# GavinLynch04/FastSelect

Hardware: AMD Instinct MI355X
Metric: feature-scores/sec (n*p/s) MultiSURF fp32 (higher is better)
Workload: dtype u16 pass 1, fp32 pass 2 (fp64 accumulation)

## Files before the change

### fastselect_amd/csrc/fs_api.cpp

```cpp
#include <cmath>
#include <cstring>
#include <string>
#include <vector>

#include "../../include/fastselect_amd.h"
#include "fs_cfs.h"
#include "fs_internal.h"
#include "fs_jmi.h"
#include "fs_mdr.h"
#include "fs_mi.h"
#include "fs_mrmr.h"
#include "fs_pairscan.h"
#include "fs_stir.h"

#include <chrono>
#include <cstdio>
#include <cstdlib>

namespace fs {
static thread_local std::string g_last_error;
void set_error(const std::string& msg) { g_last_error = msg; }

static thread_local int g_accum = FS_ACCUM_FAST;
int accumulation_mode() { return g_accum; }

TestHooks& test_hooks() {
  static TestHooks h;
  return h;
}

bool trace_on() {
  static const bool on = std::getenv("FS_TRACE") != nullptr;
  return on;
}

void trace_mark(const char* phase) {
  if (!trace_on()) return;
  using clk = std::chrono::steady_clock;
  static thread_local clk::time_point last = clk::now();
  const clk::time_point now = clk::now();
  std::fprintf(stderr, "[fs_trace] %-22s %9.3f ms\n", phase,
               std::chrono::duration<double, std::milli>(now - last).count());
  last = now;
}
}

using namespace fs;

static int map_prep_rc(int rc) { return rc == 0 ? FS_OK : FS_EINVAL; }

static int apply_accumulation(Prepared& P) {
  P.ref_accum = g_accum == FS_ACCUM_REFERENCE ? 1 : 0;
  if (P.ref_accum && P.algo == ALGO_MULTISURF && !test_hooks().ref_q16) P.no_q16 = 1;
  return FS_OK;
}

static int no_reference_devices() {
  if (g_accum != FS_ACCUM_REFERENCE) return FS_OK;
  set_error("reference-order accumulation runs on one device (its column sums are one "
            "sequential float32 sum per feature)");
  return FS_ENOTSUP;
}

static int check_backend(int backend, int device) {
  if (backend != FS_BACKEND_CPU && backend != FS_BACKEND_GPU) {
    set_error("backend must be FS_BACKEND_CPU or FS_BACKEND_GPU");
    return FS_EINVAL;
  }
  if (backend == FS_BACKEND_GPU) {
    const int nd = gpu::device_count();
    if (nd <= 0) {
      set_error("backend='gpu' was selected, but no HIP device (MI355X) is visible");
      return FS_ENODEV;
    }
    if (device < 0 || device >= nd) {
      set_error("device ordinal out of range");
      return FS_EINVAL;
    }
  }
  return FS_OK;
}

static int check_devices(const int* devices, int n) {
  if (!devices || n < 1) {
    set_error("devices: need at least one device ordinal");
    return FS_EINVAL;
  }
  const int nd = gpu::device_count();
  if (nd <= 0) {
    set_error("backend='gpu' was selected, but no HIP device (MI355X) is visible");
    return FS_ENODEV;
  }
  for (int i = 0; i < n; i++)
    if (devices[i] < 0 || devices[i] >= nd) {
      set_error("devices: ordinal " + std::to_string(devices[i]) + " out of range (" +
                std::to_string(nd) + " visible)");
      return FS_EINVAL;
    }
  return FS_OK;
}

extern "C" {

const char* fs_version(void) { return "fastselect_amd 0.1.0 (gfx950)"; }

const char* fs_last_error(void) { return g_last_error.c_str(); }

int fs_device_count(void) { return gpu::device_count(); }

int fs_set_accumulation(int mode, int* previous) {
  if (mode != FS_ACCUM_FAST && mode != FS_ACCUM_REFERENCE) {
    set_error("accumulation mode must be FS_ACCUM_FAST or FS_ACCUM_REFERENCE");
    return FS_EINVAL;
  }
  if (previous) *previous = g_accum;
  g_accum = mode;
  return FS_OK;
}

int fs_get_accumulation(void) { return g_accum; }

int fs_test_hook(const char* name, int64_t value) {
  if (!name) {
    set_error("fs_test_hook: name is NULL");
    return FS_EINVAL;
  }
  TestHooks& h = test_hooks();
  const std::string k(name);
  if (k == "reset") h = TestHooks();
  else if (k == "ksplit") h.ksplit = value;
  else if (k == "q16") h.q16 = value;
  else if (k == "sparse") h.sparse = value;
  else if (k == "shards") h.shards = value;
  else if (k == "q16_guard_off") h.q16_guard_off = value;
  else if (k == "thr_exact_all") h.thr_exact_all = value;
  else if (k == "exact_gather") h.exact_gather = value;
  else if (k == "row_panel") h.row_panel = value;
  else if (k == "rf_xlds") h.rf_xlds = value;
  else if (k == "rf_fcap") h.rf_fcap = value;
  else if (k == "ties_1w") h.ties_1w = value;
  else if (k == "ties_coop") h.ties_coop = value;
  else if (k == "rf_ref_replay") h.rf_ref_replay = value;
  else if (k == "ref_q16") h.ref_q16 = value;
  else if (k == "surf_f64") h.surf_f64 = value;
  else if (k == "star_split") h.star_split = value;
  else if (k == "colsort_star") h.colsort_star = value;
  else if (k == "colsort_bins12") h.colsort_bins12 = value;
  else if (k == "colsort_global") h.colsort_global = value;
  else if (k == "mi_tiles") h.mi_tiles = value;
  else if (k == "list_cap") h.list_cap = value;
  else if (k == "cfs_rows_cap") h.cfs_rows_cap = value;
  else if (k == "seg_len") h.seg_len = value;
  else if (k == "pass2_generic") h.pass2_generic = value;
  else if (k == "mdr_top_cap") h.mdr_top_cap = value;
  else if (k == "mdr_ranks") h.mdr_ranks = value;
  else if (k == "mdr_blocks") h.mdr_blocks = value;
  else if (k == "mdr_labels") h.mdr_labels = value;
  else if (k == "pair_tiles") h.pair_tiles = value;
  else if (k == "pair_cap") h.pair_cap = value;
  else if (k == "pair_labels") h.pair_labels = value;
  else if (k == "pair_lab_ranks") h.pair_lab_ranks = value;
  else if (k == "stir_chunk") h.stir_chunk = value;
  else if (k == "stir_seg_len") h.stir_seg_len = value;
  else {
    set_error("fs_test_hook: unknown hook '" + k + "'");
    return FS_EINVAL;
  }
  return FS_OK;
}

int fs_multisurf_last_guard(double* risk_out, int* rerun_out) {
  return gpu::multisurf_last_guard(risk_out, rerun_out);
}

int fs_device_cache_release(void) {
  gpu::dev_cache_release();
  return FS_OK;
}

int fs_host_alloc(uint64_t bytes, void** out) {
  if (!out) {
    set_error("fs_host_alloc: out is NULL");
    return FS_EINVAL;
  }
  *out = nullptr;
  if (gpu::device_count() <= 0) {
    set_error("backend='gpu' requested but no HIP device is visible");
    return FS_ENODEV;
  }
  return gpu::host_alloc(out, (size_t)bytes);
}

int fs_host_free(void* p) {
  gpu::host_free(p);
  return FS_OK;
}

int fs_stage_x(int device, const void* x, int x_is_f64, int64_t n, int64_t p, uint64_t* staged) {
  if (!x || !staged || n < 1 || p < 1) {
    set_error("fs_stage_x: need x, staged, n >= 1 and p >= 1");
    return FS_EINVAL;
  }
  if (gpu::device_count() <= 0) {
    set_error("backend='gpu' requested but no HIP device is visible");
    return FS_ENODEV;
  }
  return gpu::stage_x(device, x, x_is_f64, n, p, staged);
}

int fs_stage_x_device(int device, const void* x, const void* x_device, int x_is_f64, int64_t n,
                      int64_t p, uint64_t* staged) {
  if (!x || !x_device || !staged || n < 1 || p < 1) {
    set_error("fs_stage_x_device: need x, x_device, staged, n >= 1 and p >= 1");
    return FS_EINVAL;
  }
  if (gpu::device_count() <= 0) {
    set_error("backend='gpu' requested but no HIP device is visible");
    return FS_ENODEV;
  }
  return gpu::stage_x_device(device, x, x_device, x_is_f64, n, p, staged);
}

int fs_stage_x_cast(int device, const void* x, int x_is_f64, int64_t n, int64_t p, int n_jobs,
                    float* out, int* finite, uint64_t* staged) {
  if (!x || !out || !finite || !staged || n < 1 || p < 1) {
    set_error("fs_stage_x_cast: need x, out, finite, staged, n >= 1 and p >= 1");
    return FS_EINVAL;
  }
  if (gpu::device_count() <= 0) {
    set_error("backend='gpu' requested but no HIP device is visible");
    return FS_ENODEV;
  }
  return gpu::stage_x_cast(device, x, x_is_f64, n, p, n_jobs, out, finite, staged);
}

int fs_unstage_x(uint64_t staged) { return gpu::unstage_x(staged); }

int fs_all_finite(const void* x, int x_is_f64, int64_t n, int64_t p, int n_jobs, int* finite) {
  if (!x || !finite || n < 0 || p < 0) {
    set_error("fs_all_finite: need x, finite, n >= 0 and p >= 0");
    return FS_EINVAL;
  }
  *finite = cpu::all_finite(x, x_is_f64, n * p, n_jobs);
  return FS_OK;
}

int fs_column_stats(int backend, int device, const void* x, int x_is_f64, int64_t n, int64_t p,
                    int64_t count_cap, void* colmin_out, void* colmax_out,
                    int64_t* ndistinct_out) {
  int rc = check_backend(backend, device);
  if (rc != FS_OK) return rc;
  if (!x || !colmin_out || !colmax_out || !ndistinct_out || n < 1 || p < 1 || count_cap < 0) {
    set_error("fs_column_stats: need x, outputs, n >= 1, p >= 1 and count_cap >= 0");
    return FS_EINVAL;
  }
  const int f64 = x_is_f64 ? 1 : 0;
  trace_mark("column_stats: enter");
  if (backend == FS_BACKEND_GPU)
    rc = gpu::column_stats(x, f64, n, p, count_cap, device, colmin_out, colmax_out, ndistinct_out);
  else
    rc = cpu::column_stats(x, f64, n, p, count_cap, -1, colmin_out, colmax_out, ndistinct_out);
  trace_mark("column_stats");
  return rc;
}

int fs_multisurf_score(int backend, int device, const float* x, int64_t n, int64_t p,
                       const double* y, const float* recip, const int64_t* feat_idx,
                       int64_t n_kept, int use_star, const uint8_t* is_discrete, int n_jobs,
                       float* scores_out) {
  if (!scores_out) {
    set_error("scores_out is NULL");
    return FS_EINVAL;
  }
  int rc = check_backend(backend, device);
  if (rc != FS_OK) return rc;
  Prepared P;
  trace_mark("multisurf: enter");
  rc = prepare(P, ALGO_MULTISURF, x, 0, n, p, feat_idx, n_kept, recip, is_discrete, n_jobs,
               backend == FS_BACKEND_GPU);
  trace_mark("prepare (host)");
  if (rc) return map_prep_rc(rc);
  if (encode_labels_f64(P, y)) return FS_EINVAL;
  P.use_star = use_star ? 1 : 0;
  if ((rc = apply_accumulation(P)) != FS_OK) return rc;
  if (backend == FS_BACKEND_GPU) return gpu::multisurf_run(P, x, device, scores_out);
  cpu::CpuState st;
  std::vector<double> rs(3 * n), cnt(2 * n), S(P.n_kept);
  cpu::multisurf_pass1(P, x, 0, 1, n_jobs, st, rs.data());
  cpu::multisurf_select(P, x, 0, 1, rs.data(), n_jobs, st, cnt.data());
  cpu::multisurf_pass2(P, x, st, cnt.data(), 0, 1, n_jobs, 0, n, S.data());
  for (int64_t k = 0; k < P.n_kept; k++) scores_out[k] = (float)(S[k] / (double)n);
  return FS_OK;
}

int fs_multisurf_score_rows(int backend, int device, const float* x, int64_t n, int64_t p,
                            const double* y, const float* recip, const int64_t* feat_idx,
                            int64_t n_kept, int use_star, const uint8_t* is_discrete, int n_jobs,
                            int64_t row_begin, int64_t row_end, double* sums_out) {
  if (!sums_out) {
    set_error("sums_out is NULL");
    return FS_EINVAL;
  }
  if (!(0 <= row_begin && row_begin <= row_end && row_end <= n)) {
    set_error("row range must satisfy 0 <= row_begin <= row_end <= n");
    return FS_EINVAL;
  }
  int rc = check_backend(backend, device);
  if (rc != FS_OK) return rc;
  Prepared P;
  rc = prepare(P, ALGO_MULTISURF, x, 0, n, p, feat_idx, n_kept, recip, is_discrete, n_jobs,
               backend == FS_BACKEND_GPU);
  if (rc) return map_prep_rc(rc);
  if (encode_labels_f64(P, y)) return FS_EINVAL;
  P.use_star = use_star ? 1 : 0;
  if ((rc = apply_accumulation(P)) != FS_OK) return rc;
  if (backend == FS_BACKEND_GPU) return gpu::multisurf_rows(P, x, device, row_begin, row_end, sums_out);
  cpu::CpuState st;
  std::vector<double> rs(3 * n), cnt(2 * n);
  cpu::multisurf_pass1(P, x, 0, 1, n_jobs, st, rs.data());
  cpu::multisurf_select(P, x, 0, 1, rs.data(), n_jobs, st, cnt.data());
  return cpu::multisurf_pass2(P, x, st, cnt.data(), 0, 1, n_jobs, row_begin, row_end, sums_out);
}

static int relieff_sums(int backend, int device, const float* x, int64_t n, int64_t p,
                        const int32_t* y_enc, const float* recip, const uint8_t* is_discrete,
                        int64_t k, const float* class_probs, int64_t n_classes, int n_jobs,
                        int64_t r_lo, int64_t r_hi, double* sums, const int* devices = nullptr,
                        int n_devices = 0) {
  if (!y_enc || !class_probs || n_classes < 1 || k < 0) {
    set_error("invalid ReliefF arguments (y_enc, class_probs, n_classes, k)");
    return FS_EINVAL;
  }
  if (!(0 <= r_lo && r_lo <= r_hi && r_hi <= n)) {
    set_error("row range must satisfy 0 <= row_begin <= row_end <= n");
    return FS_EINVAL;
  }
  int rc = check_backend(backend, device);
  if (rc != FS_OK) return rc;
  Prepared P;
  trace_mark("relieff: enter");
  rc = prepare(P, ALGO_RELIEFF, x, 0, n, p, nullptr, p, recip, is_discrete, n_jobs,
               backend == FS_BACKEND_GPU);
  trace_mark("prepare (host)");
  if (rc) return map_prep_rc(rc);
  P.labels.assign(y_enc, y_enc + n);
  for (int64_t i = 0; i < n; i++)
    if (P.labels[i] < 0 || P.labels[i] >= n_classes) {
      set_error("y_enc entry outside [0, n_classes)");
      return FS_EINVAL;
    }
  P.n_classes = (int32_t)n_classes;
  P.class_prior.assign(n_classes, 0.0);
  for (int64_t c = 0; c < n_classes; c++) P.class_prior[c] = (double)class_probs[c];
  P.k_neighbors = k;
  if ((rc = apply_accumulation(P)) != FS_OK) return rc;
  if (devices) {
    if ((rc = no_reference_devices()) != FS_OK) return rc;
    if (n_classes > 64) {
      set_error("GPU ReliefF supports at most 64 classes");
      return FS_ENOTSUP;
    }
    return gpu::rows_run_devices(P, x, devices, n_devices, r_lo, r_hi, sums);
  }
  if (backend == FS_BACKEND_GPU) return gpu::relieff_run(P, x, device, r_lo, r_hi, sums);
  return cpu::relieff_run(P, x, n_jobs, r_lo, r_hi, sums);
}

static int surf_sums(int backend, int device, const double* x, int64_t n, int64_t p,
                     const int32_t* y, const float* recip, int use_star,
                     const uint8_t* is_discrete, int n_jobs, int64_t r_lo, int64_t r_hi,
                     double* sums, const int* devices = nullptr, int n_devices = 0) {
  if (!(0 <= r_lo && r_lo <= r_hi && r_hi <= n)) {
    set_error("row range must satisfy 0 <= row_begin <= row_end <= n");
    return FS_EINVAL;
  }
  int rc = check_backend(backend, device);
  if (rc != FS_OK) return rc;
  Prepared P;
  trace_mark("surf: enter");
  rc = prepare(P, ALGO_SURF, x, 1, n, p, nullptr, p, recip, is_discrete, n_jobs,
               backend == FS_BACKEND_GPU);
  trace_mark("prepare (host)");
  if (rc) return map_prep_rc(rc);
  if (encode_labels_i32(P, y)) return FS_EINVAL;
  P.use_star = use_star ? 1 : 0;
  if ((rc = apply_accumulation(P)) != FS_OK) return rc;
  if (devices) {
    if ((rc = no_reference_devices()) != FS_OK) return rc;
    return gpu::rows_run_devices(P, x, devices, n_devices, r_lo, r_hi, sums);
  }
  if (backend == FS_BACKEND_GPU) return gpu::surf_run(P, x, device, r_lo, r_hi, sums);
  return cpu::surf_run(P, x, n_jobs, r_lo, r_hi, sums);
}

int fs_relieff_score(int backend, int device, const float* x, int64_t n, int64_t p,
                     const int32_t* y_enc, const float* recip, const uint8_t* is_discrete,
                     int64_t k, const float* class_probs, int64_t n_classes, int n_jobs,
                     float* scores_out) {
  if (!scores_out) {
    set_error("scores_out is NULL");
    return FS_EINVAL;
  }
  std::vector<double> S(p > 0 ? p : 1);
  const int rc = relieff_sums(backend, device, x, n, p, y_enc, recip, is_discrete, k,
                              class_probs, n_classes, n_jobs, 0, n, S.data());
  if (rc != FS_OK) return rc;
  for (int64_t f = 0; f < p; f++) scores_out[f] = (float)(S[f] / (double)n);
  return FS_OK;
}

int fs_relieff_score_rows(int backend, int device, const float* x, int64_t n, int64_t p,
                          const int32_t* y_enc, const float* recip, const uint8_t* is_discrete,
                          int64_t k, const float* class_probs, int64_t n_classes, int n_jobs,
                          int64_t row_begin, int64_t row_end, double* sums_out) {
  if (!sums_out) {
    set_error("sums_out is NULL");
    return FS_EINVAL;
  }
  return relieff_sums(backend, device, x, n, p, y_enc, recip, is_discrete, k, class_probs,
                      n_classes, n_jobs, row_begin, row_end, sums_out);
}

int fs_surf_score(int backend, int device, const double* x, int64_t n, int64_t p,
                  const int32_t* y, const float* recip, int use_star,
                  const uint8_t* is_discrete, int n_jobs, float* scores_out) {
  if (!scores_out) {
    set_error("scores_out is NULL");
    return FS_EINVAL;
  }
  std::vector<double> S(p > 0 ? p : 1);
  const int rc = surf_sums(backend, device, x, n, p, y, recip, use_star, is_discrete, n_jobs, 0,
                           n, S.data());
  if (rc != FS_OK) return rc;
  for (int64_t f = 0; f < p; f++) scores_out[f] = (float)(S[f] / (double)n);
  return FS_OK;
}

int fs_surf_score_rows(int backend, int device, const double* x, int64_t n, int64_t p,
                       const int32_t* y, const float* recip, int use_star,
                       const uint8_t* is_discrete, int n_jobs, int64_t row_begin,
                       int64_t row_end, double* sums_out) {
  if (!sums_out) {
    set_error("sums_out is NULL");
    return FS_EINVAL;
  }
  return surf_sums(backend, device, x, n, p, y, recip, use_star, is_discrete, n_jobs, row_begin,
                   row_end, sums_out);
}

int fs_multisurf_score_devices(const int* devices, int n_devices, const float* x, int64_t n,
                               int64_t p, const double* y, const float* recip,
                               const int64_t* feat_idx, int64_t n_kept, int use_star,
                               const uint8_t* is_discrete, int n_jobs, int64_t row_begin,
                               int64_t row_end, double* sums_out) {
  if (!sums_out) {
    set_error("sums_out is NULL");
// ... 956 lines not shown
```

### fastselect_amd/csrc/fs_gpu_internal.h

```cpp
#pragma once
#include <hip/hip_runtime.h>

#include <algorithm>
#include <atomic>
#include <cmath>
#include <condition_variable>
#include <cstdio>
#include <cstdlib>
#include <cstring>
#include <map>
#include <mutex>
#include <string>
#include <thread>
#include <type_traits>
#include <unordered_map>
#include <vector>

#include "../../include/fastselect_amd.h"
#include "fs_devmem.h"
#include "fs_internal.h"

namespace fs {
namespace gpu {

#define FS_HIP(expr)                                                                      \
  do {                                                                                    \
    hipError_t e_ = (expr);                                                               \
    if (e_ != hipSuccess) {                                                               \
      set_error(std::string("HIP error '") + hipGetErrorString(e_) + "' in " #expr);      \
      return FS_EHIP;                                                                     \
    }                                                                                     \
  } while (0)

constexpr int kRowcorrMaxSlices = 16;
constexpr int kExRows = 8, kExJ = 4, kExChunk = kExJ;
constexpr int kSWaves = 16;
constexpr int kTileWeights = kTile * kTile;
constexpr int64_t kXsSlack = 512;
constexpr int kXcds = 8;


__device__ __forceinline__ uint32_t sad_u32(uint32_t a, uint32_t b, uint32_t c) {
  uint32_t d;
  asm("v_sad_u32 %0, %1, %2, %3" : "=v"(d) : "v"(a), "v"(b), "v"(c));
  return d;
}

__device__ __forceinline__ uint32_t sad_u16(uint32_t a, uint32_t b, uint32_t c) {
  uint32_t d;
  asm("v_sad_u16 %0, %1, %2, %3" : "=v"(d) : "v"(a), "v"(b), "v"(c));
  return d;
}

__device__ __forceinline__ uint32_t mismatch_u32(uint32_t a, uint32_t b, uint32_t sc, uint32_t c) {
  uint32_t t, d;
  asm("v_xor_b32 %1, %2, %3\n\tv_min_u32 %1, %1, 1\n\tv_mad_u32_u24 %0, %1, %4, %5"
      : "=v"(d), "=&v"(t)
      : "v"(a), "v"(b), "v"(sc), "v"(c));
  return d;
}

__device__ __forceinline__ double block_sum_256(double v, double* red) {
  const int tid = threadIdx.x;
  red[tid] = v;
  __syncthreads();
  for (int s = 128; s > 0; s >>= 1) {
    if (tid < s) red[tid] += red[tid + s];
    __syncthreads();
  }
  const double r = red[0];
  __syncthreads();
  return r;
}

__device__ __forceinline__ int64_t d_at(int tiled, int64_t n_pad, int64_t t, int64_t i0,
                                        int64_t j0, int a, int b) {
  return tiled ? ((t * kTile + b) * kTile + a) : ((j0 + b) * n_pad + i0 + a);
}

__device__ __forceinline__ bool d_row_in(int2 win, int64_t r) { return r >= win.x && r < win.y; }
__device__ __forceinline__ int64_t d_rd(int tiled, int2 win, int64_t n_pad, int64_t t, int64_t i0,
                                        int64_t j0, int a, int b) {
  if (tiled) return (t * kTile + b) * kTile + a;
  const int64_t j = j0 + b;
  return d_row_in(win, j) ? j * n_pad + i0 + a : (i0 + a) * n_pad + j;
}

struct Plan {
  explicit Plan(int dev) : device(dev) {}
  Prepared P;
  const int device;
  int rank = 0, world = 1;
  int x_is_f64 = 0;
  hipStream_t stream = nullptr;
  bool own_stream = false;
  hipStream_t side = nullptr;
  hipEvent_t ev_fork = nullptr, ev_join = nullptr;
  hipStream_t side2 = nullptr;
  hipEvent_t ev_star = nullptr;
  int64_t nb = 0, n_tiles = 0, seg_len = 1, nseg = 1;
  int64_t nsegpart = 1;
  int ksplit = 1;
  int64_t kfull = 0;
  int use_q16 = 0;
  double calib[7] = {0, 0, 0, 0, 1, 0, 0};
  double cal32[2] = {0, 0};
  int64_t c_lo = 0, c_hi = 0;
  int64_t r_lo = 0, r_hi = 0;
  double2* rspart = nullptr;
  double* Dpart = nullptr;
  int key_shift = 8;
  DevBuf<char> colsort_scratch{device};
  void* x = nullptr;
  const void* x_staged = nullptr;
  int64_t* src_col = nullptr;
  int64_t* out_pos = nullptr;
  double *off = nullptr, *qs = nullptr, *scl = nullptr;
  float* scl32 = nullptr;
  bool rows_direct = false;
  int64_t* dtab_off = nullptr;
  double* dtab = nullptr;
  int32_t* lab = nullptr;
  uint8_t* lab8 = nullptr;
  uint32_t* xqT = nullptr;
  float* xs = nullptr;
  float* epsT = nullptr;
  double* corr = nullptr;
  double* corr_part = nullptr;
  double* xT64 = nullptr;
  bool surf_int = false;
  double* D = nullptr;
  int tiled = 0;
  int64_t dplane = 0;
  int2 tw = make_int2(0, 0);
  int2 win = make_int2(0, 0);
  void* D_alloc = nullptr;
  float* Dk = nullptr;
  int2* tiles = nullptr;
  double* thr = nullptr;
  float* Wt = nullptr;
  float* wrow = nullptr;
  unsigned long long* nnz = nullptr;
  bool nnz_valid = false;
  int sparse = 0;
  bool star_split = false;
  float* xsT = nullptr;
  double* alpha = nullptr;
  double* tcol = nullptr;
  DevBuf<double> spart{device};
  std::vector<int2> h_tiles;
  DevBuf<int32_t> sched{device};
  int32_t* seg_off = nullptr;
  DevBuf<int2> units8{device};
  int2* units4 = nullptr;
  int64_t nunits8 = 0, nunits4 = 0, nfb8 = 0, nfb4 = 0, f_tail = 0;
  unsigned int* unc = nullptr;
  int32_t* urows = nullptr;
  DevBuf<double2> uparts{device};
  int thr_rows = kExactThrRows;
  bool thr_all = false;
  int32_t n_exact_thr = 0;
  DevBuf<int2> list{device};
  DevBuf<double> pair_part{device};
  unsigned long long* list_count = nullptr;
  int64_t n_refined = 0;
  int64_t n_tie_rows = 0;
  DevBuf<char> sort_scratch{device};
  hipEvent_t ev[6] = {nullptr, nullptr, nullptr, nullptr, nullptr, nullptr};
  std::vector<hipEvent_t> ev_stir;
  int stir_chunks = 0;
  DevArena mem_plan{device};
  DevArena mem_layout{device};
  DevArena mem_shard{device};
  DevArena mem_call{device};
  bool row_mode = false;
  bool corr_ready = false;
  bool guard_pending = false;
  std::vector<char> colmin, colmax;
  float* xk = nullptr;
  double* xk64 = nullptr;
  int64_t Kp = 0;
  int64_t* kcol = nullptr;
  float* krecip = nullptr;
  uint8_t* kdisc = nullptr;
  uint8_t* kblk = nullptr;
  uint64_t* masks = nullptr;
  int32_t* bcnt = nullptr;
  DevBuf<float> temp{device};
  int64_t ref_rows = -1;
  bool ref_defer = false;
  DevBuf<float> rkeys{device};
  bool ref_seeded = false;
  double* risk_dev = nullptr;
};

#define FS_TRY(expr)              \
  do {                            \
    int rc_ = (expr);             \
    if (rc_ != FS_OK) return rc_; \
  } while (0)

template <typename T>
int h2d(Plan* g, T* dst, const T* src, size_t count) {
  if (count == 0) return FS_OK;
  FS_HIP(hipMemcpyAsync(dst, src, count * sizeof(T), hipMemcpyHostToDevice, g->stream));
  return FS_OK;
}

inline int launch_check(const char* what) {
  hipError_t e = hipGetLastError();
  if (e != hipSuccess) {
    set_error(std::string("kernel launch failed (") + what + "): " + hipGetErrorString(e));
    return FS_EHIP;
  }
  return FS_OK;
}

hipStream_t stream_get(int device);
void stream_put(int device, hipStream_t s);
hipEvent_t event_get(int device, bool timing);
void event_put(int device, hipEvent_t e, bool timing);
struct StreamLease {
  int device;
  hipStream_t s = nullptr;
  std::vector<hipEvent_t> ev;
  explicit StreamLease(int dev) : device(dev) {}
  StreamLease(const StreamLease&) = delete;
  StreamLease& operator=(const StreamLease&) = delete;
  int open(size_t events) {
    if (!(s = stream_get(device))) return FS_EHIP;
    for (size_t k = 0; k < events; k++) {
      ev.push_back(event_get(device, true));
      if (!ev.back()) return FS_EHIP;
    }
    return FS_OK;
  }
  ~StreamLease() {
    if (s) {
      (void)hipStreamSynchronize(s);
      stream_put(device, s);
    }
    for (hipEvent_t e : ev) event_put(device, e, true);
    (void)hipGetLastError();
  }
};
inline int no_device() {
  set_error("backend='gpu' requested but no HIP device is visible");
  return FS_ENODEV;
}
int choose_ksplit(int64_t tiles, int device, int nchunks, int64_t feats, bool beside);
int calibrate_band(Plan* g);
int row_guard(Plan* g);
int apply_operand_width(Plan* g);
int run_quantize_dist(Plan* g);
int plan_score_surf(Plan* g, double* sums_dev);
int surf_resolve(Plan* g);
bool star_split_fits(int64_t n, int32_t n_classes);
int star_terms(Plan* g, hipStream_t st);
int star_sums(Plan* g, hipStream_t st, bool continuous);
int star_reduce(Plan* g, const double* counts, hipStream_t st);
int shard_segments(Plan* g);
int run_weights(Plan* g, const double* counts, int algo, double inv_sc);
int run_pass2(Plan* g, double* scores_dev);
int ref_masks(Plan* g);
int ref_temp(Plan* g, int64_t rows, float** out);
int ref_chains(Plan* g, const double* counts, double* scores);
int surf_ref(Plan* g, double* sums);
int accumulate(double* dst, const double* src, int64_t count, hipStream_t st);
int reduce_segments(const double* part, int64_t nrows, int64_t PW, const int64_t* out_pos,
                    double* sums, hipStream_t st, const double* add = nullptr);
int plan_score_relieff(Plan* g, double* sums_dev);
int relieff_run_one(const Prepared& P, const void* x, int device, int64_t r_lo, int64_t r_hi,
                    double* sums_out, const double* seed = nullptr);
int plan_layout(Plan* g);
int copy_sums(Plan* g, const double* sums_dev, double* sums_out);
int surf_run_one(const Prepared& P, const void* x, int device, int64_t r_lo, int64_t r_hi,
                 double* sums_out, const double* seed = nullptr);
extern thread_local double g_last_risk;
extern thread_local int g_last_rerun;

}
}
```

### fastselect_amd/csrc/fs_internal.h

```cpp
#pragma once

#include <cmath>
#include <condition_variable>
#include <cstdint>
#include <mutex>
#include <string>
#include <utility>
#include <vector>

#if defined(__HIPCC__)
#define FS_HD __host__ __device__
#else
#define FS_HD
#endif

namespace fs {

enum Algo : int { ALGO_MULTISURF = 0, ALGO_RELIEFF = 1, ALGO_SURF = 2 };

constexpr int kTile = 128;
constexpr int kBK64 = 16;
constexpr int kBKQ = 16;
constexpr int kFlushChunks = 256 / kBKQ;
constexpr int kHiShift = 24;
constexpr int kFeatPad = 64;
constexpr int kSubRows = 32;

void set_error(const std::string& msg);
bool trace_on();
void trace_mark(const char* phase);

struct Prepared {
  int algo = ALGO_MULTISURF;
  int use_star = 0;
  int64_t k_neighbors = 0;
  int64_t n = 0, n_pad = 0;
  int64_t p_in = 0;
  int64_t n_kept = 0;
  int64_t pc = 0, pd = 0;
  int64_t PC = 0, PD = 0, PW = 0;
  std::vector<int64_t> src_col, out_pos;
  std::vector<double> offset;
  std::vector<float> recip_in;
  std::vector<uint8_t> disc_in;
  std::vector<int64_t> kept_col;
  std::vector<double> scale;
  std::vector<int64_t> dtab_off;
  std::vector<double> dtab;
  std::vector<int32_t> labels;
  int32_t n_classes = 0;
  std::vector<double> class_prior;
  double SC = 0.0;
  uint32_t SCu = 0;
  double amb_delta = 0.0;
  double amb_delta_model = 0.0;
  double Rmax = 0.0;
  double qmax = 0.0;
  int ranges_ready = 1;
  int disc_bits = 0;
  int q16 = 0;
  int no_q16 = 0;
  int ref_accum = 0;
  int defer_guard = 0;
};

int accumulation_mode();

struct TestHooks {
  int64_t q16 = -1;
  int64_t sparse = -1;
  int64_t shards = 0;
  int64_t ksplit = 0;
  int64_t q16_guard_off = 0;
  int64_t thr_exact_all = 0;
  int64_t exact_gather = 0;
  int64_t row_panel = 0;
  int64_t rf_xlds = -1;
  int64_t rf_fcap = -1;
  int64_t ties_1w = 0;
  int64_t ties_coop = 0;
  int64_t rf_ref_replay = 0;
  int64_t ref_q16 = 0;
  int64_t surf_f64 = -1;
  int64_t star_split = -1;
  int64_t colsort_star = -1;
  int64_t colsort_bins12 = 0;
  int64_t colsort_global = 0;
  int64_t mi_tiles = 0;
  int64_t list_cap = 0;
  int64_t cfs_rows_cap = 0;
  int64_t seg_len = 0;
  int64_t pass2_generic = 0;
  int64_t mdr_top_cap = 0;
  int64_t mdr_ranks = 0;
  int64_t mdr_blocks = 0;
  int64_t mdr_labels = 0;
  int64_t pair_tiles = 0;
  int64_t pair_cap = 0;
  int64_t pair_labels = 0;
  int64_t pair_lab_ranks = 0;
  int64_t stir_chunk = 0;
  int64_t stir_seg_len = 0;
};
TestHooks& test_hooks();

int prepare(Prepared& P, int algo, const void* x, int x_is_f64, int64_t n, int64_t p_in,
            const int64_t* feat_idx, int64_t n_kept, const float* recip,
            const uint8_t* is_discrete, int n_jobs, int device_ranges = 0,
            const Prepared* dtab_src = nullptr);
int finalize_scale(Prepared& P, const double* cmin, const double* cmax);
int set_integer_scale(Prepared& P, int q16);
constexpr int64_t kCalibPairs = 4096;
void calib_pairs(int64_t n, int64_t pc, int64_t count,
                 std::vector<std::pair<int64_t, int64_t>>& out);
double calibrated_delta(double model, double SC, double rms, double max_abs);
inline int colsort_key_shift(double qmax) {
  int b = 0;
  while (b < 32 && std::ldexp(1.0, b) < qmax) b++;
  return 32 - b < 24 ? 32 - b : 24;
}
inline int32_t colsort_fx(float eps) { return (int32_t)std::llrint((double)eps * 16777216.0); }
inline uint32_t colsort_key(uint32_t q, int32_t fx, int s) {
  const uint32_t fr = (uint32_t)(((1 << 23) - fx) >> (24 - s));
  const uint32_t m = (1u << s) - 1u;
  return (q << s) | (fr < m ? fr : m);
}
constexpr int kColsortMaxFill = 64;
inline uint32_t colsort_eq12(int32_t fx) {
  const int32_t u = fx + (1 << 23);
  return (uint32_t)(u < 0 ? 0 : (u >= (1 << 24) ? 4095 : (u >> 12)));
}
inline int64_t colsort_eq12_fx(uint32_t q) { return (int64_t)(2 * q + 1) * 2048 - (int64_t(1) << 23); }
int encode_labels_f64(Prepared& P, const double* y);
int encode_labels_i32(Prepared& P, const int32_t* y);

void owned_tiles(int64_t nb, int rank, int world, std::vector<int32_t>& bi,
                 std::vector<int32_t>& bj);
void row_tiles(int64_t nb, int64_t b_lo, int64_t b_hi, std::vector<int32_t>& bi,
               std::vector<int32_t>& bj);
FS_HD inline int64_t tile_linear(int64_t nb, int64_t bi, int64_t bj) {
  return bi * nb - bi * (bi - 1) / 2 + (bj - bi);
}

int hardware_threads(int n_jobs);

constexpr int kExactThrRows = 64;
inline int64_t exact_thr_rows(int64_t n, int64_t p) {
  const double budget = 3e10 / ((double)(n > 1 ? n : 1) * (double)(p > 1 ? p : 1));
  int64_t r = n / 64 < (int64_t)budget ? n / 64 : (int64_t)budget;
  return r > kExactThrRows ? r : kExactThrRows;
}

FS_HD inline double multisurf_threshold(double s1, double s2, int64_t n) {
  const double mu = s1 / (double)(n - 1);
  double var = s2 / (double)(n - 1) - mu * mu;
  if (var < 0.0) var = 0.0;
  return mu - 0.5 * __builtin_sqrt(var);
}

FS_HD inline double multisurf_weight(bool near, bool hit, int use_star, double H, double M) {
  if (near) return hit ? -1.0 / H : 1.0 / M;
  if (use_star && !hit) return -1.0 / (M > 0.0 ? M : 1.0);
  return 0.0;
}

FS_HD inline double surf_weight(bool near, bool hit, int use_star) {
  if (near) return hit ? -1.0 : 1.0;
  if (use_star) return hit ? 1.0 : -1.0;
  return 0.0;
}

template <typename KeyFn, typename RangeFn>
FS_HD inline int numba_argsort_focus(int64_t len, int32_t* R, KeyFn key, RangeFn has_interest) {
  if (len < 2) return 0;
  constexpr int kSmall = 15, kMaxStack = 100;
  int64_t st_lo[kMaxStack], st_hi[kMaxStack];
  int ns = 1;
  st_lo[0] = 0;
  st_hi[0] = len - 1;
  while (ns > 0) {
    ns--;
    int64_t low = st_lo[ns], high = st_hi[ns];
    bool live = true;
    while (high - low >= kSmall) {
      const int64_t mid = (low + high) >> 1;
      int32_t tmp;
      if (key(R[mid]) < key(R[low])) { tmp = R[low]; R[low] = R[mid]; R[mid] = tmp; }
      if (key(R[high]) < key(R[mid])) { tmp = R[high]; R[high] = R[mid]; R[mid] = tmp; }
      if (key(R[mid]) < key(R[low])) { tmp = R[low]; R[low] = R[mid]; R[mid] = tmp; }
      const float pivot = key(R[mid]);
      tmp = R[high]; R[high] = R[mid]; R[mid] = tmp;
      int64_t i = low, j = high - 1;
      while (true) {
        while (i < high && key(R[i]) < pivot) i++;
        while (j >= low && pivot < key(R[j])) j--;
        if (i >= j) break;
        tmp = R[i]; R[i] = R[j]; R[j] = tmp;
        i++;
        j--;
      }
      tmp = R[i]; R[i] = R[high]; R[high] = tmp;
      int64_t push_lo, push_hi, keep_lo, keep_hi;
      if (high - i > i - low) {
        push_lo = i + 1; push_hi = high; keep_lo = low; keep_hi = i - 1;
      } else {
        push_lo = low; push_hi = i - 1; keep_lo = i + 1; keep_hi = high;
      }
      if (push_hi >= push_lo && has_interest(push_lo, push_hi)) {
        if (ns >= kMaxStack) return -1;
        st_lo[ns] = push_lo;
        st_hi[ns] = push_hi;
        ns++;
      }
      low = keep_lo;
      high = keep_hi;
      if (high < low || !has_interest(low, high)) {
        live = false;
        break;
      }
    }
    if (!live) continue;
    for (int64_t i = low + 1; i <= high; i++) {
      const int32_t kk = R[i];
      const float v = key(kk);
      int64_t j = i;
      while (j > low && v < key(R[j - 1])) {
        R[j] = R[j - 1];
        j--;
      }
      R[j] = kk;
    }
  }
  return 0;
}

namespace cpu {
int all_finite(const void* x, int x_is_f64, int64_t count, int n_jobs);
struct CpuState {
  std::vector<double> D;
  std::vector<float> xs;
  std::vector<double> corr;
  std::vector<double> thr;
  int64_t refined = 0;
};
int multisurf_pass1(const Prepared& P, const void* x, int rank, int world, int n_jobs,
                    CpuState& S, double* rowstats);
int multisurf_select(const Prepared& P, const void* x, int rank, int world,
                     const double* rowstats, int n_jobs, CpuState& S, double* counts);
int multisurf_pass2(const Prepared& P, const void* x, const CpuState& S, const double* counts,
                    int rank, int world, int n_jobs, int64_t r_lo, int64_t r_hi, double* scores);
int surf_run(const Prepared& P, const void* x, int n_jobs, int64_t r_lo, int64_t r_hi,
             double* scores);
int relieff_run(const Prepared& P, const void* x, int n_jobs, int64_t r_lo, int64_t r_hi,
                double* scores);
int column_stats(const void* x, int x_is_f64, int64_t n, int64_t p, int64_t cap, int n_jobs,
                 void* colmin, void* colmax, int64_t* ndistinct);
}

class StageBarrier {
 public:
  explicit StageBarrier(int n) : n_(n) {}
  bool arrive(int rc, const std::string& err) {
    std::unique_lock<std::mutex> lk(mu_);
    if (rc != 0 && rc_ == 0) {
      rc_ = rc;
      err_ = err;
    }
    const uint64_t gen = gen_;
    if (++count_ == n_) {
      count_ = 0;
      last_ok_ = rc_ == 0;
      gen_++;
      cv_.notify_all();
    } else {
      cv_.wait(lk, [&] { return gen_ != gen; });
    }
    return last_ok_;
  }
  int rc() const { return rc_; }
  const std::string& err() const { return err_; }
  int waiting() {
    std::lock_guard<std::mutex> lk(mu_);
    return count_;
  }

 private:
  std::mutex mu_;
  std::condition_variable cv_;
  int n_, count_ = 0, rc_ = 0;
  bool last_ok_ = true;
  uint64_t gen_ = 0;
  std::string err_;
};


namespace gpu {
int device_count();
int dev_alloc(void** p, size_t bytes, int device);
void dev_free(void* p);
void dev_cache_release();
int host_alloc(void** p, size_t bytes);
void host_free(void* p);
int stage_x(int device, const void* x, int x_is_f64, int64_t n, int64_t p, uint64_t* handle);
int stage_x_cast(int device, const void* x, int x_is_f64, int64_t n, int64_t p, int n_jobs,
                 float* out, int* finite, uint64_t* handle);
int stage_x_device(int device, const void* x, const void* x_dev, int x_is_f64, int64_t n,
                   int64_t p, uint64_t* handle);
int unstage_x(uint64_t handle);
const void* staged_lookup(const void* host, int64_t n, int64_t p, int x_is_f64, int device);
const void* staged_acquire(const void* host, int64_t n, int64_t p, int x_is_f64, int device);
void staged_release(const void* dev);
bool staged_extrema(const void* dev, void* cmin, void* cmax);
int column_stats(const void* x, int x_is_f64, int64_t n, int64_t p, int64_t cap, int device,
                 void* colmin, void* colmax, int64_t* ndistinct);
int column_minmax(const void* dx, int x_is_f64, int64_t n, int64_t p, void* hmin, void* hmax,
                  void* stream);
size_t pair_sort_scratch_bytes(int64_t count);
int sort_pairs(void* list, int64_t count, void* scratch, size_t scratch_bytes, void* stream);
bool colsort_lds(int64_t n);
int colsort_bin_bits(int64_t n);
size_t colsort_scratch_bytes(int64_t n, int64_t ncols);
int colsort_terms(const uint32_t* xqT, float* epsT, int64_t n, int64_t n_pad, int64_t c_lo,
                  int64_t c_hi, int q16, int key_shift, void* scratch, size_t scratch_bytes,
                  void* stream);
int colsort_star_terms(const uint32_t* xqT, float* epsT, float* xsT, const int32_t* lab,
                       const int64_t* out_pos, int ncls, int64_t n, int64_t n_pad, int64_t c_lo,
                       int64_t c_hi, int q16, int key_shift, void* stream);
struct Plan;
int plan_create(Plan** out, const Prepared& P, const void* x, int x_is_f64, int device,
                int rank, int world, uint64_t stream, int64_t r_lo = 0, int64_t r_hi = -1);
int plan_set_features(Plan* g, const Prepared& P);
int plan_pass1(Plan* g, double* rowstats_dev);
int plan_select(Plan* g, const double* rowstats_dev, double* counts_dev);
int plan_pass2(Plan* g, const double* counts_dev, double* scores_dev);
int plan_stir(Plan* g, double* sums_dev);
double plan_stir_kernel_ms(const Plan* g, int which);
int64_t ref_mask_words(const Plan* g);
int plan_ref_masks(Plan* g, uint64_t* masks_dev);
int plan_ref_pass2(Plan* g, const uint64_t* masks_dev, const double* counts_dev, int64_t row_lo,
                   int64_t row_hi);
int plan_ref_sums(Plan* g, const double* init_dev, double* sums_dev);
int plan_ref_temp(Plan* g);
int plan_decision_guard(Plan* g, const double* rowstats, const double* counts,
                        const double* sums, double* risk, int* switched);
int plan_set_rows(Plan* g, int64_t r_lo, int64_t r_hi);
int plan_set_shard(Plan* g, int rank, int world);
int multisurf_shards(const Prepared& P, int device, int world, int share = 1);
int plan_score(Plan* g, double* sums_dev);
int plan_info(const Plan* g, int64_t* tiles, double* pfe, int64_t* refined);
int plan_calibration(const Plan* g, double* out);
double plan_kernel_ms(const Plan* g, int which);
int plan_weighted_pairs(Plan* g, int64_t* pairs);
void plan_destroy(Plan* g);
int multisurf_run(const Prepared& P, const void* x, int device, float* scores_out);
int multisurf_last_guard(double* risk, int* rerun);
int multisurf_run_devices(const Prepared& P, const void* x, const int* devices, int ndev,
                          int64_t r_lo, int64_t r_hi, double* sums_out);
int rows_run_devices(const Prepared& P, const void* x, const int* devices, int ndev,
                     int64_t r_lo, int64_t r_hi, double* sums_out);
int multisurf_rows(const Prepared& P, const void* x, int device, int64_t r_lo, int64_t r_hi,
                   double* sums_out);
int surf_run(const Prepared& P, const void* x, int device, int64_t r_lo, int64_t r_hi,
             double* sums_out);
int relieff_run(const Prepared& P, const void* x, int device, int64_t r_lo, int64_t r_hi,
                double* sums_out);

namespace refacc {
int gather_kept(const float* x, int64_t n, int64_t n_pad, int64_t p_in, const int64_t* kcol,
                int64_t n_kept, int64_t Kp, float* xk, void* stream);
int gather_kept64(const double* x, int64_t n, int64_t n_pad, int64_t p_in, const int64_t* kcol,
                  int64_t n_kept, int64_t Kp, double* xk, void* stream);
int surf_masks(const double* D, int64_t n, int64_t n_pad, const double* avg, const int32_t* lab,
               int use_star, int64_t r_lo, int64_t r_hi, uint64_t* masks, void* stream);
int surf_chains(const double* xk, int64_t Kp, const float* krecip, const uint8_t* kdisc,
                const uint8_t* blkdisc, const uint64_t* masks, int64_t n, int64_t n_pad,
                int use_star, int64_t r_lo, int64_t r_hi, float* temp, void* stream);
int multisurf_masks(const double* D, int64_t n, int64_t n_pad, const void* tiles, int64_t n_tiles,
                    const double* thr, const int32_t* lab, int use_star, uint64_t* masks,
                    void* stream);
int multisurf_chains(const float* xk, int64_t Kp, const float* krecip, const uint8_t* kdisc,
                     const uint8_t* blkdisc, const uint64_t* masks, int64_t n, int64_t n_pad,
                     const double* counts, int use_star, int64_t r_lo, int64_t r_hi, float* temp,
                     void* stream);
int column_sums(const float* temp, int64_t rows, int64_t Kp, int64_t n_kept, const double* init,
                double* out, void* stream);
int relieff_order(const float* xk, int64_t Kp, const float* krecip, const uint8_t* kdisc,
                  int64_t n_kept, int C, int64_t k, int32_t* nbr, const int32_t* nfound,
                  int64_t r_lo, int64_t r_hi, float* keys, int32_t* dup, void* stream);
int relieff_row_keys(const float* xk, int64_t Kp, const float* krecip, const uint8_t* kdisc,
                     int64_t n_kept, const int32_t* rows, int64_t nr, int64_t n, float* keys,
                     void* stream);
int relieff_order_matters(const float* xk, int64_t Kp, const float* krecip,
                          const uint8_t* kdisc, int64_t n_kept, const int32_t* rows, int64_t nr,
                          const int32_t* dup, const int32_t* nbr, const int32_t* nfound,
                          int64_t r_lo, int C, int64_t k, int32_t* matters, void* stream);
// ... 8 lines not shown
```

### fastselect_amd/csrc/fs_pass2.hip

```cpp
#include "fs_gpu_internal.h"
#include "fs_sparse_asm.inc"

namespace fs {
namespace gpu {

__device__ __forceinline__ float pair_weight(const double* __restrict__ D, int64_t n, int64_t n_pad,
                                             int tiled, int2 win, int64_t t, int64_t i0, int64_t j0, int ii,
                                             int jj, bool upper,
                                             const double* __restrict__ thr,
                                             const int32_t* __restrict__ lab,
                                             const double* __restrict__ counts, int algo,
                                             int use_star, double inv_sc, int64_t r_lo,
                                             int64_t r_hi) {
  const int64_t i = i0 + ii, j = j0 + jj;
  if (!(i < n && j < n && upper)) return 0.0f;
  const double d = D[d_rd(tiled, win, n_pad, t, i0, j0, ii, jj)];
  const bool hit = lab[i] == lab[j];
  const int ws = use_star == 2 ? 0 : use_star;
  double wi, wj;
  if (algo == ALGO_MULTISURF) {
    wi = multisurf_weight(d < thr[i], hit, ws, counts[2 * i], counts[2 * i + 1]);
    wj = multisurf_weight(d < thr[j], hit, ws, counts[2 * j], counts[2 * j + 1]);
    if (use_star == 2 && !hit) {
      wi *= 2.0;
// ... 66 lines not shown
                                            int64_t c0, int wave,
                                            const int2* __restrict__ tiles,
                                            const float* __restrict__ Wt, int64_t t_begin,
                                            int64_t t_end, double& out0, double& out1) {
  double s0 = 0.0, s1 = 0.0;
  float a0[kSubRows], a1[kSubRows];
  int cur_bi = -1;
  float wA[kSubRows], wB[kSubRows];
  {
    const float* __restrict__ w0 = Wt + t_begin * (kTile * kTile) + wave * kSubRows;
#pragma unroll
    for (int r = 0; r < kSubRows; r++) wA[r] = w0[r];
  }
  for (int64_t t = t_begin; t < t_end; t++) {
    const int2 tl = tiles[t];
    if (tl.x != cur_bi) {
      cur_bi = tl.x;
      const float* __restrict__ xa = xs + ((int64_t)tl.x * kTile + wave * kSubRows) * PW + c0;
#pragma unroll
      for (int r = 0; r < kSubRows; r++) {
        a0[r] = xa[(int64_t)r * PW];
        a1[r] = TWO ? xa[(int64_t)r * PW + 64] : 0.0f;
      }
    }
    const float* __restrict__ wt = Wt + t * (kTile * kTile) + wave * kSubRows;
    const float* __restrict__ xb = xs + (int64_t)tl.y * kTile * PW + c0;
    float bA0 = xb[0], bA1 = TWO ? xb[64] : 0.0f;
    float bB0 = xb[PW], bB1 = TWO ? xb[PW + 64] : 0.0f;
    const float* __restrict__ xn = xb + 2 * PW;
    const float* __restrict__ wn = wt + kTile;
    for (int jb = 0; jb < kTile; jb += 32) {
      float acc[8] = {0.0f, 0.0f, 0.0f, 0.0f, 0.0f, 0.0f, 0.0f, 0.0f};
      for (int jj = 0; jj < 32; jj += 2) {
        const float cA0 = xn[0], cA1 = TWO ? xn[64] : 0.0f;
        const float cB0 = xn[PW], cB1 = TWO ? xn[PW + 64] : 0.0f;
        score_column<D0, D1, TWO>(a0, a1, wA, bA0, bA1, acc, wn, wB);
        score_column<D0, D1, TWO>(a0, a1, wB, bB0, bB1, acc, wn + kTile, wA);
        bA0 = cA0; bA1 = cA1; bB0 = cB0; bB1 = cB1;
        xn += 2 * PW;
        wn += 2 * kTile;
      }
      s0 += ((double)acc[0] + (double)acc[1]) + ((double)acc[2] + (double)acc[3]);
      if (TWO) s1 += ((double)acc[4] + (double)acc[5]) + ((double)acc[6] + (double)acc[7]);
    }
  }
  out0 = s0;
  out1 = s1;
}

__global__ __launch_bounds__(256) void k_score(const float* __restrict__ xs, int64_t PW,
                                               int64_t PC, const int2* __restrict__ tiles,
                                               const float* __restrict__ Wt, int64_t n_tiles,
                                               int64_t seg_len, int64_t nseg, int64_t nfb,
                                               double* __restrict__ spart) {
  __shared__ double red[2][4][64];
  const int lane = threadIdx.x & 63;
  const int wave = __builtin_amdgcn_readfirstlane(threadIdx.x >> 6);
  const int64_t w = blockIdx.x;
  const int64_t xcd = w % kXcds, k = w / kXcds;
  const int64_t seg = xcd + kXcds * (k / nfb), fb = k % nfb;
  if (seg >= nseg) return;
  const int64_t f0 = fb * 128;
  const int64_t c0 = f0 + lane;
  const int64_t t_begin = seg * seg_len;
  const int64_t t_end = t_begin + seg_len < n_tiles ? t_begin + seg_len : n_tiles;
  const bool two = f0 + 64 < PW;
  const bool d0 = f0 >= PC, d1 = f0 + 64 >= PC;
  double s0 = 0.0, s1 = 0.0;
  if (two) {
    if (!d1) score_tiles<false, false, true>(xs, PW, c0, wave, tiles, Wt, t_begin, t_end, s0, s1);
    else if (d0) score_tiles<true, true, true>(xs, PW, c0, wave, tiles, Wt, t_begin, t_end, s0, s1);
    else score_tiles<false, true, true>(xs, PW, c0, wave, tiles, Wt, t_begin, t_end, s0, s1);
  } else {
    if (d0) score_tiles<true, true, false>(xs, PW, c0, wave, tiles, Wt, t_begin, t_end, s0, s1);
    else score_tiles<false, false, false>(xs, PW, c0, wave, tiles, Wt, t_begin, t_end, s0, s1);
  }
  red[0][wave][lane] = s0;
  red[1][wave][lane] = s1;
  __syncthreads();
  if (wave < 2 && (wave == 0 || two)) {
    const double v = (red[wave][0][lane] + red[wave][1][lane]) + (red[wave][2][lane] + red[wave][3][lane]);
    spart[seg * PW + c0 + wave * 64] = v;
  }
}

constexpr int kHalf = 64;
constexpr int kWaveCols = kTile / kSWaves;
constexpr int kStreamWeights = kWaveCols * kHalf;
static_assert(kStreamWeights * 2 * kSWaves == kTileWeights, "two halves x 16 streams per tile");

__global__ __launch_bounds__(1024) void k_weights_sparse3(
    const double* __restrict__ D, int64_t n, int64_t n_pad, int tiled, int2 win,
    const int2* __restrict__ tiles, const double* __restrict__ thr,
    const int32_t* __restrict__ lab,
    const double* __restrict__ counts, int algo, int use_star, double inv_sc, int64_t r_lo,
    int64_t r_hi, float* __restrict__ wrow, unsigned long long* __restrict__ nnz) {
  __shared__ int wave_nnz[kSWaves];
  const int2 tl = tiles[blockIdx.x];
  const int64_t i0 = (int64_t)tl.x * kTile, j0 = (int64_t)tl.y * kTile;
  const int lane = threadIdx.x & 63, wave = threadIdx.x >> 6;
  float* out0 = wrow + (((int64_t)blockIdx.x * 2 + 0) * kSWaves + wave) * kStreamWeights + lane * kWaveCols;
  float* out1 = wrow + (((int64_t)blockIdx.x * 2 + 1) * kSWaves + wave) * kStreamWeights + lane * kWaveCols;
  float v0[kWaveCols], v1[kWaveCols];
  int nz = 0;
#pragma unroll
  for (int c = 0; c < kWaveCols; c++) {
    const int jj = wave + kSWaves * c;
    const float w0 = pair_weight(D, n, n_pad, tiled, win, blockIdx.x, i0, j0, lane, jj,
                                 tl.x < tl.y || lane < jj, thr, lab, counts, algo, use_star,
                                 inv_sc, r_lo, r_hi);
    const float w1 = pair_weight(D, n, n_pad, tiled, win, blockIdx.x, i0, j0, lane + 64, jj,
                                 tl.x < tl.y || lane + 64 < jj, thr, lab, counts, algo, use_star,
                                 inv_sc, r_lo, r_hi);
    v0[c] = w0 != 0.0f ? w0 : 0.0f;
    v1[c] = w1 != 0.0f ? w1 : 0.0f;
    nz += __popcll(__ballot(w0 != 0.0f)) + __popcll(__ballot(w1 != 0.0f));
  }
#pragma unroll
  for (int c = 0; c < kWaveCols; c += 4) {
    *(float4*)(out0 + c) = make_float4(v0[c], v0[c + 1], v0[c + 2], v0[c + 3]);
    *(float4*)(out1 + c) = make_float4(v1[c], v1[c + 1], v1[c + 2], v1[c + 3]);
  }
  if (lane == 0) wave_nnz[wave] = nz;
  __syncthreads();
  if (threadIdx.x == 0) {
    unsigned long long t = 0;
    for (int w = 0; w < kSWaves; w++) t += (unsigned long long)wave_nnz[w];
    atomicAdd(nnz, t);
  }
}

template <int F>
__device__ __forceinline__ void sparse3_rows_generic(const float4* __restrict__ As,
                                                     const float* __restrict__ wp,
                                                     const float* __restrict__ xb, int64_t bstride,
                                                     int lane, const bool (&disc)[F],
                                                     float (&acc)[F]) {
  constexpr int C = F / 4;
  float b[kWaveCols][F];
#pragma unroll
  for (int j = 0; j < kWaveCols; j++)
#pragma unroll
    for (int c = 0; c < C; c++) {
      const float4 v = *(const float4*)(xb + j * bstride + 256 * c);
      b[j][4 * c] = v.x; b[j][4 * c + 1] = v.y; b[j][4 * c + 2] = v.z; b[j][4 * c + 3] = v.w;
    }
  float4 a[C], an[C];
#pragma unroll
  for (int c = 0; c < C; c++) a[c] = As[64 * c + lane];
  for (int r = 0; r < kHalf; r++) {
    const int rn = (r + 1) & (kHalf - 1);
#pragma unroll
    for (int c = 0; c < C; c++) an[c] = As[(rn * 2 + c) * 64 + lane];
    float av[F];
#pragma unroll
    for (int c = 0; c < C; c++) {
      av[4 * c] = a[c].x; av[4 * c + 1] = a[c].y; av[4 * c + 2] = a[c].z; av[4 * c + 3] = a[c].w;
    }
#pragma unroll
    for (int j = 0; j < kWaveCols; j++) {
      const float w = wp[r * kWaveCols + j];
      if (__float_as_uint(w) != 0u) {
#pragma unroll
        for (int f = 0; f < F; f++)
          acc[f] = disc[f] ? pair_term<true>(av[f], b[j][f], w, acc[f])
                           : pair_term<false>(av[f], b[j][f], w, acc[f]);
      }
    }
#pragma unroll
    for (int c = 0; c < C; c++) a[c] = an[c];
  }
}


template <int F>
__device__ __forceinline__ void sparse3_stage(float4* __restrict__ As, const float* __restrict__ xs,
                                              int64_t PW, int bi, int64_t h, int64_t f0, int lane,
                                              int wave) {
  constexpr int C = F / 4;
  __syncthreads();
  const float* __restrict__ xa = xs + ((int64_t)bi * kTile + h * kHalf) * PW + f0 + 4 * lane;
  constexpr int kPer = kHalf * 2 / kSWaves;
  float4 v[kPer];
#pragma unroll
  for (int m = 0; m < kPer; m++) {
    const int rc = wave + kSWaves * m, r = rc >> 1, c = rc & 1;
    v[m] = make_float4(0.0f, 0.0f, 0.0f, 0.0f);
    if (c < C && f0 + 256 * c + 4 * lane < PW) v[m] = *(const float4*)(xa + (int64_t)r * PW + 256 * c);
  }
#pragma unroll
  for (int m = 0; m < kPer; m++) As[(wave + kSWaves * m) * 64 + lane] = v[m];
  __syncthreads();
}

template <int F>
__global__ __launch_bounds__(1024) void k_score_sparse3(
    const float* __restrict__ xs, int64_t PW, int64_t PC, const int2* __restrict__ tiles,
    const float* __restrict__ wrow, const int32_t* __restrict__ sched,
    const int32_t* __restrict__ seg_off, const int2* __restrict__ units, int64_t f_base,
    double* __restrict__ spart, int generic) {
  constexpr int C = F / 4;
  __shared__ float4 As[kHalf * 2 * 64];
  const int lane = threadIdx.x & 63;
  const int wave = __builtin_amdgcn_readfirstlane(threadIdx.x >> 6);
  const int2 unit = units[blockIdx.x];
  if (unit.x < 0) return;
  const int64_t seg = unit.x, fb = unit.y >> 1, h = unit.y & 1;
  const int64_t f0 = f_base + fb * (64 * F);
  const int64_t t_begin = seg_off[seg];
  const int64_t t_end = seg_off[seg + 1];
  const int64_t f_end = f0 + 64 * F < PW ? f0 + 64 * F : PW;
  const bool fast = f_end <= PC && !generic;
  const uint32_t lds_lane = (uint32_t)(uintptr_t)As + (uint32_t)lane * 16u;
  const uint32_t glb_lane = (uint32_t)lane * 16u;
  const int64_t bstride = kSWaves * PW;
  const uint32_t bstride_b = (uint32_t)(bstride * sizeof(float));
  double* __restrict__ out = spart + (seg * 2 + h) * PW + f0;
  int nvalid = (int)(PW - f0 < 64 * F ? PW - f0 : 64 * F);
  asm volatile("" : "+s"(out), "+s"(nvalid));
  double s[F];
#pragma unroll
  for (int q = 0; q < F; q++) s[q] = 0.0;
  __shared__ unsigned int wg_done;
  if (threadIdx.x == 0) wg_done = 0u;
  if (fast) {
    const uint64_t entw = (uint64_t)(uintptr_t)(wrow + (h * kSWaves + wave) * kStreamWeights);
    const uint64_t xsw = (uint64_t)(uintptr_t)(xs + (int64_t)wave * PW + f0);
    const uint32_t entw_lo = (uint32_t)entw, entw_hi = (uint32_t)(entw >> 32);
    const uint32_t xsw_lo = (uint32_t)xsw, xsw_hi = (uint32_t)(xsw >> 32);
    const uint32_t wgd = (uint32_t)(uintptr_t)&wg_done;
    if (t_begin < t_end) sparse3_stage<F>(As, xs, PW, tiles[sched[t_begin]].x, h, f0, lane, wave);
    for (int k0 = (int)t_begin, k_end = (int)t_end; k0 < k_end; k0 += 64) {
      const uint32_t done0 = (uint32_t)(k0 - (int)t_begin);
      const int kk = k0 + lane;
      const int my_t = sched[kk < k_end ? kk : k0];
      const int my_y = tiles[my_t].y;
      const uint32_t nt = (uint32_t)(k_end - k0 < 64 ? k_end - k0 : 64);
      if constexpr (F == 8) {
        FS_SPARSE3_SEG_ASM_F8(s, lds_lane, glb_lane, my_t, my_y, nt, entw_lo, entw_hi, xsw_lo, xsw_hi,
                              bstride_b, wgd, done0);
      } else
        FS_SPARSE3_SEG_ASM_F4(s, lds_lane, glb_lane, my_t, my_y, nt, entw_lo, entw_hi, xsw_lo, xsw_hi,
                              bstride_b, wgd, done0);
    }
  } else {
    bool disc[F];
#pragma unroll
    for (int c = 0; c < C; c++)
#pragma unroll
      for (int q = 0; q < 4; q++) disc[4 * c + q] = f0 + 256 * c + 4 * lane + q >= PC;
    unsigned int my_done = 0;
    int my_t = 0, my_x = -1, my_y = 0;
    int cur_bi = -1;
    for (int64_t k = t_begin; k < t_end; k++) {
      const int idx = (int)((k - t_begin) & 63);
      if (idx == 0) {
        const int64_t kk = k + lane;
        my_t = kk < t_end ? sched[kk] : sched[k];
        const int2 tt = tiles[my_t];
        my_x = tt.x;
        my_y = tt.y;
      }
      const int64_t t = __builtin_amdgcn_readlane(my_t, idx);
      const int2 tl = make_int2(__builtin_amdgcn_readlane(my_x, idx), __builtin_amdgcn_readlane(my_y, idx));
      if (tl.x != cur_bi) {
        sparse3_stage<F>(As, xs, PW, tl.x, h, f0, lane, wave);
        cur_bi = tl.x;
      }
      float acc[F];
#pragma unroll
      for (int q = 0; q < F; q++) acc[q] = 0.0f;
      const float* __restrict__ wp = wrow + ((t * 2 + h) * kSWaves + wave) * kStreamWeights;
      const float* __restrict__ xb = xs + ((int64_t)tl.y * kTile + wave) * PW + f0;
      sparse3_rows_generic<F>(As, wp, xb + 4 * lane, bstride, lane, disc, acc);
#pragma unroll
      for (int q = 0; q < F; q++) s[q] += (double)acc[q];
      unsigned int tot = 0;
      if (lane == 0) tot = atomicAdd(&wg_done, 1u) + 1u;
      tot = __builtin_amdgcn_readfirstlane(tot);
      ++my_done;
      if (my_done * kSWaves < tot)
        __builtin_amdgcn_s_setprio(2);
      else
        __builtin_amdgcn_s_setprio(0);
    }
  }
  __syncthreads();
  double* red = (double*)As;
#pragma unroll
  for (int q = 0; q < F; q++) red[(q * kSWaves + wave) * 64 + lane] = s[q];
  __syncthreads();
  if (wave < F) {
    const int q = wave;
    const int f = 256 * (q >> 2) + 4 * lane + (q & 3);
    const double* rr = red + q * kSWaves * 64 + lane;
    double v = 0.0;
#pragma unroll
    for (int w = 0; w < kSWaves; w += 4)
      v += (rr[w * 64] + rr[(w + 1) * 64]) + (rr[(w + 2) * 64] + rr[(w + 3) * 64]);
    if (f < nvalid) out[f] = v;
  }
}

__global__ void k_accumulate(double* __restrict__ dst, const double* __restrict__ src,
                             int64_t count) {
  const int64_t k = (int64_t)blockIdx.x * 256 + threadIdx.x;
  if (k < count) dst[k] += src[k];
}

constexpr int kReduceWaves = 16;
__global__ __launch_bounds__(1024) void k_reduce(const double* __restrict__ part, int64_t nseg,
                                                 int64_t PW, const int64_t* __restrict__ out_pos,
                                                 const double* __restrict__ add,
                                                 double* __restrict__ out) {
  __shared__ double red[kReduceWaves][64];
  const int lane = threadIdx.x & 63, wave = threadIdx.x >> 6;
  const int64_t c = (int64_t)blockIdx.x * 64 + lane;
  double s = 0.0;
  if (c < PW)
    for (int64_t g = wave; g < nseg; g += kReduceWaves) s += part[g * PW + c];
  red[wave][lane] = s;
  __syncthreads();
  if (wave != 0 || c >= PW) return;
  const int64_t o = out_pos[c];
  if (o < 0) return;
  double q[4];
#pragma unroll
  for (int k = 0; k < 4; k++)
    q[k] = (red[4 * k][lane] + red[4 * k + 1][lane]) + (red[4 * k + 2][lane] + red[4 * k + 3][lane]);
  out[o] = ((q[0] + q[1]) + (q[2] + q[3])) + (add ? add[c] : 0.0);
}

int accumulate(double* dst, const double* src, int64_t count, hipStream_t st) {
  if (count <= 0) return FS_OK;
  k_accumulate<<<(unsigned)((count + 255) / 256), 256, 0, st>>>(dst, src, count);
  return launch_check("k_accumulate");
}

int reduce_segments(const double* part, int64_t nrows, int64_t PW, const int64_t* out_pos,
                    double* sums, hipStream_t st, const double* add) {
  k_reduce<<<(unsigned)((PW + 63) / 64), 1024, 0, st>>>(part, nrows, PW, out_pos, add, sums);
  return launch_check("k_reduce");
}

#ifndef FS_SCHED_ROWS
#define FS_SCHED_ROWS 16
#endif
#ifndef FS_SCHED_UNITS
#define FS_SCHED_UNITS 32
#endif
constexpr int kSchedRows = FS_SCHED_ROWS;
constexpr int kSchedFb = FS_SCHED_UNITS / kSchedRows;

static int build_sparse_schedule(Plan* g) {
  const Prepared& Q = g->P;
  const int64_t T = g->n_tiles;
  const int64_t CJ = std::max<int64_t>(1, g->seg_len * std::max(1, g->world));
  std::vector<int32_t> sched, seg_off{0};
  std::vector<int64_t> seg_tiles;
  std::map<std::pair<int64_t, int64_t>, std::vector<int32_t>> groups;
  sched.reserve((size_t)T);
  for (int64_t t = 0; t < T;) {
    const int I = g->h_tiles[t].x;
    const int64_t c = g->h_tiles[t].y / CJ;
    int64_t e = t;
    while (e < T && e - t < 64 && g->h_tiles[e].x == I && g->h_tiles[e].y / CJ == c) e++;
    for (int64_t k = e - 1; k >= t; k--) sched.push_back((int32_t)k);
    groups[{c, I / kSchedRows}].push_back((int32_t)seg_tiles.size());
    seg_tiles.push_back(e - t);
    seg_off.push_back((int32_t)sched.size());
    t = e;
  }
  g->nseg = std::max<int64_t>(1, (int64_t)seg_tiles.size());
  g->nfb8 = Q.PW / 512;
  if (Q.PW - g->nfb8 * 512 > 256) g->nfb8++;
  g->f_tail = std::min<int64_t>(g->nfb8 * 512, Q.PW);
  g->nfb4 = (Q.PW - g->f_tail + 255) / 256;
  auto units_of = [&](int64_t nfb, std::vector<int2>& table) {
    std::vector<std::vector<int2>> per(kXcds);
    std::vector<int64_t> load(kXcds, 0);
    for (const auto& gr : groups)
      for (int64_t f0 = 0; f0 < nfb; f0 += kSchedFb) {
        int x = 0;
        for (int q = 1; q < kXcds; q++)
          if (load[q] < load[x]) x = q;
        for (int64_t fb = f0; fb < std::min<int64_t>(nfb, f0 + kSchedFb); fb++)
          for (int32_t sg : gr.second)
            for (int h = 0; h < 2; h++) {
              per[x].push_back(make_int2(sg, (int)(2 * fb + h)));
              load[x] += seg_tiles[sg];
            }
      }
    size_t kmax = 0;
    for (const auto& v : per) kmax = std::max(kmax, v.size());
    table.assign(kXcds * kmax, make_int2(-1, 0));
    for (int x = 0; x < kXcds; x++)
      for (size_t k = 0; k < per[x].size(); k++) table[x + kXcds * k] = per[x][k];
  };
  std::vector<int2> u8, u4;
  units_of(g->nfb8, u8);
  units_of(g->nfb4, u4);
  g->nunits8 = (int64_t)u8.size();
  g->nunits4 = (int64_t)u4.size();
  if (sched.empty()) sched.push_back(0);
  const size_t ns = sched.size() + seg_off.size();
  const size_t nu = std::max<size_t>(1, u8.size() + u4.size());
  FS_TRY(g->sched.reserve(ns, 0, &g->stream, 1));
  FS_TRY(g->units8.reserve(nu, 0, &g->stream, 1));
  g->seg_off = g->sched.p + sched.size();
  g->units4 = g->units8.p + u8.size();
  FS_TRY(h2d(g, g->sched.p, sched.data(), sched.size()));
  FS_TRY(h2d(g, g->seg_off, seg_off.data(), seg_off.size()));
  if (!u8.empty()) FS_TRY(h2d(g, g->units8.p, u8.data(), u8.size()));
  if (!u4.empty()) FS_TRY(h2d(g, g->units4, u4.data(), u4.size()));
  return FS_OK;
}

int shard_segments(Plan* g) {
  const Prepared& Q = g->P;
  g->corr_ready = false;
  g->c_lo = Q.pc * g->rank / g->world;
  g->c_hi = Q.pc * (g->rank + 1) / g->world;
  const int64_t nfb = !g->sparse ? (Q.PW + 127) / 128 : 2 * ((Q.PW + 511) / 512);
  const int64_t wgs =
      g->sparse ? std::min<int64_t>(32768, std::max<int64_t>(1024, g->n_tiles * nfb / 16)) : 65536;
  g->seg_len = std::max<int64_t>(1, (g->n_tiles * nfb + wgs - 1) / wgs);
  if (g->sparse && test_hooks().seg_len >= 1) g->seg_len = test_hooks().seg_len;
  g->nseg = std::max<int64_t>(1, (g->n_tiles + g->seg_len - 1) / g->seg_len);
  if (Q.algo == ALGO_RELIEFF) return FS_OK;
  if (g->sparse) FS_TRY(build_sparse_schedule(g));
  g->nsegpart = g->sparse ? 2 * g->nseg : g->nseg;
  return g->spart.reserve((size_t)g->nsegpart * Q.PW, 0, &g->stream, 1);
}

int run_weights(Plan* g, const double* counts, int algo, double inv_sc) {
  const Prepared& Q = g->P;
  if (g->star_split && algo == ALGO_MULTISURF) {
    FS_HIP(hipStreamWaitEvent(g->stream, g->ev_star, 0));
    FS_TRY(star_reduce(g, counts, g->stream));
  }
  if (g->n_tiles == 0) return FS_OK;
  const int star = g->star_split ? 2 : Q.use_star;
  if (g->sparse) {
    FS_HIP(hipMemsetAsync(g->nnz, 0, sizeof(unsigned long long), g->stream));
    g->nnz_valid = true;
    k_weights_sparse3<<<(unsigned)g->n_tiles, 64 * kSWaves, 0, g->stream>>>(
        g->D, Q.n, Q.n_pad, g->tiled, g->win, g->tiles, g->thr, g->lab, counts, algo,
        star, inv_sc, g->r_lo, g->r_hi, g->wrow, g->nnz);
    return launch_check("k_weights_sparse3");
  }
  k_weights<<<(unsigned)g->n_tiles, 256, 0, g->stream>>>(g->D, Q.n, Q.n_pad, g->tiled, g->win,
                                                         g->tiles,
                                                         g->thr,
                                                         g->lab, counts, algo, star, inv_sc,
                                                         g->r_lo, g->r_hi, g->Wt);
  return launch_check("k_weights");
}

int run_pass2(Plan* g, double* scores_dev) {
  const Prepared& Q = g->P;
  const int64_t nfb = (Q.PW + 127) / 128;
  const double* add = g->star_split ? g->tcol : nullptr;
  FS_HIP(hipMemsetAsync(scores_dev, 0, sizeof(double) * Q.n_kept, g->stream));
  if (add && Q.algo == ALGO_SURF) FS_HIP(hipStreamWaitEvent(g->stream, g->ev_join, 0));
  if (g->n_tiles == 0) {
    if (add) return reduce_segments(g->spart.p, 0, Q.PW, g->out_pos, scores_dev, g->stream, add);
    return FS_OK;
  }
  FS_HIP(hipEventRecord(g->ev[2], g->stream));
  const int64_t seg_per_xcd = (g->nseg + kXcds - 1) / kXcds;
  if (g->sparse) {
    const int generic = test_hooks().pass2_generic == 1 ? 1 : 0;
    if (g->nunits8 > 0) {
      k_score_sparse3<8><<<(unsigned)g->nunits8, 64 * kSWaves, 0, g->stream>>>(
          g->xs, Q.PW, Q.PC, g->tiles, g->wrow, g->sched.p, g->seg_off, g->units8.p, 0, g->spart.p,
          generic);
      FS_TRY(launch_check("k_score_sparse3<8>"));
    }
    if (g->nunits4 > 0) {
      k_score_sparse3<4><<<(unsigned)g->nunits4, 64 * kSWaves, 0, g->stream>>>(
          g->xs, Q.PW, Q.PC, g->tiles, g->wrow, g->sched.p, g->seg_off, g->units4, g->f_tail,
          g->spart.p, generic);
      FS_TRY(launch_check("k_score_sparse3<4>"));
    }
  } else {
    k_score<<<(unsigned)(kXcds * seg_per_xcd * nfb), 256, 0, g->stream>>>(
        g->xs, Q.PW, Q.PC, g->tiles, g->Wt, g->n_tiles, g->seg_len, g->nseg, nfb, g->spart.p);
    FS_TRY(launch_check("k_score"));
  }
  FS_HIP(hipEventRecord(g->ev[3], g->stream));
  k_reduce<<<(unsigned)((Q.PW + 63) / 64), 1024, 0, g->stream>>>(g->spart.p, g->nsegpart, Q.PW,
                                                                   g->out_pos, add, scores_dev);
  return launch_check("k_reduce");
}

int ref_masks(Plan* g) {
  const Prepared& Q = g->P;
  if (!g->masks) FS_TRY(g->mem_plan.alloc(&g->masks, (size_t)ref_mask_words(g)));
  return refacc::multisurf_masks(g->D, Q.n, Q.n_pad, g->tiles, g->n_tiles, g->thr, g->lab,
                                 Q.use_star, g->masks, g->stream);
}

int ref_temp(Plan* g, int64_t rows, float** out) {
  const size_t need = (size_t)std::max<int64_t>(rows, 1) * (size_t)g->Kp;
  FS_TRY(g->temp.reserve(need, 0, &g->stream, 1));
  *out = g->temp.p;
  return FS_OK;
}

int surf_ref(Plan* g, double* sums) {
  const Prepared& Q = g->P;
  const int64_t rows = g->r_hi - g->r_lo;
  if (!g->ref_defer && !g->ref_seeded)
    FS_HIP(hipMemsetAsync(sums, 0, sizeof(double) * Q.n_kept, g->stream));
  if (rows <= 0) {
    g->ref_rows = 0;
    return FS_OK;
  }
  uint64_t* m = nullptr;
  FS_TRY(g->mem_call.alloc(&m, (size_t)rows * (Q.n_pad / 64) * 4));
  float* temp = nullptr;
  FS_TRY(ref_temp(g, rows, &temp));
  FS_HIP(hipEventRecord(g->ev[2], g->stream));
  FS_TRY(refacc::surf_masks(g->D, Q.n, Q.n_pad, g->thr, g->lab, Q.use_star, g->r_lo, g->r_hi, m,
                            g->stream));
  FS_TRY(refacc::surf_chains(g->xk64, g->Kp, g->krecip, g->kdisc, g->kblk, m, Q.n, Q.n_pad,
                             Q.use_star, g->r_lo, g->r_hi, temp, g->stream));
  FS_HIP(hipEventRecord(g->ev[3], g->stream));
  if (g->ref_defer) {
    g->ref_rows = rows;
    return FS_OK;
  }
  return refacc::column_sums(temp, rows, g->Kp, Q.n_kept, g->ref_seeded ? sums : nullptr, sums,
                             g->stream);
}

int ref_chains(Plan* g, const double* counts, double* scores) {
  const Prepared& Q = g->P;
  const int64_t rows = g->r_hi - g->r_lo;
  FS_HIP(hipMemsetAsync(scores, 0, sizeof(double) * Q.n_kept, g->stream));
  if (rows <= 0) return FS_OK;
  float* temp = nullptr;
  FS_TRY(ref_temp(g, rows, &temp));
  FS_HIP(hipEventRecord(g->ev[2], g->stream));
  FS_TRY(refacc::multisurf_chains(g->xk, g->Kp, g->krecip, g->kdisc, g->kblk, g->masks, Q.n,
                                  Q.n_pad, counts, Q.use_star, g->r_lo, g->r_hi, temp, g->stream));
  FS_HIP(hipEventRecord(g->ev[3], g->stream));
  return refacc::column_sums(temp, rows, g->Kp, Q.n_kept, nullptr, scores, g->stream);
}

int64_t ref_mask_words(const Plan* g) {
  return g->P.n_pad * (g->P.n_pad / 64) * 4;
}

int plan_ref_masks(Plan* g, uint64_t* masks) {
  const Prepared& Q = g->P;
  FS_HIP(hipSetDevice(g->device));
  FS_HIP(hipMemsetAsync(masks, 0, sizeof(uint64_t) * (size_t)ref_mask_words(g), g->stream));
  FS_TRY(refacc::multisurf_masks(g->D, Q.n, Q.n_pad, g->tiles, g->n_tiles, g->thr, g->lab,
                                 Q.use_star, masks, g->stream));
  if (g->own_stream) FS_HIP(hipStreamSynchronize(g->stream));
  return FS_OK;
}

int plan_ref_pass2(Plan* g, const uint64_t* masks, const double* counts, int64_t lo,
                   int64_t hi) {
  const Prepared& Q = g->P;
  FS_HIP(hipSetDevice(g->device));
  g->ref_rows = std::max<int64_t>(hi - lo, 0);
  if (g->ref_rows > 0) {
    float* temp = nullptr;
    FS_TRY(ref_temp(g, g->ref_rows, &temp));
    FS_HIP(hipEventRecord(g->ev[2], g->stream));
    FS_TRY(refacc::multisurf_chains(g->xk, g->Kp, g->krecip, g->kdisc, g->kblk, masks, Q.n,
                                    Q.n_pad, counts, Q.use_star, lo, hi, temp, g->stream));
    FS_HIP(hipEventRecord(g->ev[3], g->stream));
  }
  if (g->own_stream) FS_HIP(hipStreamSynchronize(g->stream));
  return FS_OK;
}

int plan_ref_sums(Plan* g, const double* init, double* sums) {
  const Prepared& Q = g->P;
  FS_HIP(hipSetDevice(g->device));
  if (g->ref_rows < 0) {
    set_error("fs_plan_ref_sums: no fs_plan_ref_pass2 since the plan was created or re-targeted");
    return FS_EINVAL;
  }
  if (g->ref_rows == 0) {
    if (init)
      FS_HIP(hipMemcpyAsync(sums, init, sizeof(double) * Q.n_kept, hipMemcpyDeviceToDevice,
                            g->stream));
    else
      FS_HIP(hipMemsetAsync(sums, 0, sizeof(double) * Q.n_kept, g->stream));
  } else {
    FS_TRY(refacc::column_sums(g->temp.p, g->ref_rows, g->Kp, Q.n_kept, init, sums, g->stream));
  }
  if (g->own_stream) FS_HIP(hipStreamSynchronize(g->stream));
  return FS_OK;
}

int plan_pass2(Plan* g, const double* counts, double* scores) {
  const Prepared& Q = g->P;
  FS_HIP(hipSetDevice(g->device));
  if (Q.ref_accum) {
    if (g->world > 1) {
      set_error("reference-order accumulation with world > 1: pass 2 is fs_plan_ref_masks, a "
                "SUM all-reduce of the masks, then fs_plan_ref_pass2 chained over the ranks");
      return FS_ENOTSUP;
    }
    FS_TRY(ref_masks(g));
    FS_TRY(ref_chains(g, counts, scores));
    if (g->own_stream) FS_HIP(hipStreamSynchronize(g->stream));
    return FS_OK;
  }
  FS_TRY(run_weights(g, counts, ALGO_MULTISURF, 1.0 / Q.SC));
  FS_TRY(run_pass2(g, scores));
  if (g->own_stream) FS_HIP(hipStreamSynchronize(g->stream));
  return FS_OK;
}

}
}
```

### fastselect_amd/csrc/fs_plan.hip

```cpp
#include "fs_gpu_internal.h"

namespace fs {
namespace gpu {

void plan_destroy(Plan* g) {
  if (!g) return;
  if (g->stream) (void)hipStreamSynchronize(g->stream);
  trace_mark("kernels (to sync)");
  if (g->side) (void)hipStreamSynchronize(g->side);
  if (g->side2) (void)hipStreamSynchronize(g->side2);
  if (g->x_staged) staged_release(g->x_staged);
  for (auto& e : g->ev) event_put(g->device, e, true);
  for (auto& e : g->ev_stir) event_put(g->device, e, true);
  event_put(g->device, g->ev_fork, false);
  event_put(g->device, g->ev_join, false);
  event_put(g->device, g->ev_star, false);
  stream_put(g->device, g->side);
  if (g->side2) stream_put(g->device, g->side2);
  if (g->own_stream) stream_put(g->device, g->stream);
  delete g;
  trace_mark("plan: free");
}

constexpr int64_t kQ16MinRowsRF = 4096, kQ16MinRowsMS = 16384, kQ16MinRowsMSStar = 10000;
static int choose_q16(const Prepared& P) {
  if (P.algo == ALGO_SURF || P.no_q16) return 0;
  if (P.algo == ALGO_MULTISURF && P.ref_accum && !test_hooks().ref_q16) return 0;
  if (test_hooks().q16 >= 0) return test_hooks().q16 != 0 ? 1 : 0;
  const int64_t min_rows = P.algo == ALGO_RELIEFF ? kQ16MinRowsRF
                           : P.use_star           ? kQ16MinRowsMSStar
                                                  : kQ16MinRowsMS;
  return (P.n >= min_rows && P.pc >= kFeatPad) ? 1 : 0;
}

static bool choose_star_split(const Prepared& P, int device) {
  if (!P.use_star || P.ref_accum || P.algo == ALGO_RELIEFF) return false;
  if (!star_split_fits(P.n, P.n_classes)) return false;
  if (test_hooks().star_split >= 0) return test_hooks().star_split != 0;
  size_t free_b = 0, total_b = 0;
  if (hipSetDevice(device) != hipSuccess || hipMemGetInfo(&free_b, &total_b) != hipSuccess) {
    (void)hipGetLastError();
    return false;
  }
  return (double)P.n_pad * (double)P.PW * sizeof(float) <= 0.25 * (double)free_b;
}

constexpr int64_t kSparseMinRowsSurf = 4096;
static int choose_sparse(const Plan* g, const Prepared& P) {
  if (P.algo == ALGO_RELIEFF) return 0;
  if (test_hooks().sparse >= 0) return test_hooks().sparse != 0 ? 1 : 0;
  if (g->star_split) return 1;
  if (!P.use_star) return (P.algo == ALGO_MULTISURF || P.n >= kSparseMinRowsSurf ||
                           g->r_hi - g->r_lo < P.n) ? 1 : 0;
  return (P.algo == ALGO_SURF && g->r_hi - g->r_lo < P.n) ? 1 : 0;
}

static int ref_layout(Plan* g) {
  const Prepared& Q = g->P;
  const bool surf = Q.algo == ALGO_SURF;
  if (g->x_is_f64 != (surf ? 1 : 0)) {
    set_error("reference-order accumulation: float32 X for MultiSURF / ReliefF, float64 for SURF");
    return FS_ENOTSUP;
  }
  const int64_t blk_w = surf ? 128 : 256;
  g->Kp = (Q.n_kept + blk_w - 1) / blk_w * blk_w;
  std::vector<float> rec((size_t)g->Kp, 0.0f);
  std::vector<uint8_t> dsc((size_t)g->Kp, 0), blk((size_t)(g->Kp / blk_w), 0);
  for (int64_t k = 0; k < Q.n_kept; k++) {
    const int64_t col = Q.kept_col[k];
    rec[k] = Q.recip_in[col];
    dsc[k] = Q.disc_in[col] ? 1 : 0;
    if (dsc[k]) blk[k / blk_w] = 1;
  }
  g->xk = nullptr;
  g->xk64 = nullptr;
  DevArena& M = g->mem_layout;
  int rc;
  if ((rc = surf ? M.alloc(&g->xk64, (size_t)Q.n_pad * g->Kp)
                 : M.alloc(&g->xk, (size_t)Q.n_pad * g->Kp)) ||
      (rc = M.alloc(&g->kcol, Q.n_kept)) || (rc = M.alloc(&g->krecip, g->Kp)) ||
      (rc = M.alloc(&g->kdisc, g->Kp)) || (rc = M.alloc(&g->kblk, g->Kp / blk_w)) ||
      (rc = h2d(g, g->kcol, Q.kept_col.data(), Q.n_kept)) ||
      (rc = h2d(g, g->krecip, rec.data(), rec.size())) ||
      (rc = h2d(g, g->kdisc, dsc.data(), dsc.size())) ||
      (rc = h2d(g, g->kblk, blk.data(), blk.size())))
    return rc;
  rc = surf ? refacc::gather_kept64((const double*)g->x, Q.n, Q.n_pad, Q.p_in, g->kcol, Q.n_kept,
                                    g->Kp, g->xk64, g->stream)
            : refacc::gather_kept((const float*)g->x, Q.n, Q.n_pad, Q.p_in, g->kcol, Q.n_kept,
                                  g->Kp, g->xk, g->stream);
  if (rc == FS_OK) FS_HIP(hipStreamSynchronize(g->stream));
  return rc;
}

static int size_exact_rows(Plan* g) {
  const Prepared& Q = g->P;
  if (Q.algo != ALGO_MULTISURF) return FS_OK;
  g->thr_rows = (int)(g->thr_all ? Q.n : exact_thr_rows(Q.n, Q.pc + Q.pd));
  const int64_t nchunk = (Q.n + kExChunk - 1) / kExChunk;
  return g->uparts.reserve((size_t)g->thr_rows * nchunk, 0, &g->stream, 1);
}

int plan_layout(Plan* g) {
  Prepared& Q = g->P;
  g->corr_ready = false;
  FS_HIP(hipStreamSynchronize(g->stream));
  if (g->side) FS_HIP(hipStreamSynchronize(g->side));
  if (g->side2) FS_HIP(hipStreamSynchronize(g->side2));
  g->mem_call.release();
  g->mem_layout.release();
  int rc;
  Q.q16 = g->use_q16;
  if (!Q.ranges_ready) {
    const size_t esz = g->x_is_f64 ? 8 : 4;
    if (g->colmin.empty()) {
      g->colmin.resize((size_t)Q.p_in * esz);
      g->colmax.resize((size_t)Q.p_in * esz);
      if (!(g->x_staged && staged_extrema(g->x_staged, g->colmin.data(), g->colmax.data()))) {
        if ((rc = column_minmax(g->x, g->x_is_f64, Q.n, Q.p_in, g->colmin.data(),
                                g->colmax.data(), g->stream))) {
          g->colmin.clear();
          return rc;
        }
        trace_mark("plan: device ranges");
      }
    }
    std::vector<double> cmin((size_t)Q.pc), cmax((size_t)Q.pc);
    for (int64_t c = 0; c < Q.pc; c++) {
      const int64_t col = Q.src_col[c];
      cmin[c] = g->x_is_f64 ? ((const double*)g->colmin.data())[col]
                            : (double)((const float*)g->colmin.data())[col];
      cmax[c] = g->x_is_f64 ? ((const double*)g->colmax.data())[col]
                            : (double)((const float*)g->colmax.data())[col];
    }
    if (finalize_scale(Q, cmin.data(), cmax.data())) return FS_EINVAL;
  } else if (set_integer_scale(Q, Q.q16)) {
    return FS_EINVAL;
  }
  g->key_shift = colsort_key_shift(Q.qmax);
  DevArena& M = g->mem_layout;
  rc = FS_OK;
  if ((rc = M.alloc(&g->src_col, Q.PW)) || (rc = M.alloc(&g->out_pos, Q.PW)) ||
      (rc = M.alloc(&g->off, Q.PW)) || (rc = M.alloc(&g->qs, Q.PW)) ||
      (rc = M.alloc(&g->scl, Q.PW)) || (rc = M.alloc(&g->scl32, Q.PW)) ||
      (rc = M.alloc(&g->dtab_off, Q.PW + 1)) ||
      (rc = M.alloc(&g->dtab, Q.dtab.size())) ||
      (rc = M.alloc(&g->xs, (size_t)(Q.n_pad + 2) * Q.PW + kXsSlack)) ||
      (g->star_split && ((rc = M.alloc(&g->xsT, (size_t)Q.PW * Q.n_pad)) ||
                         (rc = M.alloc(&g->tcol, Q.PW))))) {
  } else if (Q.algo == ALGO_SURF) {
  } else if ((rc = M.alloc(&g->xqT, (size_t)Q.PW * Q.n_pad)) == FS_OK) {
    rc = M.alloc(&g->epsT, (size_t)Q.PW * Q.n_pad);
  }
  if (rc) return rc;
  if ((rc = shard_segments(g))) return rc;
  std::vector<double> qs(Q.PW, 0.0);
  for (int64_t c = 0; c < Q.PW; c++) qs[c] = Q.scale[c] * Q.SC;
  std::vector<float> scl32(Q.PW, 0.0f);
  for (int64_t c = 0; c < Q.PW; c++) scl32[c] = (float)Q.scale[c];
  g->rows_direct = !g->x_is_f64 && Q.pd == 0 && Q.pc == Q.p_in && Q.p_in % 4 == 0;
  for (int64_t c = 0; g->rows_direct && c < Q.pc; c++) g->rows_direct = Q.src_col[c] == c;
  if ((rc = h2d(g, g->src_col, Q.src_col.data(), Q.PW)) ||
      (rc = h2d(g, g->out_pos, Q.out_pos.data(), Q.PW)) ||
      (rc = h2d(g, g->off, Q.offset.data(), Q.PW)) || (rc = h2d(g, g->qs, qs.data(), Q.PW)) ||
      (rc = h2d(g, g->scl, Q.scale.data(), Q.PW)) ||
      (rc = h2d(g, g->scl32, scl32.data(), Q.PW)) ||
      (rc = h2d(g, g->dtab_off, Q.dtab_off.data(), Q.PW + 1)) ||
      (rc = h2d(g, g->dtab, Q.dtab.data(), Q.dtab.size())))
    return rc;
  if ((rc = size_exact_rows(g))) return rc;
  if (Q.ref_accum && (rc = ref_layout(g))) return rc;
  if ((rc = calibrate_band(g))) return rc;
  if (Q.algo == ALGO_SURF) {
    if ((rc = g->surf_int ? M.alloc(&g->xqT, (size_t)Q.PW * Q.n_pad)
                          : M.alloc(&g->xT64, (size_t)Q.PW * Q.n_pad)))
      return rc;
  }
  if ((rc = row_guard(g))) return rc;
  if (g->calib[5] != 0.0 && (rc = apply_operand_width(g))) return rc;
  FS_HIP(hipStreamSynchronize(g->stream));
  return FS_OK;
}

int apply_operand_width(Plan* g) {
  const Prepared& Q = g->P;
  std::vector<double> qs(Q.PW, 0.0);
  for (int64_t c = 0; c < Q.PW; c++) qs[c] = Q.scale[c] * Q.SC;
  g->key_shift = colsort_key_shift(Q.qmax);
  FS_TRY(h2d(g, g->qs, qs.data(), Q.PW));
  FS_HIP(hipStreamSynchronize(g->stream));
  return FS_OK;
}

static int setup_shard(Plan* g, const std::vector<int32_t>& bi, const std::vector<int32_t>& bj) {
  const Prepared& Q = g->P;
  g->n_tiles = (int64_t)bi.size();
  std::vector<int2> tl(g->n_tiles);
  for (int64_t t = 0; t < g->n_tiles; t++) tl[t] = make_int2(bi[t], bj[t]);
  g->h_tiles = tl;
  g->tiled = (Q.algo == ALGO_MULTISURF && !g->row_mode) ? 1 : 0;
  if (g->tiled) {
    g->win = make_int2(0, 0);
  } else {
    const int64_t w0 = g->row_mode ? g->r_lo / kTile * kTile : 0;
    const int64_t w1 = g->row_mode ? std::min<int64_t>(Q.n_pad, (g->r_hi + kTile - 1) / kTile * kTile)
                                   : Q.n_pad;
    g->win = make_int2((int)w0, (int)std::max(w0, w1));
  }
  g->dplane = g->tiled ? std::max<int64_t>(g->n_tiles, 1) * kTile * kTile
                       : std::max<int64_t>((int64_t)(g->win.y - g->win.x), 1) * Q.n_pad;
  g->tw = g->tiled ? make_int2((int)g->nb, g->world) : make_int2(0, 0);
  const int64_t rows_q = (g->use_q16 ? Q.PC / 2 : Q.PC) + Q.PD;
  g->ksplit = choose_ksplit(g->n_tiles, g->device, (int)(rows_q / kBKQ),
                            (g->use_q16 ? Q.pc / 2 : Q.pc) + Q.pd,
                            Q.algo == ALGO_MULTISURF && Q.pc > 0);
  if (test_hooks().ksplit >= 1) g->ksplit = (int)std::min<int64_t>(16, test_hooks().ksplit);
  const bool dkeys = Q.algo == ALGO_RELIEFF;
  if (dkeys) g->ksplit = 1;
  g->kfull = g->ksplit > 1 ? 0 : g->n_tiles;
  DevArena& M = g->mem_shard;
  int rc = FS_OK;
  g->Dk = nullptr;
  if ((rc = dkeys ? M.alloc((float**)&g->D_alloc, (size_t)g->dplane)
                  : M.alloc((double**)&g->D_alloc, (size_t)g->dplane)) ||
      (dkeys ? (g->Dk = (float*)g->D_alloc - (int64_t)g->win.x * Q.n_pad, g->D = nullptr)
             : (g->D = (double*)g->D_alloc - (g->tiled ? 0 : (int64_t)g->win.x * Q.n_pad)),
       false) ||
      (rc = M.alloc(&g->tiles, g->n_tiles)) ||
      (rc = M.alloc(&g->rspart, (size_t)std::max<int64_t>(g->n_tiles, 1) * 256))) {
  } else if (Q.algo != ALGO_RELIEFF && !g->sparse) {
    rc = M.alloc(&g->Wt, (size_t)(g->n_tiles + 1) * kTile * kTile);
  } else if (g->sparse) {
    const size_t count = (size_t)(g->n_tiles + 1) * kTileWeights;
    if (!(rc = M.alloc(&g->wrow, count)) && !(rc = M.alloc(&g->nnz, 1)) &&
        hipMemsetAsync(g->wrow + (size_t)g->n_tiles * kTileWeights, 0,
                       sizeof(float) * kTileWeights, g->stream) != hipSuccess)
      rc = FS_EHIP;
  }
  if (!rc && g->ksplit > 1)
    rc = M.alloc(&g->Dpart,
                (size_t)(g->n_tiles - g->kfull) * (g->ksplit - 1) * kTile * kTile);
  if (rc) return rc;
  g->nnz_valid = false;
  return h2d(g, g->tiles, tl.data(), g->n_tiles);
}

int plan_set_shard(Plan* g, int rank, int world) {
  if (g->P.algo != ALGO_MULTISURF || g->row_mode) {
    set_error("tile shards of a plan are MultiSURF-only");
    return FS_EINVAL;
  }
  if (world < 1 || rank < 0 || rank >= world) {
    set_error("invalid shard rank/world");
    return FS_EINVAL;
  }
  FS_HIP(hipSetDevice(g->device));
  FS_HIP(hipStreamSynchronize(g->stream));
  if (g->side) FS_HIP(hipStreamSynchronize(g->side));
  if (g->side2) FS_HIP(hipStreamSynchronize(g->side2));
  g->mem_call.release();
  g->mem_shard.release();
  g->D = g->Dpart = nullptr;
  g->D_alloc = nullptr;
  g->Wt = nullptr;
  g->wrow = nullptr;
  g->tiles = nullptr;
  g->rspart = nullptr;
  g->nnz = nullptr;
  g->rank = rank;
  g->world = world;
  std::vector<int32_t> bi, bj;
  owned_tiles(g->nb, rank, world, bi, bj);
  FS_TRY(setup_shard(g, bi, bj));
  return shard_segments(g);
}

int plan_create(Plan** out, const Prepared& P, const void* x, int x_is_f64, int device,
                int rank, int world, uint64_t stream, int64_t r_lo, int64_t r_hi) {
  *out = nullptr;
  const int ndev = device_count();
  if (ndev <= 0) {
    set_error("backend='gpu' requested but no HIP device is visible");
    return FS_ENODEV;
  }
  if (device < 0 || device >= ndev) {
    set_error("device ordinal out of range");
    return FS_EINVAL;
  }
  if (world < 1 || rank < 0 || rank >= world) {
    set_error("invalid rank/world");
    return FS_EINVAL;
  }
  if (P.n >= (1 << 20)) {
    set_error("the GPU backend supports fewer than 2^20 samples");
    return FS_ENOTSUP;
  }
  const bool row_mode = r_hi >= 0;
  if (row_mode && !(0 <= r_lo && r_lo <= r_hi && r_hi <= P.n)) {
    set_error("row range outside [0, n)");
    return FS_EINVAL;
  }
  FS_HIP(hipSetDevice(device));
  Plan* g = new Plan(device);
  g->P = P;
  g->rank = rank;
  g->world = world;
  g->x_is_f64 = x_is_f64;
  if (stream) {
    g->stream = (hipStream_t)(uintptr_t)stream;
  } else {
    if (!(g->stream = stream_get(device))) {
      delete g;
      return FS_EHIP;
    }
    g->own_stream = true;
  }
  auto fail = [&](int rc) {
    plan_destroy(g);
    return rc;
  };
  for (auto& e : g->ev)
    if (!(e = event_get(device, true))) return fail(FS_EHIP);
  if (!(g->side = stream_get(device)) || !(g->ev_fork = event_get(device, false)) ||
      !(g->ev_join = event_get(device, false)) || !(g->ev_star = event_get(device, false)))
    return fail(FS_EHIP);
  const Prepared& Q = g->P;
  g->nb = Q.n_pad / kTile;
  std::vector<int32_t> bi, bj;
  if (row_mode) {
    g->r_lo = r_lo;
    g->r_hi = r_hi;
    if (r_hi > r_lo) row_tiles(g->nb, r_lo / kTile, (r_hi + kTile - 1) / kTile, bi, bj);
  } else {
    g->r_lo = 0;
    g->r_hi = Q.n;
    owned_tiles(g->nb, rank, world, bi, bj);
  }
  g->row_mode = row_mode;
  int64_t list_cap = Q.algo == ALGO_RELIEFF ? 1 : std::max<int64_t>(1 << 16, Q.n * 64);
  if (test_hooks().list_cap >= 1) list_cap = test_hooks().list_cap;
  g->use_q16 = choose_q16(Q);
  const size_t xbytes = (size_t)Q.n * Q.p_in * (x_is_f64 ? 8 : 4);
  DevArena& M = g->mem_plan;
  int rc;
  trace_mark("plan: host setup");
  g->x_staged = staged_acquire(x, Q.n, Q.p_in, x_is_f64, g->device);
  if (g->x_staged) g->x = const_cast<void*>(g->x_staged);
  if ((!g->x_staged && (rc = M.alloc((char**)&g->x, xbytes))) ||
      (rc = M.alloc(&g->lab, Q.n_pad)) ||
      (rc = M.alloc(&g->corr, Q.n_pad)) ||
      (rc = M.alloc(&g->corr_part, (int64_t)kRowcorrMaxSlices * Q.n_pad)) ||
      (rc = M.alloc(&g->thr, Q.n_pad)) ||
      (rc = g->list.reserve((size_t)list_cap, 0, &g->stream, 1)) ||
      (rc = M.alloc(&g->list_count, 1)))
    return fail(rc);
  if (Q.algo == ALGO_MULTISURF) {
    g->thr_all = test_hooks().thr_exact_all != 0;
// ... 416 lines not shown
```

### fastselect_amd/csrc/fs_sparse_asm.inc

```

#define FS_SPARSE3_SEG_ASM_F8(s_, lds_lane_, glb_lane_, tiles_, ys_, nt_, entw_lo_, entw_hi_, xsw_lo_, xsw_hi_, bstride_, wgd_, done0_)  \
  asm volatile(  \
      "s_mov_b32 s22, 0\n"  \
      "v_readlane_b32 s68, %[tiles], s22\n"  \
      "s_nop 0\n"  \
      "s_lshl_b32 s72, s68, 16\n"  \
      "s_lshr_b32 s73, s68, 16\n"  \
      "s_add_u32 s24, %[entw_lo], s72\n"  \
      "s_addc_u32 s25, %[entw_hi], s73\n"  \
      "v_readlane_b32 s68, %[ys], s22\n"  \
      "s_nop 0\n"  \
      "s_lshl_b32 s70, %[bstride], 3\n"  \
      "s_mul_i32 s72, s68, s70\n"  \
      "s_mul_hi_u32 s73, s68, s70\n"  \
      "s_add_u32 s20, %[xsw_lo], s72\n"  \
      "s_addc_u32 s21, %[xsw_hi], s73\n"  \
      "s_load_dwordx16 s[36:51], s[24:25], 0x0\n"  \
      "s_load_dwordx16 s[52:67], s[24:25], 0x40\n"  \
      "global_load_dwordx4 v[30:33], %[glb_lane], s[20:21]\n"  \
      "global_load_dwordx4 v[34:37], %[glb_lane], s[20:21] offset:1024\n"  \
      "s_add_u32 s20, s20, %[bstride]\n"  \
      "s_addc_u32 s21, s21, 0\n"  \
      "global_load_dwordx4 v[38:41], %[glb_lane], s[20:21]\n"  \
      "global_load_dwordx4 v[42:45], %[glb_lane], s[20:21] offset:1024\n"  \
// ... 2987 lines not shown
      "s_cbranch_scc1 177f\n"  \
      "v_sub_f32 v70, v66, v46\n"  \
      "v_sub_f32 v71, v67, v47\n"  \
      "v_sub_f32 v72, v68, v48\n"  \
      "v_sub_f32 v73, v69, v49\n"  \
      "v_fma_f32 v75, s80, |v70|, v75\n"  \
      "v_fma_f32 v76, s80, |v71|, v76\n"  \
      "v_fma_f32 v77, s80, |v72|, v77\n"  \
      "v_fma_f32 v78, s80, |v73|, v78\n"  \
      "177:\n"  \
      "s_cmp_eq_u32 s81, 0\n"  \
      "s_cbranch_scc1 178f\n"  \
      "v_sub_f32 v70, v66, v50\n"  \
      "v_sub_f32 v71, v67, v51\n"  \
      "v_sub_f32 v72, v68, v52\n"  \
      "v_sub_f32 v73, v69, v53\n"  \
      "v_fma_f32 v75, s81, |v70|, v75\n"  \
      "v_fma_f32 v76, s81, |v71|, v76\n"  \
      "v_fma_f32 v77, s81, |v72|, v77\n"  \
      "v_fma_f32 v78, s81, |v73|, v78\n"  \
      "178:\n"  \
      "s_cmp_eq_u32 s82, 0\n"  \
      "s_cbranch_scc1 179f\n"  \
      "v_sub_f32 v70, v66, v54\n"  \
      "v_sub_f32 v71, v67, v55\n"  \
      "v_sub_f32 v72, v68, v56\n"  \
      "v_sub_f32 v73, v69, v57\n"  \
      "v_fma_f32 v75, s82, |v70|, v75\n"  \
      "v_fma_f32 v76, s82, |v71|, v76\n"  \
      "v_fma_f32 v77, s82, |v72|, v77\n"  \
      "v_fma_f32 v78, s82, |v73|, v78\n"  \
      "179:\n"  \
      "s_cmp_eq_u32 s83, 0\n"  \
      "s_cbranch_scc1 180f\n"  \
      "v_sub_f32 v70, v66, v58\n"  \
      "v_sub_f32 v71, v67, v59\n"  \
      "v_sub_f32 v72, v68, v60\n"  \
      "v_sub_f32 v73, v69, v61\n"  \
      "v_fma_f32 v75, s83, |v70|, v75\n"  \
      "v_fma_f32 v76, s83, |v71|, v76\n"  \
      "v_fma_f32 v77, s83, |v72|, v77\n"  \
      "v_fma_f32 v78, s83, |v73|, v78\n"  \
      "180:\n"  \
      "ds_read_b128 v[66:69], v74 offset:14336\n"  \
      "s_waitcnt lgkmcnt(1)\n"  \
      "s_cmp_eq_u32 s84, 0\n"  \
      "s_cbranch_scc1 181f\n"  \
      "v_sub_f32 v70, v62, v30\n"  \
      "v_sub_f32 v71, v63, v31\n"  \
      "v_sub_f32 v72, v64, v32\n"  \
      "v_sub_f32 v73, v65, v33\n"  \
      "v_fma_f32 v75, s84, |v70|, v75\n"  \
      "v_fma_f32 v76, s84, |v71|, v76\n"  \
      "v_fma_f32 v77, s84, |v72|, v77\n"  \
      "v_fma_f32 v78, s84, |v73|, v78\n"  \
      "181:\n"  \
      "s_cmp_eq_u32 s85, 0\n"  \
      "s_cbranch_scc1 182f\n"  \
      "v_sub_f32 v70, v62, v34\n"  \
      "v_sub_f32 v71, v63, v35\n"  \
      "v_sub_f32 v72, v64, v36\n"  \
      "v_sub_f32 v73, v65, v37\n"  \
      "v_fma_f32 v75, s85, |v70|, v75\n"  \
      "v_fma_f32 v76, s85, |v71|, v76\n"  \
      "v_fma_f32 v77, s85, |v72|, v77\n"  \
      "v_fma_f32 v78, s85, |v73|, v78\n"  \
      "182:\n"  \
      "s_cmp_eq_u32 s86, 0\n"  \
      "s_cbranch_scc1 183f\n"  \
      "v_sub_f32 v70, v62, v38\n"  \
      "v_sub_f32 v71, v63, v39\n"  \
      "v_sub_f32 v72, v64, v40\n"  \
      "v_sub_f32 v73, v65, v41\n"  \
      "v_fma_f32 v75, s86, |v70|, v75\n"  \
      "v_fma_f32 v76, s86, |v71|, v76\n"  \
      "v_fma_f32 v77, s86, |v72|, v77\n"  \
      "v_fma_f32 v78, s86, |v73|, v78\n"  \
      "183:\n"  \
      "s_cmp_eq_u32 s87, 0\n"  \
      "s_cbranch_scc1 184f\n"  \
      "v_sub_f32 v70, v62, v42\n"  \
      "v_sub_f32 v71, v63, v43\n"  \
      "v_sub_f32 v72, v64, v44\n"  \
      "v_sub_f32 v73, v65, v45\n"  \
      "v_fma_f32 v75, s87, |v70|, v75\n"  \
      "v_fma_f32 v76, s87, |v71|, v76\n"  \
      "v_fma_f32 v77, s87, |v72|, v77\n"  \
      "v_fma_f32 v78, s87, |v73|, v78\n"  \
      "184:\n"  \
      "s_cmp_eq_u32 s88, 0\n"  \
      "s_cbranch_scc1 185f\n"  \
      "v_sub_f32 v70, v62, v46\n"  \
      "v_sub_f32 v71, v63, v47\n"  \
      "v_sub_f32 v72, v64, v48\n"  \
      "v_sub_f32 v73, v65, v49\n"  \
      "v_fma_f32 v75, s88, |v70|, v75\n"  \
      "v_fma_f32 v76, s88, |v71|, v76\n"  \
      "v_fma_f32 v77, s88, |v72|, v77\n"  \
      "v_fma_f32 v78, s88, |v73|, v78\n"  \
      "185:\n"  \
      "s_cmp_eq_u32 s89, 0\n"  \
      "s_cbranch_scc1 186f\n"  \
      "v_sub_f32 v70, v62, v50\n"  \
      "v_sub_f32 v71, v63, v51\n"  \
      "v_sub_f32 v72, v64, v52\n"  \
      "v_sub_f32 v73, v65, v53\n"  \
      "v_fma_f32 v75, s89, |v70|, v75\n"  \
      "v_fma_f32 v76, s89, |v71|, v76\n"  \
      "v_fma_f32 v77, s89, |v72|, v77\n"  \
      "v_fma_f32 v78, s89, |v73|, v78\n"  \
      "186:\n"  \
      "s_cmp_eq_u32 s90, 0\n"  \
      "s_cbranch_scc1 187f\n"  \
      "v_sub_f32 v70, v62, v54\n"  \
      "v_sub_f32 v71, v63, v55\n"  \
      "v_sub_f32 v72, v64, v56\n"  \
      "v_sub_f32 v73, v65, v57\n"  \
      "v_fma_f32 v75, s90, |v70|, v75\n"  \
      "v_fma_f32 v76, s90, |v71|, v76\n"  \
      "v_fma_f32 v77, s90, |v72|, v77\n"  \
      "v_fma_f32 v78, s90, |v73|, v78\n"  \
      "187:\n"  \
      "s_cmp_eq_u32 s91, 0\n"  \
      "s_cbranch_scc1 188f\n"  \
      "v_sub_f32 v70, v62, v58\n"  \
      "v_sub_f32 v71, v63, v59\n"  \
      "v_sub_f32 v72, v64, v60\n"  \
      "v_sub_f32 v73, v65, v61\n"  \
      "v_fma_f32 v75, s91, |v70|, v75\n"  \
      "v_fma_f32 v76, s91, |v71|, v76\n"  \
      "v_fma_f32 v77, s91, |v72|, v77\n"  \
      "v_fma_f32 v78, s91, |v73|, v78\n"  \
      "188:\n"  \
      "v_mov_b32 v74, %[lds_lane]\n"  \
      "ds_read_b128 v[62:65], v74\n"  \
      "s_waitcnt lgkmcnt(1)\n"  \
      "s_cmp_eq_u32 s92, 0\n"  \
      "s_cbranch_scc1 189f\n"  \
      "v_sub_f32 v70, v66, v30\n"  \
      "v_sub_f32 v71, v67, v31\n"  \
      "v_sub_f32 v72, v68, v32\n"  \
      "v_sub_f32 v73, v69, v33\n"  \
      "v_fma_f32 v75, s92, |v70|, v75\n"  \
      "v_fma_f32 v76, s92, |v71|, v76\n"  \
      "v_fma_f32 v77, s92, |v72|, v77\n"  \
      "v_fma_f32 v78, s92, |v73|, v78\n"  \
      "189:\n"  \
      "global_load_dwordx4 v[30:33], %[glb_lane], s[20:21]\n"  \
      "s_add_u32 s20, s20, %[bstride]\n"  \
      "s_addc_u32 s21, s21, 0\n"  \
      "s_cmp_eq_u32 s93, 0\n"  \
      "s_cbranch_scc1 190f\n"  \
      "v_sub_f32 v70, v66, v34\n"  \
      "v_sub_f32 v71, v67, v35\n"  \
      "v_sub_f32 v72, v68, v36\n"  \
      "v_sub_f32 v73, v69, v37\n"  \
      "v_fma_f32 v75, s93, |v70|, v75\n"  \
      "v_fma_f32 v76, s93, |v71|, v76\n"  \
      "v_fma_f32 v77, s93, |v72|, v77\n"  \
      "v_fma_f32 v78, s93, |v73|, v78\n"  \
      "190:\n"  \
      "global_load_dwordx4 v[34:37], %[glb_lane], s[20:21]\n"  \
      "s_add_u32 s20, s20, %[bstride]\n"  \
      "s_addc_u32 s21, s21, 0\n"  \
      "s_cmp_eq_u32 s94, 0\n"  \
      "s_cbranch_scc1 191f\n"  \
      "v_sub_f32 v70, v66, v38\n"  \
      "v_sub_f32 v71, v67, v39\n"  \
      "v_sub_f32 v72, v68, v40\n"  \
      "v_sub_f32 v73, v69, v41\n"  \
      "v_fma_f32 v75, s94, |v70|, v75\n"  \
      "v_fma_f32 v76, s94, |v71|, v76\n"  \
      "v_fma_f32 v77, s94, |v72|, v77\n"  \
      "v_fma_f32 v78, s94, |v73|, v78\n"  \
      "191:\n"  \
      "global_load_dwordx4 v[38:41], %[glb_lane], s[20:21]\n"  \
      "s_add_u32 s20, s20, %[bstride]\n"  \
      "s_addc_u32 s21, s21, 0\n"  \
      "s_cmp_eq_u32 s95, 0\n"  \
      "s_cbranch_scc1 192f\n"  \
      "v_sub_f32 v70, v66, v42\n"  \
      "v_sub_f32 v71, v67, v43\n"  \
      "v_sub_f32 v72, v68, v44\n"  \
      "v_sub_f32 v73, v69, v45\n"  \
      "v_fma_f32 v75, s95, |v70|, v75\n"  \
      "v_fma_f32 v76, s95, |v71|, v76\n"  \
      "v_fma_f32 v77, s95, |v72|, v77\n"  \
      "v_fma_f32 v78, s95, |v73|, v78\n"  \
      "192:\n"  \
      "global_load_dwordx4 v[42:45], %[glb_lane], s[20:21]\n"  \
      "s_add_u32 s20, s20, %[bstride]\n"  \
      "s_addc_u32 s21, s21, 0\n"  \
      "s_cmp_eq_u32 s96, 0\n"  \
      "s_cbranch_scc1 193f\n"  \
      "v_sub_f32 v70, v66, v46\n"  \
      "v_sub_f32 v71, v67, v47\n"  \
      "v_sub_f32 v72, v68, v48\n"  \
      "v_sub_f32 v73, v69, v49\n"  \
      "v_fma_f32 v75, s96, |v70|, v75\n"  \
      "v_fma_f32 v76, s96, |v71|, v76\n"  \
      "v_fma_f32 v77, s96, |v72|, v77\n"  \
      "v_fma_f32 v78, s96, |v73|, v78\n"  \
      "193:\n"  \
      "global_load_dwordx4 v[46:49], %[glb_lane], s[20:21]\n"  \
      "s_add_u32 s20, s20, %[bstride]\n"  \
      "s_addc_u32 s21, s21, 0\n"  \
      "s_cmp_eq_u32 s97, 0\n"  \
      "s_cbranch_scc1 194f\n"  \
      "v_sub_f32 v70, v66, v50\n"  \
      "v_sub_f32 v71, v67, v51\n"  \
      "v_sub_f32 v72, v68, v52\n"  \
      "v_sub_f32 v73, v69, v53\n"  \
      "v_fma_f32 v75, s97, |v70|, v75\n"  \
      "v_fma_f32 v76, s97, |v71|, v76\n"  \
      "v_fma_f32 v77, s97, |v72|, v77\n"  \
      "v_fma_f32 v78, s97, |v73|, v78\n"  \
      "194:\n"  \
      "global_load_dwordx4 v[50:53], %[glb_lane], s[20:21]\n"  \
      "s_add_u32 s20, s20, %[bstride]\n"  \
      "s_addc_u32 s21, s21, 0\n"  \
      "s_cmp_eq_u32 s98, 0\n"  \
      "s_cbranch_scc1 195f\n"  \
      "v_sub_f32 v70, v66, v54\n"  \
      "v_sub_f32 v71, v67, v55\n"  \
      "v_sub_f32 v72, v68, v56\n"  \
      "v_sub_f32 v73, v69, v57\n"  \
      "v_fma_f32 v75, s98, |v70|, v75\n"  \
      "v_fma_f32 v76, s98, |v71|, v76\n"  \
      "v_fma_f32 v77, s98, |v72|, v77\n"  \
      "v_fma_f32 v78, s98, |v73|, v78\n"  \
      "195:\n"  \
      "global_load_dwordx4 v[54:57], %[glb_lane], s[20:21]\n"  \
      "s_add_u32 s20, s20, %[bstride]\n"  \
      "s_addc_u32 s21, s21, 0\n"  \
      "s_cmp_eq_u32 s99, 0\n"  \
      "s_cbranch_scc1 196f\n"  \
      "v_sub_f32 v70, v66, v58\n"  \
      "v_sub_f32 v71, v67, v59\n"  \
      "v_sub_f32 v72, v68, v60\n"  \
      "v_sub_f32 v73, v69, v61\n"  \
      "v_fma_f32 v75, s99, |v70|, v75\n"  \
      "v_fma_f32 v76, s99, |v71|, v76\n"  \
      "v_fma_f32 v77, s99, |v72|, v77\n"  \
      "v_fma_f32 v78, s99, |v73|, v78\n"  \
      "196:\n"  \
      "global_load_dwordx4 v[58:61], %[glb_lane], s[20:21]\n"  \
      "v_cvt_f64_f32 v[70:71], v75\n"  \
      "v_add_f64 %[s0], %[s0], v[70:71]\n"  \
      "v_mov_b32 v75, 0\n"  \
      "v_cvt_f64_f32 v[70:71], v76\n"  \
      "v_add_f64 %[s1], %[s1], v[70:71]\n"  \
      "v_mov_b32 v76, 0\n"  \
      "v_cvt_f64_f32 v[70:71], v77\n"  \
      "v_add_f64 %[s2], %[s2], v[70:71]\n"  \
      "v_mov_b32 v77, 0\n"  \
      "v_cvt_f64_f32 v[70:71], v78\n"  \
      "v_add_f64 %[s3], %[s3], v[70:71]\n"  \
      "v_mov_b32 v78, 0\n"  \
      "v_mov_b32 v72, %[wgd]\n"  \
      "v_min_u32 v73, 1, %[glb_lane]\n"  \
      "v_xor_b32 v73, 1, v73\n"  \
      "ds_add_rtn_u32 v72, v72, v73\n"  \
      "s_add_u32 s22, s22, 1\n"  \
      "s_add_u32 s69, s22, 1\n"  \
      "s_sub_u32 s70, %[nt], 1\n"  \
      "s_min_u32 s69, s69, s70\n"  \
      "v_readlane_b32 s68, %[tiles], s69\n"  \
      "s_nop 0\n"  \
      "s_lshl_b32 s72, s68, 16\n"  \
      "s_lshr_b32 s73, s68, 16\n"  \
      "s_add_u32 s26, %[entw_lo], s72\n"  \
      "s_addc_u32 s27, %[entw_hi], s73\n"  \
      "v_readlane_b32 s68, %[ys], s69\n"  \
      "s_nop 0\n"  \
      "s_lshl_b32 s70, %[bstride], 3\n"  \
      "s_mul_i32 s72, s68, s70\n"  \
      "s_mul_hi_u32 s73, s68, s70\n"  \
      "s_add_u32 s20, %[xsw_lo], s72\n"  \
      "s_addc_u32 s21, %[xsw_hi], s73\n"  \
      "s_waitcnt lgkmcnt(0)\n"  \
      "s_nop 0\n"  \
      "v_readfirstlane_b32 s68, v72\n"  \
      "s_nop 0\n"  \
      "s_add_u32 s68, s68, 1\n"  \
      "s_add_u32 s70, s22, %[done0]\n"  \
      "s_lshl_b32 s70, s70, 4\n"  \
      "s_cmp_lt_u32 s70, s68\n"  \
      "s_cbranch_scc1 64f\n"  \
      "s_setprio 0\n"  \
      "s_branch 65f\n"  \
      "64:\n"  \
      "s_setprio 2\n"  \
      "65:\n"  \
      "s_cmp_lt_u32 s22, %[nt]\n"  \
      "s_cbranch_scc1 50b\n"  \
      "s_waitcnt vmcnt(0) lgkmcnt(0)\n"  \
      : [s0] "+v"(s_[0]), [s1] "+v"(s_[1]), [s2] "+v"(s_[2]), [s3] "+v"(s_[3])  \
      : [lds_lane] "v"(lds_lane_), [glb_lane] "v"(glb_lane_), [tiles] "v"(tiles_), [ys] "v"(ys_),  \
        [nt] "s"(nt_), [entw_lo] "s"(entw_lo_), [entw_hi] "s"(entw_hi_), [xsw_lo] "s"(xsw_lo_),  \
        [xsw_hi] "s"(xsw_hi_), [bstride] "s"(bstride_), [wgd] "s"(wgd_),  \
        [done0] "s"(done0_)  \
      : "v30", "v31", "v32", "v33", "v34", "v35", "v36", "v37", "v38", "v39", "v40", "v41", "v42", "v43", "v44", "v45", "v46", "v47", "v48", "v49", "v50", "v51", "v52", "v53", "v54", "v55", "v56", "v57", "v58", "v59", "v60", "v61", "v62", "v63", "v64", "v65", "v66", "v67", "v68", "v69", "v70", "v71", "v72", "v73", "v74", "v75", "v76", "v77", "v78",  \
        "s0", "s1", "s2", "s3", "s20", "s21", "s22", "s23", "s24", "s25", "s26", "s27", "s36", "s37", "s38", "s39", "s40", "s41", "s42", "s43", "s44", "s45", "s46", "s47", "s48", "s49", "s50", "s51", "s52", "s53", "s54", "s55", "s56", "s57", "s58", "s59", "s60", "s61", "s62", "s63", "s64", "s65", "s66", "s67", "s68", "s69", "s70", "s71", "s72", "s73", "s74", "s75", "s76", "s77", "s78", "s79", "s80", "s81", "s82", "s83", "s84", "s85", "s86", "s87", "s88", "s89", "s90", "s91", "s92", "s93", "s94", "s95", "s96", "s97", "s98", "s99", "scc", "memory")
```

Baseline: 2.887 billion.

## Add narrow 4-feature-per-lane sparse pass-2 kernel for leading feature blocks

```diff
diff --git a/fastselect_amd/csrc/fs_api.cpp b/fastselect_amd/csrc/fs_api.cpp
--- a/fastselect_amd/csrc/fs_api.cpp
+++ b/fastselect_amd/csrc/fs_api.cpp
@@ -152,6 +152,7 @@
   else if (k == "cfs_rows_cap") h.cfs_rows_cap = value;
   else if (k == "seg_len") h.seg_len = value;
   else if (k == "pass2_generic") h.pass2_generic = value;
+  else if (k == "pass2_w8") h.pass2_w8 = value;
   else if (k == "mdr_top_cap") h.mdr_top_cap = value;
   else if (k == "mdr_ranks") h.mdr_ranks = value;
   else if (k == "mdr_blocks") h.mdr_blocks = value;
diff --git a/fastselect_amd/csrc/fs_gpu_internal.h b/fastselect_amd/csrc/fs_gpu_internal.h
--- a/fastselect_amd/csrc/fs_gpu_internal.h
+++ b/fastselect_amd/csrc/fs_gpu_internal.h
@@ -153,7 +153,9 @@
   int32_t* seg_off = nullptr;
   DevBuf<int2> units8{device};
   int2* units4 = nullptr;
+  int2* unitsw = nullptr;
   int64_t nunits8 = 0, nunits4 = 0, nfb8 = 0, nfb4 = 0, f_tail = 0;
+  int64_t nunitsw = 0, nfbw = 0, f_w8 = 0;
   unsigned int* unc = nullptr;
   int32_t* urows = nullptr;
   DevBuf<double2> uparts{device};
@@ -260,6 +262,7 @@
 int star_sums(Plan* g, hipStream_t st, bool continuous);
 int star_reduce(Plan* g, const double* counts, hipStream_t st);
 int shard_segments(Plan* g);
+int choose_w8(int64_t units, double tiles_per_seg);
 int run_weights(Plan* g, const double* counts, int algo, double inv_sc);
 int run_pass2(Plan* g, double* scores_dev);
 int ref_masks(Plan* g);
diff --git a/fastselect_amd/csrc/fs_internal.h b/fastselect_amd/csrc/fs_internal.h
--- a/fastselect_amd/csrc/fs_internal.h
+++ b/fastselect_amd/csrc/fs_internal.h
@@ -91,6 +91,7 @@
   int64_t cfs_rows_cap = 0;
   int64_t seg_len = 0;
   int64_t pass2_generic = 0;
+  int64_t pass2_w8 = -1;
   int64_t mdr_top_cap = 0;
   int64_t mdr_ranks = 0;
   int64_t mdr_blocks = 0;
diff --git a/fastselect_amd/csrc/fs_pass2.hip b/fastselect_amd/csrc/fs_pass2.hip
--- a/fastselect_amd/csrc/fs_pass2.hip
+++ b/fastselect_amd/csrc/fs_pass2.hip
@@ -392,6 +392,74 @@
   }
 }
 
+__global__ __launch_bounds__(1024, 8) void k_score_sparse3_w8(
+    const float* __restrict__ xs, int64_t PW, const int2* __restrict__ tiles,
+    const float* __restrict__ wrow, const int32_t* __restrict__ sched,
+    const int32_t* __restrict__ seg_off, const int2* __restrict__ units,
+    double* __restrict__ spart) {
+  constexpr int F = 4;
+  __shared__ float4 As[kHalf * 64];
+  __shared__ unsigned int wg_done;
+  const int lane = threadIdx.x & 63;
+  const int wave = __builtin_amdgcn_readfirstlane(threadIdx.x >> 6);
+  const int2 unit = units[blockIdx.x];
+  if (unit.x < 0) return;
+  const int64_t seg = unit.x, fb = unit.y >> 1, h = unit.y & 1;
+  const int64_t f0 = fb * (64 * F);
+  const int t_begin = seg_off[seg], t_end = seg_off[seg + 1];
+  const uint32_t lds_lane = (uint32_t)(uintptr_t)As + (uint32_t)lane * 16u;
+  const uint32_t glb_lane = (uint32_t)lane * 16u;
+  const uint32_t bstride_b = (uint32_t)(kSWaves * PW * sizeof(float));
+  double* __restrict__ out = spart + (seg * 2 + h) * PW + f0;
+  int nvalid = (int)(PW - f0 < 64 * F ? PW - f0 : 64 * F);
+  asm volatile("" : "+s"(out), "+s"(nvalid));
+  double s[F] = {0.0, 0.0, 0.0, 0.0};
+  if (threadIdx.x == 0) wg_done = 0u;
+  if (t_begin < t_end) {
+    const int bi = tiles[sched[t_begin]].x;
+    const float* __restrict__ xa = xs + ((int64_t)bi * kTile + h * kHalf + wave) * PW + f0 + 4 * lane;
+    constexpr int kPer = kHalf / kSWaves;
+    float4 v[kPer];
+#pragma unroll
+    for (int m = 0; m < kPer; m++) {
+      v[m] = make_float4(0.0f, 0.0f, 0.0f, 0.0f);
+      if (f0 + 4 * lane < PW) v[m] = *(const float4*)(xa + (int64_t)(kSWaves * m) * PW);
+    }
+#pragma unroll
+    for (int m = 0; m < kPer; m++) As[(wave + kSWaves * m) * 64 + lane] = v[m];
+    __syncthreads();
+    const uint64_t entw = (uint64_t)(uintptr_t)(wrow + (h * kSWaves + wave) * kStreamWeights);
+    const uint64_t xsw = (uint64_t)(uintptr_t)(xs + (int64_t)wave * PW + f0);
+    const uint32_t entw_lo = (uint32_t)entw, entw_hi = (uint32_t)(entw >> 32);
+    const uint32_t xsw_lo = (uint32_t)xsw, xsw_hi = (uint32_t)(xsw >> 32);
+    const uint32_t wgd = (uint32_t)(uintptr_t)&wg_done;
+    for (int k0 = t_begin; k0 < t_end; k0 += 64) {
+      const uint32_t done0 = (uint32_t)(k0 - t_begin);
+      const int kk = k0 + lane;
+      const int my_t = sched[kk < t_end ? kk : k0];
+      const int my_y = tiles[my_t].y;
+      const uint32_t nt = (uint32_t)(t_end - k0 < 64 ? t_end - k0 : 64);
+      FS_SPARSE3_SEG_ASM_W8(s, lds_lane, glb_lane, my_t, my_y, nt, entw_lo, entw_hi, xsw_lo, xsw_hi,
+                            bstride_b, wgd, done0);
+    }
+  }
+  __syncthreads();
+  double* red = (double*)As;
+#pragma unroll
+  for (int q = 0; q < F; q++) red[(q * kSWaves + wave) * 64 + lane] = s[q];
+  __syncthreads();
+  if (wave < F) {
+    const int q = wave;
+    const int f = 4 * lane + q;
+    const double* rr = red + q * kSWaves * 64 + lane;
+    double v = 0.0;
+#pragma unroll
+    for (int w = 0; w < kSWaves; w += 4)
+      v += (rr[w * 64] + rr[(w + 1) * 64]) + (rr[(w + 2) * 64] + rr[(w + 3) * 64]);
+    if (f < nvalid) out[f] = v;
+  }
+}
+
 __global__ void k_accumulate(double* __restrict__ dst, const double* __restrict__ src,
                              int64_t count) {
   const int64_t k = (int64_t)blockIdx.x * 256 + threadIdx.x;
@@ -441,6 +509,10 @@
 #endif
 constexpr int kSchedRows = FS_SCHED_ROWS;
 constexpr int kSchedFb = FS_SCHED_UNITS / kSchedRows;
+#ifndef FS_SCHED_FB_W8
+#define FS_SCHED_FB_W8 4
+#endif
+constexpr int kSchedFbW8 = FS_SCHED_FB_W8;
 
 static int build_sparse_schedule(Plan* g) {
   const Prepared& Q = g->P;
@@ -462,19 +534,24 @@
     t = e;
   }
   g->nseg = std::max<int64_t>(1, (int64_t)seg_tiles.size());
-  g->nfb8 = Q.PW / 512;
-  if (Q.PW - g->nfb8 * 512 > 256) g->nfb8++;
-  g->f_tail = std::min<int64_t>(g->nfb8 * 512, Q.PW);
+  const int64_t nfb_all = 2 * ((Q.PW + 511) / 512);
+  const int w8 = choose_w8(g->nseg * 2 * nfb_all, (double)T / (double)g->nseg);
+  g->nfbw = !w8 ? 0 : Q.PC == Q.PW ? (Q.PW + 255) / 256 : Q.PC / 256;
+  g->f_w8 = std::min<int64_t>(g->nfbw * 256, Q.PW);
+  const int64_t rest = Q.PW - g->f_w8;
+  g->nfb8 = rest / 512;
+  if (rest - g->nfb8 * 512 > 256) g->nfb8++;
+  g->f_tail = std::min<int64_t>(g->f_w8 + g->nfb8 * 512, Q.PW);
   g->nfb4 = (Q.PW - g->f_tail + 255) / 256;
-  auto units_of = [&](int64_t nfb, std::vector<int2>& table) {
+  auto units_of = [&](int64_t nfb, int64_t kfb, std::vector<int2>& table) {
     std::vector<std::vector<int2>> per(kXcds);
     std::vector<int64_t> load(kXcds, 0);
     for (const auto& gr : groups)
-      for (int64_t f0 = 0; f0 < nfb; f0 += kSchedFb) {
+      for (int64_t f0 = 0; f0 < nfb; f0 += kfb) {
         int x = 0;
         for (int q = 1; q < kXcds; q++)
           if (load[q] < load[x]) x = q;
-        for (int64_t fb = f0; fb < std::min<int64_t>(nfb, f0 + kSchedFb); fb++)
+        for (int64_t fb = f0; fb < std::min<int64_t>(nfb, f0 + kfb); fb++)
           for (int32_t sg : gr.second)
             for (int h = 0; h < 2; h++) {
               per[x].push_back(make_int2(sg, (int)(2 * fb + h)));
@@ -487,22 +564,26 @@
     for (int x = 0; x < kXcds; x++)
       for (size_t k = 0; k < per[x].size(); k++) table[x + kXcds * k] = per[x][k];
   };
-  std::vector<int2> u8, u4;
-  units_of(g->nfb8, u8);
-  units_of(g->nfb4, u4);
+  std::vector<int2> u8, u4, uw;
+  units_of(g->nfb8, kSchedFb, u8);
+  units_of(g->nfb4, kSchedFb, u4);
+  units_of(g->nfbw, kSchedFbW8, uw);
   g->nunits8 = (int64_t)u8.size();
   g->nunits4 = (int64_t)u4.size();
+  g->nunitsw = (int64_t)uw.size();
   if (sched.empty()) sched.push_back(0);
   const size_t ns = sched.size() + seg_off.size();
-  const size_t nu = std::max<size_t>(1, u8.size() + u4.size());
+  const size_t nu = std::max<size_t>(1, u8.size() + u4.size() + uw.size());
   FS_TRY(g->sched.reserve(ns, 0, &g->stream, 1));
   FS_TRY(g->units8.reserve(nu, 0, &g->stream, 1));
   g->seg_off = g->sched.p + sched.size();
   g->units4 = g->units8.p + u8.size();
+  g->unitsw = g->units4 + u4.size();
   FS_TRY(h2d(g, g->sched.p, sched.data(), sched.size()));
   FS_TRY(h2d(g, g->seg_off, seg_off.data(), seg_off.size()));
   if (!u8.empty()) FS_TRY(h2d(g, g->units8.p, u8.data(), u8.size()));
   if (!u4.empty()) FS_TRY(h2d(g, g->units4, u4.data(), u4.size()));
+  if (!uw.empty()) FS_TRY(h2d(g, g->unitsw, uw.data(), uw.size()));
   return FS_OK;
 }
 
@@ -561,10 +642,15 @@
   const int64_t seg_per_xcd = (g->nseg + kXcds - 1) / kXcds;
   if (g->sparse) {
     const int generic = test_hooks().pass2_generic == 1 ? 1 : 0;
+    if (g->nunitsw > 0) {
+      k_score_sparse3_w8<<<(unsigned)g->nunitsw, 64 * kSWaves, 0, g->stream>>>(
+          g->xs, Q.PW, g->tiles, g->wrow, g->sched.p, g->seg_off, g->unitsw, g->spart.p);
+      FS_TRY(launch_check("k_score_sparse3_w8"));
+    }
     if (g->nunits8 > 0) {
       k_score_sparse3<8><<<(unsigned)g->nunits8, 64 * kSWaves, 0, g->stream>>>(
-          g->xs, Q.PW, Q.PC, g->tiles, g->wrow, g->sched.p, g->seg_off, g->units8.p, 0, g->spart.p,
-          generic);
+          g->xs, Q.PW, Q.PC, g->tiles, g->wrow, g->sched.p, g->seg_off, g->units8.p, g->f_w8,
+          g->spart.p, generic);
       FS_TRY(launch_check("k_score_sparse3<8>"));
     }
     if (g->nunits4 > 0) {
diff --git a/fastselect_amd/csrc/fs_plan.hip b/fastselect_amd/csrc/fs_plan.hip
--- a/fastselect_amd/csrc/fs_plan.hip
+++ b/fastselect_amd/csrc/fs_plan.hip
@@ -53,6 +53,17 @@
   if (!P.use_star) return (P.algo == ALGO_MULTISURF || P.n >= kSparseMinRowsSurf ||
                            g->r_hi - g->r_lo < P.n) ? 1 : 0;
   return (P.algo == ALGO_SURF && g->r_hi - g->r_lo < P.n) ? 1 : 0;
+}
+
+#ifndef FS_W8_MIN_UNITS
+#define FS_W8_MIN_UNITS 3520
+#endif
+constexpr int64_t kW8MinUnits = FS_W8_MIN_UNITS;
+int choose_w8(int64_t units, double tiles_per_seg) {
+  if (test_hooks().pass2_generic == 1) return 0;
+  if (test_hooks().pass2_w8 >= 0) return test_hooks().pass2_w8 != 0 ? 1 : 0;
+  (void)tiles_per_seg;
+  return units >= kW8MinUnits ? 1 : 0;
 }
 
 static int ref_layout(Plan* g) {
diff --git a/fastselect_amd/csrc/fs_sparse_asm.inc b/fastselect_amd/csrc/fs_sparse_asm.inc
--- a/fastselect_amd/csrc/fs_sparse_asm.inc
+++ b/fastselect_amd/csrc/fs_sparse_asm.inc
@@ -3313,3 +3313,1072 @@
         [done0] "s"(done0_)  \
       : "v30", "v31", "v32", "v33", "v34", "v35", "v36", "v37", "v38", "v39", "v40", "v41", "v42", "v43", "v44", "v45", "v46", "v47", "v48", "v49", "v50", "v51", "v52", "v53", "v54", "v55", "v56", "v57", "v58", "v59", "v60", "v61", "v62", "v63", "v64", "v65", "v66", "v67", "v68", "v69", "v70", "v71", "v72", "v73", "v74", "v75", "v76", "v77", "v78",  \
         "s0", "s1", "s2", "s3", "s20", "s21", "s22", "s23", "s24", "s25", "s26", "s27", "s36", "s37", "s38", "s39", "s40", "s41", "s42", "s43", "s44", "s45", "s46", "s47", "s48", "s49", "s50", "s51", "s52", "s53", "s54", "s55", "s56", "s57", "s58", "s59", "s60", "s61", "s62", "s63", "s64", "s65", "s66", "s67", "s68", "s69", "s70", "s71", "s72", "s73", "s74", "s75", "s76", "s77", "s78", "s79", "s80", "s81", "s82", "s83", "s84", "s85", "s86", "s87", "s88", "s89", "s90", "s91", "s92", "s93", "s94", "s95", "s96", "s97", "s98", "s99", "scc", "memory")
+
+#define FS_SPARSE3_SEG_ASM_W8(s_, lds_lane_, glb_lane_, tiles_, ys_, nt_, entw_lo_, entw_hi_, xsw_lo_, xsw_hi_, bstride_, wgd_, done0_)  \
+  asm volatile(  \
+      "s_mov_b32 s22, 0\n"  \
+      "v_readlane_b32 s52, %[tiles], s22\n"  \
+      "s_nop 0\n"  \
+      "s_lshl_b32 s56, s52, 16\n"  \
+      "s_lshr_b32 s57, s52, 16\n"  \
+      "s_add_u32 s24, %[entw_lo], s56\n"  \
+      "s_addc_u32 s25, %[entw_hi], s57\n"  \
+      "v_readlane_b32 s52, %[ys], s22\n"  \
+      "s_nop 0\n"  \
+      "s_lshl_b32 s54, %[bstride], 3\n"  \
+      "s_mul_i32 s56, s52, s54\n"  \
+      "s_mul_hi_u32 s57, s52, s54\n"  \
+      "s_add_u32 s20, %[xsw_lo], s56\n"  \
+      "s_addc_u32 s21, %[xsw_hi], s57\n"  \
+      "s_load_dwordx16 s[36:51], s[24:25], 0x0\n"  \
+      "global_load_dwordx4 v[14:17], %[glb_lane], s[20:21]\n"  \
+      "s_add_u32 s20, s20, %[bstride]\n"  \
+      "s_addc_u32 s21, s21, 0\n"  \
+      "global_load_dwordx4 v[18:21], %[glb_lane], s[20:21]\n"  \
+      "s_add_u32 s20, s20, %[bstride]\n"  \
+      "s_addc_u32 s21, s21, 0\n"  \
+      "global_load_dwordx4 v[22:25], %[glb_lane], s[20:21]\n"  \
+      "s_add_u32 s20, s20, %[bstride]\n"  \
+      "s_addc_u32 s21, s21, 0\n"  \
+      "global_load_dwordx4 v[26:29], %[glb_lane], s[20:21]\n"  \
+      "s_add_u32 s20, s20, %[bstride]\n"  \
+      "s_addc_u32 s21, s21, 0\n"  \
+      "global_load_dwordx4 v[30:33], %[glb_lane], s[20:21]\n"  \
+      "s_add_u32 s20, s20, %[bstride]\n"  \
+      "s_addc_u32 s21, s21, 0\n"  \
+      "global_load_dwordx4 v[34:37], %[glb_lane], s[20:21]\n"  \
+      "s_add_u32 s20, s20, %[bstride]\n"  \
+      "s_addc_u32 s21, s21, 0\n"  \
+      "global_load_dwordx4 v[38:41], %[glb_lane], s[20:21]\n"  \
+      "s_add_u32 s20, s20, %[bstride]\n"  \
+      "s_addc_u32 s21, s21, 0\n"  \
+      "global_load_dwordx4 v[42:45], %[glb_lane], s[20:21]\n"  \
+      "v_mov_b32 v59, 0\n"  \
+      "v_mov_b32 v60, 0\n"  \
+      "v_mov_b32 v61, 0\n"  \
+      "v_mov_b32 v62, 0\n"  \
+      "v_mov_b32 v58, %[lds_lane]\n"  \
+      "ds_read_b128 v[46:49], v58\n"  \
+      "s_add_u32 s53, s22, 1\n"  \
+      "s_sub_u32 s54, %[nt], 1\n"  \
+      "s_min_u32 s53, s53, s54\n"  \
+      "v_readlane_b32 s52, %[tiles], s53\n"  \
+      "s_nop 0\n"  \
+      "s_lshl_b32 s56, s52, 16\n"  \
+      "s_lshr_b32 s57, s52, 16\n"  \
+      "s_add_u32 s26, %[entw_lo], s56\n"  \
+      "s_addc_u32 s27, %[entw_hi], s57\n"  \
+      "v_readlane_b32 s52, %[ys], s53\n"  \
+      "s_nop 0\n"  \
+      "s_lshl_b32 s54, %[bstride], 3\n"  \
+      "s_mul_i32 s56, s52, s54\n"  \
+      "s_mul_hi_u32 s57, s52, s54\n"  \
+      "s_add_u32 s20, %[xsw_lo], s56\n"  \
+      "s_addc_u32 s21, %[xsw_hi], s57\n"  \
+      "50:\n"  \
+      "s_mov_b32 s23, 64\n"  \
+      "7:\n"  \
+      "s_waitcnt lgkmcnt(0)\n"  \
+      "s_load_dwordx16 s[52:67], s[24:25], s23\n"  \
+      "s_add_u32 s23, s23, 64\n"  \
+      "ds_read_b128 v[50:53], v58 offset:1024\n"  \
+      "s_cmp_eq_u32 s36, 0\n"  \
+      "s_cbranch_scc1 101f\n"  \
+      "s_waitcnt vmcnt(7)\n"  \
+      "v_sub_f32 v54, v46, v14\n"  \
+      "v_sub_f32 v55, v47, v15\n"  \
+      "v_sub_f32 v56, v48, v16\n"  \
+      "v_sub_f32 v57, v49, v17\n"  \
+      "v_fma_f32 v59, s36, |v54|, v59\n"  \
+      "v_fma_f32 v60, s36, |v55|, v60\n"  \
+      "v_fma_f32 v61, s36, |v56|, v61\n"  \
+      "v_fma_f32 v62, s36, |v57|, v62\n"  \
+      "101:\n"  \
+      "s_cmp_eq_u32 s37, 0\n"  \
+      "s_cbranch_scc1 102f\n"  \
+      "s_waitcnt vmcnt(6)\n"  \
+      "v_sub_f32 v54, v46, v18\n"  \
+      "v_sub_f32 v55, v47, v19\n"  \
+      "v_sub_f32 v56, v48, v20\n"  \
+      "v_sub_f32 v57, v49, v21\n"  \
+      "v_fma_f32 v59, s37, |v54|, v59\n"  \
+      "v_fma_f32 v60, s37, |v55|, v60\n"  \
+      "v_fma_f32 v61, s37, |v56|, v61\n"  \
+      "v_fma_f32 v62, s37, |v57|, v62\n"  \
+      "102:\n"  \
+      "s_cmp_eq_u32 s38, 0\n"  \
+      "s_cbranch_scc1 103f\n"  \
+      "s_waitcnt vmcnt(5)\n"  \
+      "v_sub_f32 v54, v46, v22\n"  \
+      "v_sub_f32 v55, v47, v23\n"  \
+      "v_sub_f32 v56, v48, v24\n"  \
+      "v_sub_f32 v57, v49, v25\n"  \
+      "v_fma_f32 v59, s38, |v54|, v59\n"  \
+      "v_fma_f32 v60, s38, |v55|, v60\n"  \
+      "v_fma_f32 v61, s38, |v56|, v61\n"  \
+      "v_fma_f32 v62, s38, |v57|, v62\n"  \
+      "103:\n"  \
+      "s_cmp_eq_u32 s39, 0\n"  \
+      "s_cbranch_scc1 104f\n"  \
+      "s_waitcnt vmcnt(4)\n"  \
+      "v_sub_f32 v54, v46, v26\n"  \
+      "v_sub_f32 v55, v47, v27\n"  \
+      "v_sub_f32 v56, v48, v28\n"  \
+      "v_sub_f32 v57, v49, v29\n"  \
+      "v_fma_f32 v59, s39, |v54|, v59\n"  \
+      "v_fma_f32 v60, s39, |v55|, v60\n"  \
+      "v_fma_f32 v61, s39, |v56|, v61\n"  \
+      "v_fma_f32 v62, s39, |v57|, v62\n"  \
+      "104:\n"  \
+      "s_cmp_eq_u32 s40, 0\n"  \
+      "s_cbranch_scc1 105f\n"  \
+      "s_waitcnt vmcnt(3)\n"  \
+      "v_sub_f32 v54, v46, v30\n"  \
+      "v_sub_f32 v55, v47, v31\n"  \
+      "v_sub_f32 v56, v48, v32\n"  \
+      "v_sub_f32 v57, v49, v33\n"  \
+      "v_fma_f32 v59, s40, |v54|, v59\n"  \
+      "v_fma_f32 v60, s40, |v55|, v60\n"  \
+      "v_fma_f32 v61, s40, |v56|, v61\n"  \
+      "v_fma_f32 v62, s40, |v57|, v62\n"  \
+      "105:\n"  \
+      "s_cmp_eq_u32 s41, 0\n"  \
+      "s_cbranch_scc1 106f\n"  \
+      "s_waitcnt vmcnt(2)\n"  \
+      "v_sub_f32 v54, v46, v34\n"  \
+      "v_sub_f32 v55, v47, v35\n"  \
+      "v_sub_f32 v56, v48, v36\n"  \
+      "v_sub_f32 v57, v49, v37\n"  \
+      "v_fma_f32 v59, s41, |v54|, v59\n"  \
+      "v_fma_f32 v60, s41, |v55|, v60\n"  \
+      "v_fma_f32 v61, s41, |v56|, v61\n"  \
+      "v_fma_f32 v62, s41, |v57|, v62\n"  \
+      "106:\n"  \
+      "s_cmp_eq_u32 s42, 0\n"  \
+      "s_cbranch_scc1 107f\n"  \
+      "s_waitcnt vmcnt(1)\n"  \
+      "v_sub_f32 v54, v46, v38\n"  \
+      "v_sub_f32 v55, v47, v39\n"  \
+      "v_sub_f32 v56, v48, v40\n"  \
+      "v_sub_f32 v57, v49, v41\n"  \
+      "v_fma_f32 v59, s42, |v54|, v59\n"  \
+      "v_fma_f32 v60, s42, |v55|, v60\n"  \
+      "v_fma_f32 v61, s42, |v56|, v61\n"  \
+      "v_fma_f32 v62, s42, |v57|, v62\n"  \
+      "107:\n"  \
+      "s_cmp_eq_u32 s43, 0\n"  \
+      "s_cbranch_scc1 108f\n"  \
+      "s_waitcnt vmcnt(0)\n"  \
+      "v_sub_f32 v54, v46, v42\n"  \
+      "v_sub_f32 v55, v47, v43\n"  \
+      "v_sub_f32 v56, v48, v44\n"  \
+      "v_sub_f32 v57, v49, v45\n"  \
+      "v_fma_f32 v59, s43, |v54|, v59\n"  \
+      "v_fma_f32 v60, s43, |v55|, v60\n"  \
+      "v_fma_f32 v61, s43, |v56|, v61\n"  \
+      "v_fma_f32 v62, s43, |v57|, v62\n"  \
+      "108:\n"  \
+      "s_waitcnt vmcnt(0)\n"  \
+      "ds_read_b128 v[46:49], v58 offset:2048\n"  \
+      "s_waitcnt lgkmcnt(1)\n"  \
+      "s_cmp_eq_u32 s44, 0\n"  \
+      "s_cbranch_scc1 109f\n"  \
+      "v_sub_f32 v54, v50, v14\n"  \
+      "v_sub_f32 v55, v51, v15\n"  \
+      "v_sub_f32 v56, v52, v16\n"  \
+      "v_sub_f32 v57, v53, v17\n"  \
+      "v_fma_f32 v59, s44, |v54|, v59\n"  \
+      "v_fma_f32 v60, s44, |v55|, v60\n"  \
+      "v_fma_f32 v61, s44, |v56|, v61\n"  \
+      "v_fma_f32 v62, s44, |v57|, v62\n"  \
+      "109:\n"  \
+      "s_cmp_eq_u32 s45, 0\n"  \
+      "s_cbranch_scc1 110f\n"  \
+      "v_sub_f32 v54, v50, v18\n"  \
+      "v_sub_f32 v55, v51, v19\n"  \
+      "v_sub_f32 v56, v52, v20\n"  \
+      "v_sub_f32 v57, v53, v21\n"  \
+      "v_fma_f32 v59, s45, |v54|, v59\n"  \
+      "v_fma_f32 v60, s45, |v55|, v60\n"  \
+      "v_fma_f32 v61, s45, |v56|, v61\n"  \
+      "v_fma_f32 v62, s45, |v57|, v62\n"  \
+      "110:\n"  \
+      "s_cmp_eq_u32 s46, 0\n"  \
+      "s_cbranch_scc1 111f\n"  \
+      "v_sub_f32 v54, v50, v22\n"  \
+      "v_sub_f32 v55, v51, v23\n"  \
+      "v_sub_f32 v56, v52, v24\n"  \
+      "v_sub_f32 v57, v53, v25\n"  \
+      "v_fma_f32 v59, s46, |v54|, v59\n"  \
+      "v_fma_f32 v60, s46, |v55|, v60\n"  \
+      "v_fma_f32 v61, s46, |v56|, v61\n"  \
+      "v_fma_f32 v62, s46, |v57|, v62\n"  \
+      "111:\n"  \
+      "s_cmp_eq_u32 s47, 0\n"  \
+      "s_cbranch_scc1 112f\n"  \
+      "v_sub_f32 v54, v50, v26\n"  \
+      "v_sub_f32 v55, v51, v27\n"  \
+      "v_sub_f32 v56, v52, v28\n"  \
+      "v_sub_f32 v57, v53, v29\n"  \
+      "v_fma_f32 v59, s47, |v54|, v59\n"  \
+      "v_fma_f32 v60, s47, |v55|, v60\n"  \
+      "v_fma_f32 v61, s47, |v56|, v61\n"  \
+      "v_fma_f32 v62, s47, |v57|, v62\n"  \
+      "112:\n"  \
+      "s_cmp_eq_u32 s48, 0\n"  \
+      "s_cbranch_scc1 113f\n"  \
+      "v_sub_f32 v54, v50, v30\n"  \
+      "v_sub_f32 v55, v51, v31\n"  \
+      "v_sub_f32 v56, v52, v32\n"  \
+      "v_sub_f32 v57, v53, v33\n"  \
+      "v_fma_f32 v59, s48, |v54|, v59\n"  \
+      "v_fma_f32 v60, s48, |v55|, v60\n"  \
+      "v_fma_f32 v61, s48, |v56|, v61\n"  \
+      "v_fma_f32 v62, s48, |v57|, v62\n"  \
+      "113:\n"  \
+      "s_cmp_eq_u32 s49, 0\n"  \
+      "s_cbranch_scc1 114f\n"  \
+      "v_sub_f32 v54, v50, v34\n"  \
+      "v_sub_f32 v55, v51, v35\n"  \
+      "v_sub_f32 v56, v52, v36\n"  \
+      "v_sub_f32 v57, v53, v37\n"  \
+      "v_fma_f32 v59, s49, |v54|, v59\n"  \
+      "v_fma_f32 v60, s49, |v55|, v60\n"  \
+      "v_fma_f32 v61, s49, |v56|, v61\n"  \
+      "v_fma_f32 v62, s49, |v57|, v62\n"  \
+      "114:\n"  \
+      "s_cmp_eq_u32 s50, 0\n"  \
+      "s_cbranch_scc1 115f\n"  \
+      "v_sub_f32 v54, v50, v38\n"  \
+      "v_sub_f32 v55, v51, v39\n"  \
+      "v_sub_f32 v56, v52, v40\n"  \
+      "v_sub_f32 v57, v53, v41\n"  \
+      "v_fma_f32 v59, s50, |v54|, v59\n"  \
+      "v_fma_f32 v60, s50, |v55|, v60\n"  \
+      "v_fma_f32 v61, s50, |v56|, v61\n"  \
+      "v_fma_f32 v62, s50, |v57|, v62\n"  \
+      "115:\n"  \
+      "s_cmp_eq_u32 s51, 0\n"  \
+      "s_cbranch_scc1 116f\n"  \
+      "v_sub_f32 v54, v50, v42\n"  \
+      "v_sub_f32 v55, v51, v43\n"  \
+      "v_sub_f32 v56, v52, v44\n"  \
+      "v_sub_f32 v57, v53, v45\n"  \
+      "v_fma_f32 v59, s51, |v54|, v59\n"  \
+      "v_fma_f32 v60, s51, |v55|, v60\n"  \
+      "v_fma_f32 v61, s51, |v56|, v61\n"  \
+      "v_fma_f32 v62, s51, |v57|, v62\n"  \
+      "116:\n"  \
+      "s_waitcnt lgkmcnt(0)\n"  \
+      "s_load_dwordx16 s[36:51], s[24:25], s23\n"  \
+      "s_add_u32 s23, s23, 64\n"  \
+      "ds_read_b128 v[50:53], v58 offset:3072\n"  \
+      "s_cmp_eq_u32 s52, 0\n"  \
+      "s_cbranch_scc1 117f\n"  \
+      "v_sub_f32 v54, v46, v14\n"  \
+      "v_sub_f32 v55, v47, v15\n"  \
+      "v_sub_f32 v56, v48, v16\n"  \
+      "v_sub_f32 v57, v49, v17\n"  \
+      "v_fma_f32 v59, s52, |v54|, v59\n"  \
+      "v_fma_f32 v60, s52, |v55|, v60\n"  \
+      "v_fma_f32 v61, s52, |v56|, v61\n"  \
+      "v_fma_f32 v62, s52, |v57|, v62\n"  \
+      "117:\n"  \
+      "s_cmp_eq_u32 s53, 0\n"  \
+      "s_cbranch_scc1 118f\n"  \
+      "v_sub_f32 v54, v46, v18\n"  \
+      "v_sub_f32 v55, v47, v19\n"  \
+      "v_sub_f32 v56, v48, v20\n"  \
+      "v_sub_f32 v57, v49, v21\n"  \
+      "v_fma_f32 v59, s53, |v54|, v59\n"  \
+      "v_fma_f32 v60, s53, |v55|, v60\n"  \
+      "v_fma_f32 v61, s53, |v56|, v61\n"  \
+      "v_fma_f32 v62, s53, |v57|, v62\n"  \
+      "118:\n"  \
+      "s_cmp_eq_u32 s54, 0\n"  \
+      "s_cbranch_scc1 119f\n"  \
+      "v_sub_f32 v54, v46, v22\n"  \
+      "v_sub_f32 v55, v47, v23\n"  \
+      "v_sub_f32 v56, v48, v24\n"  \
+      "v_sub_f32 v57, v49, v25\n"  \
+      "v_fma_f32 v59, s54, |v54|, v59\n"  \
+      "v_fma_f32 v60, s54, |v55|, v60\n"  \
+      "v_fma_f32 v61, s54, |v56|, v61\n"  \
+      "v_fma_f32 v62, s54, |v57|, v62\n"  \
+      "119:\n"  \
+      "s_cmp_eq_u32 s55, 0\n"  \
+      "s_cbranch_scc1 120f\n"  \
+      "v_sub_f32 v54, v46, v26\n"  \
+      "v_sub_f32 v55, v47, v27\n"  \
+      "v_sub_f32 v56, v48, v28\n"  \
+      "v_sub_f32 v57, v49, v29\n"  \
+      "v_fma_f32 v59, s55, |v54|, v59\n"  \
+      "v_fma_f32 v60, s55, |v55|, v60\n"  \
+      "v_fma_f32 v61, s55, |v56|, v61\n"  \
+      "v_fma_f32 v62, s55, |v57|, v62\n"  \
+      "120:\n"  \
+      "s_cmp_eq_u32 s56, 0\n"  \
+      "s_cbranch_scc1 121f\n"  \
+      "v_sub_f32 v54, v46, v30\n"  \
+      "v_sub_f32 v55, v47, v31\n"  \
+      "v_sub_f32 v56, v48, v32\n"  \
+      "v_sub_f32 v57, v49, v33\n"  \
+      "v_fma_f32 v59, s56, |v54|, v59\n"  \
+      "v_fma_f32 v60, s56, |v55|, v60\n"  \
+      "v_fma_f32 v61, s56, |v56|, v61\n"  \
+      "v_fma_f32 v62, s56, |v57|, v62\n"  \
+      "121:\n"  \
+      "s_cmp_eq_u32 s57, 0\n"  \
+      "s_cbranch_scc1 122f\n"  \
+      "v_sub_f32 v54, v46, v34\n"  \
+      "v_sub_f32 v55, v47, v35\n"  \
+      "v_sub_f32 v56, v48, v36\n"  \
+      "v_sub_f32 v57, v49, v37\n"  \
+      "v_fma_f32 v59, s57, |v54|, v59\n"  \
+      "v_fma_f32 v60, s57, |v55|, v60\n"  \
+      "v_fma_f32 v61, s57, |v56|, v61\n"  \
+      "v_fma_f32 v62, s57, |v57|, v62\n"  \
+      "122:\n"  \
+      "s_cmp_eq_u32 s58, 0\n"  \
+      "s_cbranch_scc1 123f\n"  \
+      "v_sub_f32 v54, v46, v38\n"  \
+      "v_sub_f32 v55, v47, v39\n"  \
+      "v_sub_f32 v56, v48, v40\n"  \
+      "v_sub_f32 v57, v49, v41\n"  \
+      "v_fma_f32 v59, s58, |v54|, v59\n"  \
+      "v_fma_f32 v60, s58, |v55|, v60\n"  \
+      "v_fma_f32 v61, s58, |v56|, v61\n"  \
+      "v_fma_f32 v62, s58, |v57|, v62\n"  \
+      "123:\n"  \
+      "s_cmp_eq_u32 s59, 0\n"  \
+      "s_cbranch_scc1 124f\n"  \
+      "v_sub_f32 v54, v46, v42\n"  \
+      "v_sub_f32 v55, v47, v43\n"  \
+      "v_sub_f32 v56, v48, v44\n"  \
+      "v_sub_f32 v57, v49, v45\n"  \
+      "v_fma_f32 v59, s59, |v54|, v59\n"  \
+      "v_fma_f32 v60, s59, |v55|, v60\n"  \
+      "v_fma_f32 v61, s59, |v56|, v61\n"  \
+      "v_fma_f32 v62, s59, |v57|, v62\n"  \
+      "124:\n"  \
+      "ds_read_b128 v[46:49], v58 offset:4096\n"  \
+      "s_waitcnt lgkmcnt(1)\n"  \
+      "s_cmp_eq_u32 s60, 0\n"  \
+      "s_cbranch_scc1 125f\n"  \
+      "v_sub_f32 v54, v50, v14\n"  \
+      "v_sub_f32 v55, v51, v15\n"  \
+      "v_sub_f32 v56, v52, v16\n"  \
+      "v_sub_f32 v57, v53, v17\n"  \
+      "v_fma_f32 v59, s60, |v54|, v59\n"  \
+      "v_fma_f32 v60, s60, |v55|, v60\n"  \
+      "v_fma_f32 v61, s60, |v56|, v61\n"  \
+      "v_fma_f32 v62, s60, |v57|, v62\n"  \
+      "125:\n"  \
+      "s_cmp_eq_u32 s61, 0\n"  \
+      "s_cbranch_scc1 126f\n"  \
+      "v_sub_f32 v54, v50, v18\n"  \
+      "v_sub_f32 v55, v51, v19\n"  \
+      "v_sub_f32 v56, v52, v20\n"  \
+      "v_sub_f32 v57, v53, v21\n"  \
+      "v_fma_f32 v59, s61, |v54|, v59\n"  \
+      "v_fma_f32 v60, s61, |v55|, v60\n"  \
+      "v_fma_f32 v61, s61, |v56|, v61\n"  \
+      "v_fma_f32 v62, s61, |v57|, v62\n"  \
+      "126:\n"  \
+      "s_cmp_eq_u32 s62, 0\n"  \
+      "s_cbranch_scc1 127f\n"  \
+      "v_sub_f32 v54, v50, v22\n"  \
+      "v_sub_f32 v55, v51, v23\n"  \
+      "v_sub_f32 v56, v52, v24\n"  \
+      "v_sub_f32 v57, v53, v25\n"  \
+      "v_fma_f32 v59, s62, |v54|, v59\n"  \
+      "v_fma_f32 v60, s62, |v55|, v60\n"  \
+      "v_fma_f32 v61, s62, |v56|, v61\n"  \
+      "v_fma_f32 v62, s62, |v57|, v62\n"  \
+      "127:\n"  \
+      "s_cmp_eq_u32 s63, 0\n"  \
+      "s_cbranch_scc1 128f\n"  \
+      "v_sub_f32 v54, v50, v26\n"  \
+      "v_sub_f32 v55, v51, v27\n"  \
+      "v_sub_f32 v56, v52, v28\n"  \
+      "v_sub_f32 v57, v53, v29\n"  \
+      "v_fma_f32 v59, s63, |v54|, v59\n"  \
+      "v_fma_f32 v60, s63, |v55|, v60\n"  \
+      "v_fma_f32 v61, s63, |v56|, v61\n"  \
+      "v_fma_f32 v62, s63, |v57|, v62\n"  \
+      "128:\n"  \
+      "s_cmp_eq_u32 s64, 0\n"  \
+      "s_cbranch_scc1 129f\n"  \
+      "v_sub_f32 v54, v50, v30\n"  \
+      "v_sub_f32 v55, v51, v31\n"  \
+      "v_sub_f32 v56, v52, v32\n"  \
+      "v_sub_f32 v57, v53, v33\n"  \
+      "v_fma_f32 v59, s64, |v54|, v59\n"  \
+      "v_fma_f32 v60, s64, |v55|, v60\n"  \
+      "v_fma_f32 v61, s64, |v56|, v61\n"  \
+      "v_fma_f32 v62, s64, |v57|, v62\n"  \
+      "129:\n"  \
+      "s_cmp_eq_u32 s65, 0\n"  \
+      "s_cbranch_scc1 130f\n"  \
+      "v_sub_f32 v54, v50, v34\n"  \
+      "v_sub_f32 v55, v51, v35\n"  \
+      "v_sub_f32 v56, v52, v36\n"  \
+      "v_sub_f32 v57, v53, v37\n"  \
+      "v_fma_f32 v59, s65, |v54|, v59\n"  \
+      "v_fma_f32 v60, s65, |v55|, v60\n"  \
+      "v_fma_f32 v61, s65, |v56|, v61\n"  \
+      "v_fma_f32 v62, s65, |v57|, v62\n"  \
+      "130:\n"  \
+      "s_cmp_eq_u32 s66, 0\n"  \
+      "s_cbranch_scc1 131f\n"  \
+      "v_sub_f32 v54, v50, v38\n"  \
+      "v_sub_f32 v55, v51, v39\n"  \
+      "v_sub_f32 v56, v52, v40\n"  \
+      "v_sub_f32 v57, v53, v41\n"  \
+      "v_fma_f32 v59, s66, |v54|, v59\n"  \
+      "v_fma_f32 v60, s66, |v55|, v60\n"  \
+      "v_fma_f32 v61, s66, |v56|, v61\n"  \
+      "v_fma_f32 v62, s66, |v57|, v62\n"  \
+      "131:\n"  \
+      "s_cmp_eq_u32 s67, 0\n"  \
+      "s_cbranch_scc1 132f\n"  \
+      "v_sub_f32 v54, v50, v42\n"  \
+      "v_sub_f32 v55, v51, v43\n"  \
+      "v_sub_f32 v56, v52, v44\n"  \
+      "v_sub_f32 v57, v53, v45\n"  \
+      "v_fma_f32 v59, s67, |v54|, v59\n"  \
+      "v_fma_f32 v60, s67, |v55|, v60\n"  \
+      "v_fma_f32 v61, s67, |v56|, v61\n"  \
+      "v_fma_f32 v62, s67, |v57|, v62\n"  \
+      "132:\n"  \
+      "s_waitcnt lgkmcnt(0)\n"  \
+      "s_load_dwordx16 s[52:67], s[24:25], s23\n"  \
+      "s_add_u32 s23, s23, 64\n"  \
+      "ds_read_b128 v[50:53], v58 offset:5120\n"  \
+      "s_cmp_eq_u32 s36, 0\n"  \
+      "s_cbranch_scc1 133f\n"  \
+      "v_sub_f32 v54, v46, v14\n"  \
+      "v_sub_f32 v55, v47, v15\n"  \
+      "v_sub_f32 v56, v48, v16\n"  \
+      "v_sub_f32 v57, v49, v17\n"  \
+      "v_fma_f32 v59, s36, |v54|, v59\n"  \
+      "v_fma_f32 v60, s36, |v55|, v60\n"  \
+      "v_fma_f32 v61, s36, |v56|, v61\n"  \
+      "v_fma_f32 v62, s36, |v57|, v62\n"  \
+      "133:\n"  \
+      "s_cmp_eq_u32 s37, 0\n"  \
+      "s_cbranch_scc1 134f\n"  \
+      "v_sub_f32 v54, v46, v18\n"  \
+      "v_sub_f32 v55, v47, v19\n"  \
+      "v_sub_f32 v56, v48, v20\n"  \
+      "v_sub_f32 v57, v49, v21\n"  \
+      "v_fma_f32 v59, s37, |v54|, v59\n"  \
+      "v_fma_f32 v60, s37, |v55|, v60\n"  \
+      "v_fma_f32 v61, s37, |v56|, v61\n"  \
+      "v_fma_f32 v62, s37, |v57|, v62\n"  \
+      "134:\n"  \
+      "s_cmp_eq_u32 s38, 0\n"  \
+      "s_cbranch_scc1 135f\n"  \
+      "v_sub_f32 v54, v46, v22\n"  \
+      "v_sub_f32 v55, v47, v23\n"  \
+      "v_sub_f32 v56, v48, v24\n"  \
+      "v_sub_f32 v57, v49, v25\n"  \
+      "v_fma_f32 v59, s38, |v54|, v59\n"  \
+      "v_fma_f32 v60, s38, |v55|, v60\n"  \
+      "v_fma_f32 v61, s38, |v56|, v61\n"  \
+      "v_fma_f32 v62, s38, |v57|, v62\n"  \
+      "135:\n"  \
+      "s_cmp_eq_u32 s39, 0\n"  \
+      "s_cbranch_scc1 136f\n"  \
+      "v_sub_f32 v54, v46, v26\n"  \
+      "v_sub_f32 v55, v47, v27\n"  \
+      "v_sub_f32 v56, v48, v28\n"  \
+      "v_sub_f32 v57, v49, v29\n"  \
+      "v_fma_f32 v59, s39, |v54|, v59\n"  \
+      "v_fma_f32 v60, s39, |v55|, v60\n"  \
+      "v_fma_f32 v61, s39, |v56|, v61\n"  \
+      "v_fma_f32 v62, s39, |v57|, v62\n"  \
+      "136:\n"  \
+      "s_cmp_eq_u32 s40, 0\n"  \
+      "s_cbranch_scc1 137f\n"  \
+      "v_sub_f32 v54, v46, v30\n"  \
+      "v_sub_f32 v55, v47, v31\n"  \
+      "v_sub_f32 v56, v48, v32\n"  \
+      "v_sub_f32 v57, v49, v33\n"  \
+      "v_fma_f32 v59, s40, |v54|, v59\n"  \
+      "v_fma_f32 v60, s40, |v55|, v60\n"  \
+      "v_fma_f32 v61, s40, |v56|, v61\n"  \
+      "v_fma_f32 v62, s40, |v57|, v62\n"  \
+      "137:\n"  \
+      "s_cmp_eq_u32 s41, 0\n"  \
+      "s_cbranch_scc1 138f\n"  \
+      "v_sub_f32 v54, v46, v34\n"  \
+      "v_sub_f32 v55, v47, v35\n"  \
+      "v_sub_f32 v56, v48, v36\n"  \
+      "v_sub_f32 v57, v49, v37\n"  \
+      "v_fma_f32 v59, s41, |v54|, v59\n"  \
+      "v_fma_f32 v60, s41, |v55|, v60\n"  \
+      "v_fma_f32 v61, s41, |v56|, v61\n"  \
+      "v_fma_f32 v62, s41, |v57|, v62\n"  \
+      "138:\n"  \
+      "s_cmp_eq_u32 s42, 0\n"  \
+      "s_cbranch_scc1 139f\n"  \
+      "v_sub_f32 v54, v46, v38\n"  \
+      "v_sub_f32 v55, v47, v39\n"  \
+      "v_sub_f32 v56, v48, v40\n"  \
+      "v_sub_f32 v57, v49, v41\n"  \
+      "v_fma_f32 v59, s42, |v54|, v59\n"  \
+      "v_fma_f32 v60, s42, |v55|, v60\n"  \
+      "v_fma_f32 v61, s42, |v56|, v61\n"  \
+      "v_fma_f32 v62, s42, |v57|, v62\n"  \
+      "139:\n"  \
+      "s_cmp_eq_u32 s43, 0\n"  \
+      "s_cbranch_scc1 140f\n"  \
+      "v_sub_f32 v54, v46, v42\n"  \
+      "v_sub_f32 v55, v47, v43\n"  \
+      "v_sub_f32 v56, v48, v44\n"  \
+      "v_sub_f32 v57, v49, v45\n"  \
+      "v_fma_f32 v59, s43, |v54|, v59\n"  \
+      "v_fma_f32 v60, s43, |v55|, v60\n"  \
+      "v_fma_f32 v61, s43, |v56|, v61\n"  \
+      "v_fma_f32 v62, s43, |v57|, v62\n"  \
+      "140:\n"  \
+      "ds_read_b128 v[46:49], v58 offset:6144\n"  \
+      "s_waitcnt lgkmcnt(1)\n"  \
+      "s_cmp_eq_u32 s44, 0\n"  \
+      "s_cbranch_scc1 141f\n"  \
+      "v_sub_f32 v54, v50, v14\n"  \
+      "v_sub_f32 v55, v51, v15\n"  \
+      "v_sub_f32 v56, v52, v16\n"  \
+      "v_sub_f32 v57, v53, v17\n"  \
+      "v_fma_f32 v59, s44, |v54|, v59\n"  \
+      "v_fma_f32 v60, s44, |v55|, v60\n"  \
+      "v_fma_f32 v61, s44, |v56|, v61\n"  \
+      "v_fma_f32 v62, s44, |v57|, v62\n"  \
+      "141:\n"  \
+      "s_cmp_eq_u32 s45, 0\n"  \
+      "s_cbranch_scc1 142f\n"  \
+      "v_sub_f32 v54, v50, v18\n"  \
+      "v_sub_f32 v55, v51, v19\n"  \
+      "v_sub_f32 v56, v52, v20\n"  \
+      "v_sub_f32 v57, v53, v21\n"  \
+      "v_fma_f32 v59, s45, |v54|, v59\n"  \
+      "v_fma_f32 v60, s45, |v55|, v60\n"  \
+      "v_fma_f32 v61, s45, |v56|, v61\n"  \
+      "v_fma_f32 v62, s45, |v57|, v62\n"  \
+      "142:\n"  \
+      "s_cmp_eq_u32 s46, 0\n"  \
+      "s_cbranch_scc1 143f\n"  \
+      "v_sub_f32 v54, v50, v22\n"  \
+      "v_sub_f32 v55, v51, v23\n"  \
+      "v_sub_f32 v56, v52, v24\n"  \
+      "v_sub_f32 v57, v53, v25\n"  \
+      "v_fma_f32 v59, s46, |v54|, v59\n"  \
+      "v_fma_f32 v60, s46, |v55|, v60\n"  \
+      "v_fma_f32 v61, s46, |v56|, v61\n"  \
+      "v_fma_f32 v62, s46, |v57|, v62\n"  \
+      "143:\n"  \
+      "s_cmp_eq_u32 s47, 0\n"  \
+      "s_cbranch_scc1 144f\n"  \
+      "v_sub_f32 v54, v50, v26\n"  \
+      "v_sub_f32 v55, v51, v27\n"  \
+      "v_sub_f32 v56, v52, v28\n"  \
+      "v_sub_f32 v57, v53, v29\n"  \
+      "v_fma_f32 v59, s47, |v54|, v59\n"  \
+      "v_fma_f32 v60, s47, |v55|, v60\n"  \
+      "v_fma_f32 v61, s47, |v56|, v61\n"  \
+      "v_fma_f32 v62, s47, |v57|, v62\n"  \
+      "144:\n"  \
+      "s_cmp_eq_u32 s48, 0\n"  \
+      "s_cbranch_scc1 145f\n"  \
+      "v_sub_f32 v54, v50, v30\n"  \
+      "v_sub_f32 v55, v51, v31\n"  \
+      "v_sub_f32 v56, v52, v32\n"  \
+      "v_sub_f32 v57, v53, v33\n"  \
+      "v_fma_f32 v59, s48, |v54|, v59\n"  \
+      "v_fma_f32 v60, s48, |v55|, v60\n"  \
+      "v_fma_f32 v61, s48, |v56|, v61\n"  \
+      "v_fma_f32 v62, s48, |v57|, v62\n"  \
+      "145:\n"  \
+      "s_cmp_eq_u32 s49, 0\n"  \
+      "s_cbranch_scc1 146f\n"  \
+      "v_sub_f32 v54, v50, v34\n"  \
+      "v_sub_f32 v55, v51, v35\n"  \
+      "v_sub_f32 v56, v52, v36\n"  \
+      "v_sub_f32 v57, v53, v37\n"  \
+      "v_fma_f32 v59, s49, |v54|, v59\n"  \
+      "v_fma_f32 v60, s49, |v55|, v60\n"  \
+      "v_fma_f32 v61, s49, |v56|, v61\n"  \
+      "v_fma_f32 v62, s49, |v57|, v62\n"  \
+      "146:\n"  \
+      "s_cmp_eq_u32 s50, 0\n"  \
+      "s_cbranch_scc1 147f\n"  \
+      "v_sub_f32 v54, v50, v38\n"  \
+      "v_sub_f32 v55, v51, v39\n"  \
+      "v_sub_f32 v56, v52, v40\n"  \
+      "v_sub_f32 v57, v53, v41\n"  \
+      "v_fma_f32 v59, s50, |v54|, v59\n"  \
+      "v_fma_f32 v60, s50, |v55|, v60\n"  \
+      "v_fma_f32 v61, s50, |v56|, v61\n"  \
+      "v_fma_f32 v62, s50, |v57|, v62\n"  \
+      "147:\n"  \
+      "s_cmp_eq_u32 s51, 0\n"  \
+      "s_cbranch_scc1 148f\n"  \
+      "v_sub_f32 v54, v50, v42\n"  \
+      "v_sub_f32 v55, v51, v43\n"  \
+      "v_sub_f32 v56, v52, v44\n"  \
+      "v_sub_f32 v57, v53, v45\n"  \
+      "v_fma_f32 v59, s51, |v54|, v59\n"  \
+      "v_fma_f32 v60, s51, |v55|, v60\n"  \
+      "v_fma_f32 v61, s51, |v56|, v61\n"  \
+      "v_fma_f32 v62, s51, |v57|, v62\n"  \
+      "148:\n"  \
+      "s_cmp_eq_u32 s23, 2048\n"  \
+      "s_cbranch_scc1 9f\n"  \
+      "s_waitcnt lgkmcnt(0)\n"  \
+      "s_load_dwordx16 s[36:51], s[24:25], s23\n"  \
+      "s_add_u32 s23, s23, 64\n"  \
+      "ds_read_b128 v[50:53], v58 offset:7168\n"  \
+      "s_cmp_eq_u32 s52, 0\n"  \
+      "s_cbranch_scc1 149f\n"  \
+      "v_sub_f32 v54, v46, v14\n"  \
+      "v_sub_f32 v55, v47, v15\n"  \
+      "v_sub_f32 v56, v48, v16\n"  \
+      "v_sub_f32 v57, v49, v17\n"  \
+      "v_fma_f32 v59, s52, |v54|, v59\n"  \
+      "v_fma_f32 v60, s52, |v55|, v60\n"  \
+      "v_fma_f32 v61, s52, |v56|, v61\n"  \
+      "v_fma_f32 v62, s52, |v57|, v62\n"  \
+      "149:\n"  \
+      "s_cmp_eq_u32 s53, 0\n"  \
+      "s_cbranch_scc1 150f\n"  \
+      "v_sub_f32 v54, v46, v18\n"  \
+      "v_sub_f32 v55, v47, v19\n"  \
+      "v_sub_f32 v56, v48, v20\n"  \
+      "v_sub_f32 v57, v49, v21\n"  \
+      "v_fma_f32 v59, s53, |v54|, v59\n"  \
+      "v_fma_f32 v60, s53, |v55|, v60\n"  \
+      "v_fma_f32 v61, s53, |v56|, v61\n"  \
+      "v_fma_f32 v62, s53, |v57|, v62\n"  \
+      "150:\n"  \
+      "s_cmp_eq_u32 s54, 0\n"  \
+      "s_cbranch_scc1 151f\n"  \
+      "v_sub_f32 v54, v46, v22\n"  \
+      "v_sub_f32 v55, v47, v23\n"  \
+      "v_sub_f32 v56, v48, v24\n"  \
+      "v_sub_f32 v57, v49, v25\n"  \
+      "v_fma_f32 v59, s54, |v54|, v59\n"  \
+      "v_fma_f32 v60, s54, |v55|, v60\n"  \
+      "v_fma_f32 v61, s54, |v56|, v61\n"  \
+      "v_fma_f32 v62, s54, |v57|, v62\n"  \
+      "151:\n"  \
+      "s_cmp_eq_u32 s55, 0\n"  \
+      "s_cbranch_scc1 152f\n"  \
+      "v_sub_f32 v54, v46, v26\n"  \
+      "v_sub_f32 v55, v47, v27\n"  \
+      "v_sub_f32 v56, v48, v28\n"  \
+      "v_sub_f32 v57, v49, v29\n"  \
+      "v_fma_f32 v59, s55, |v54|, v59\n"  \
+      "v_fma_f32 v60, s55, |v55|, v60\n"  \
+      "v_fma_f32 v61, s55, |v56|, v61\n"  \
+      "v_fma_f32 v62, s55, |v57|, v62\n"  \
+      "152:\n"  \
+      "s_cmp_eq_u32 s56, 0\n"  \
+      "s_cbranch_scc1 153f\n"  \
+      "v_sub_f32 v54, v46, v30\n"  \
+      "v_sub_f32 v55, v47, v31\n"  \
+      "v_sub_f32 v56, v48, v32\n"  \
+      "v_sub_f32 v57, v49, v33\n"  \
+      "v_fma_f32 v59, s56, |v54|, v59\n"  \
+      "v_fma_f32 v60, s56, |v55|, v60\n"  \
+      "v_fma_f32 v61, s56, |v56|, v61\n"  \
+      "v_fma_f32 v62, s56, |v57|, v62\n"  \
+      "153:\n"  \
+      "s_cmp_eq_u32 s57, 0\n"  \
+      "s_cbranch_scc1 154f\n"  \
+      "v_sub_f32 v54, v46, v34\n"  \
+      "v_sub_f32 v55, v47, v35\n"  \
+      "v_sub_f32 v56, v48, v36\n"  \
+      "v_sub_f32 v57, v49, v37\n"  \
+      "v_fma_f32 v59, s57, |v54|, v59\n"  \
+      "v_fma_f32 v60, s57, |v55|, v60\n"  \
+      "v_fma_f32 v61, s57, |v56|, v61\n"  \
+      "v_fma_f32 v62, s57, |v57|, v62\n"  \
+      "154:\n"  \
+      "s_cmp_eq_u32 s58, 0\n"  \
+      "s_cbranch_scc1 155f\n"  \
+      "v_sub_f32 v54, v46, v38\n"  \
+      "v_sub_f32 v55, v47, v39\n"  \
+      "v_sub_f32 v56, v48, v40\n"  \
+      "v_sub_f32 v57, v49, v41\n"  \
+      "v_fma_f32 v59, s58, |v54|, v59\n"  \
+      "v_fma_f32 v60, s58, |v55|, v60\n"  \
+      "v_fma_f32 v61, s58, |v56|, v61\n"  \
+      "v_fma_f32 v62, s58, |v57|, v62\n"  \
+      "155:\n"  \
+      "s_cmp_eq_u32 s59, 0\n"  \
+      "s_cbranch_scc1 156f\n"  \
+      "v_sub_f32 v54, v46, v42\n"  \
+      "v_sub_f32 v55, v47, v43\n"  \
+      "v_sub_f32 v56, v48, v44\n"  \
+      "v_sub_f32 v57, v49, v45\n"  \
+      "v_fma_f32 v59, s59, |v54|, v59\n"  \
+      "v_fma_f32 v60, s59, |v55|, v60\n"  \
+      "v_fma_f32 v61, s59, |v56|, v61\n"  \
+      "v_fma_f32 v62, s59, |v57|, v62\n"  \
+      "156:\n"  \
+      "v_add_u32 v58, 0x2000, v58\n"  \
+      "ds_read_b128 v[46:49], v58\n"  \
+      "s_waitcnt lgkmcnt(1)\n"  \
+      "s_cmp_eq_u32 s60, 0\n"  \
+      "s_cbranch_scc1 157f\n"  \
+      "v_sub_f32 v54, v50, v14\n"  \
+      "v_sub_f32 v55, v51, v15\n"  \
+      "v_sub_f32 v56, v52, v16\n"  \
+      "v_sub_f32 v57, v53, v17\n"  \
+      "v_fma_f32 v59, s60, |v54|, v59\n"  \
+      "v_fma_f32 v60, s60, |v55|, v60\n"  \
+      "v_fma_f32 v61, s60, |v56|, v61\n"  \
+      "v_fma_f32 v62, s60, |v57|, v62\n"  \
+      "157:\n"  \
+      "s_cmp_eq_u32 s61, 0\n"  \
+      "s_cbranch_scc1 158f\n"  \
+      "v_sub_f32 v54, v50, v18\n"  \
+      "v_sub_f32 v55, v51, v19\n"  \
+      "v_sub_f32 v56, v52, v20\n"  \
+      "v_sub_f32 v57, v53, v21\n"  \
+      "v_fma_f32 v59, s61, |v54|, v59\n"  \
+      "v_fma_f32 v60, s61, |v55|, v60\n"  \
+      "v_fma_f32 v61, s61, |v56|, v61\n"  \
+      "v_fma_f32 v62, s61, |v57|, v62\n"  \
+      "158:\n"  \
+      "s_cmp_eq_u32 s62, 0\n"  \
+      "s_cbranch_scc1 159f\n"  \
+      "v_sub_f32 v54, v50, v22\n"  \
+      "v_sub_f32 v55, v51, v23\n"  \
+      "v_sub_f32 v56, v52, v24\n"  \
+      "v_sub_f32 v57, v53, v25\n"  \
+      "v_fma_f32 v59, s62, |v54|, v59\n"  \
+      "v_fma_f32 v60, s62, |v55|, v60\n"  \
+      "v_fma_f32 v61, s62, |v56|, v61\n"  \
+      "v_fma_f32 v62, s62, |v57|, v62\n"  \
+      "159:\n"  \
+      "s_cmp_eq_u32 s63, 0\n"  \
+      "s_cbranch_scc1 160f\n"  \
+      "v_sub_f32 v54, v50, v26\n"  \
+      "v_sub_f32 v55, v51, v27\n"  \
+      "v_sub_f32 v56, v52, v28\n"  \
+      "v_sub_f32 v57, v53, v29\n"  \
+      "v_fma_f32 v59, s63, |v54|, v59\n"  \
+      "v_fma_f32 v60, s63, |v55|, v60\n"  \
+      "v_fma_f32 v61, s63, |v56|, v61\n"  \
+      "v_fma_f32 v62, s63, |v57|, v62\n"  \
+      "160:\n"  \
+      "s_cmp_eq_u32 s64, 0\n"  \
+      "s_cbranch_scc1 161f\n"  \
+      "v_sub_f32 v54, v50, v30\n"  \
+      "v_sub_f32 v55, v51, v31\n"  \
+      "v_sub_f32 v56, v52, v32\n"  \
+      "v_sub_f32 v57, v53, v33\n"  \
+      "v_fma_f32 v59, s64, |v54|, v59\n"  \
+      "v_fma_f32 v60, s64, |v55|, v60\n"  \
+      "v_fma_f32 v61, s64, |v56|, v61\n"  \
+      "v_fma_f32 v62, s64, |v57|, v62\n"  \
+      "161:\n"  \
+      "s_cmp_eq_u32 s65, 0\n"  \
+      "s_cbranch_scc1 162f\n"  \
+      "v_sub_f32 v54, v50, v34\n"  \
+      "v_sub_f32 v55, v51, v35\n"  \
+      "v_sub_f32 v56, v52, v36\n"  \
+      "v_sub_f32 v57, v53, v37\n"  \
+      "v_fma_f32 v59, s65, |v54|, v59\n"  \
+      "v_fma_f32 v60, s65, |v55|, v60\n"  \
+      "v_fma_f32 v61, s65, |v56|, v61\n"  \
+      "v_fma_f32 v62, s65, |v57|, v62\n"  \
+      "162:\n"  \
+      "s_cmp_eq_u32 s66, 0\n"  \
+      "s_cbranch_scc1 163f\n"  \
+      "v_sub_f32 v54, v50, v38\n"  \
+      "v_sub_f32 v55, v51, v39\n"  \
+      "v_sub_f32 v56, v52, v40\n"  \
+      "v_sub_f32 v57, v53, v41\n"  \
+      "v_fma_f32 v59, s66, |v54|, v59\n"  \
+      "v_fma_f32 v60, s66, |v55|, v60\n"  \
+      "v_fma_f32 v61, s66, |v56|, v61\n"  \
+      "v_fma_f32 v62, s66, |v57|, v62\n"  \
+      "163:\n"  \
+      "s_cmp_eq_u32 s67, 0\n"  \
+      "s_cbranch_scc1 164f\n"  \
+      "v_sub_f32 v54, v50, v42\n"  \
+      "v_sub_f32 v55, v51, v43\n"  \
+      "v_sub_f32 v56, v52, v44\n"  \
+      "v_sub_f32 v57, v53, v45\n"  \
+      "v_fma_f32 v59, s67, |v54|, v59\n"  \
+      "v_fma_f32 v60, s67, |v55|, v60\n"  \
+      "v_fma_f32 v61, s67, |v56|, v61\n"  \
+      "v_fma_f32 v62, s67, |v57|, v62\n"  \
+      "164:\n"  \
+      "s_branch 7b\n"  \
+      "9:\n"  \
+      "s_waitcnt lgkmcnt(0)\n"  \
+      "s_mov_b64 s[24:25], s[26:27]\n"  \
+      "s_load_dwordx16 s[36:51], s[24:25], 0x0\n"  \
+      "ds_read_b128 v[50:53], v58 offset:7168\n"  \
+      "s_cmp_eq_u32 s52, 0\n"  \
+      "s_cbranch_scc1 165f\n"  \
+      "v_sub_f32 v54, v46, v14\n"  \
+      "v_sub_f32 v55, v47, v15\n"  \
+      "v_sub_f32 v56, v48, v16\n"  \
+      "v_sub_f32 v57, v49, v17\n"  \
+      "v_fma_f32 v59, s52, |v54|, v59\n"  \
+      "v_fma_f32 v60, s52, |v55|, v60\n"  \
+      "v_fma_f32 v61, s52, |v56|, v61\n"  \
+      "v_fma_f32 v62, s52, |v57|, v62\n"  \
+      "165:\n"  \
+      "s_cmp_eq_u32 s53, 0\n"  \
+      "s_cbranch_scc1 166f\n"  \
+      "v_sub_f32 v54, v46, v18\n"  \
+      "v_sub_f32 v55, v47, v19\n"  \
+      "v_sub_f32 v56, v48, v20\n"  \
+      "v_sub_f32 v57, v49, v21\n"  \
+      "v_fma_f32 v59, s53, |v54|, v59\n"  \
+      "v_fma_f32 v60, s53, |v55|, v60\n"  \
+      "v_fma_f32 v61, s53, |v56|, v61\n"  \
+      "v_fma_f32 v62, s53, |v57|, v62\n"  \
+      "166:\n"  \
+      "s_cmp_eq_u32 s54, 0\n"  \
+      "s_cbranch_scc1 167f\n"  \
+      "v_sub_f32 v54, v46, v22\n"  \
+      "v_sub_f32 v55, v47, v23\n"  \
+      "v_sub_f32 v56, v48, v24\n"  \
+      "v_sub_f32 v57, v49, v25\n"  \
+      "v_fma_f32 v59, s54, |v54|, v59\n"  \
+      "v_fma_f32 v60, s54, |v55|, v60\n"  \
+      "v_fma_f32 v61, s54, |v56|, v61\n"  \
+      "v_fma_f32 v62, s54, |v57|, v62\n"  \
+      "167:\n"  \
+      "s_cmp_eq_u32 s55, 0\n"  \
+      "s_cbranch_scc1 168f\n"  \
+      "v_sub_f32 v54, v46, v26\n"  \
+      "v_sub_f32 v55, v47, v27\n"  \
+      "v_sub_f32 v56, v48, v28\n"  \
+      "v_sub_f32 v57, v49, v29\n"  \
+      "v_fma_f32 v59, s55, |v54|, v59\n"  \
+      "v_fma_f32 v60, s55, |v55|, v60\n"  \
+      "v_fma_f32 v61, s55, |v56|, v61\n"  \
+      "v_fma_f32 v62, s55, |v57|, v62\n"  \
+      "168:\n"  \
+      "s_cmp_eq_u32 s56, 0\n"  \
+      "s_cbranch_scc1 169f\n"  \
+      "v_sub_f32 v54, v46, v30\n"  \
+      "v_sub_f32 v55, v47, v31\n"  \
+      "v_sub_f32 v56, v48, v32\n"  \
+      "v_sub_f32 v57, v49, v33\n"  \
+      "v_fma_f32 v59, s56, |v54|, v59\n"  \
+      "v_fma_f32 v60, s56, |v55|, v60\n"  \
+      "v_fma_f32 v61, s56, |v56|, v61\n"  \
+      "v_fma_f32 v62, s56, |v57|, v62\n"  \
+      "169:\n"  \
+      "s_cmp_eq_u32 s57, 0\n"  \
+      "s_cbranch_scc1 170f\n"  \
+      "v_sub_f32 v54, v46, v34\n"  \
+      "v_sub_f32 v55, v47, v35\n"  \
+      "v_sub_f32 v56, v48, v36\n"  \
+      "v_sub_f32 v57, v49, v37\n"  \
+      "v_fma_f32 v59, s57, |v54|, v59\n"  \
+      "v_fma_f32 v60, s57, |v55|, v60\n"  \
+      "v_fma_f32 v61, s57, |v56|, v61\n"  \
+      "v_fma_f32 v62, s57, |v57|, v62\n"  \
+      "170:\n"  \
+      "s_cmp_eq_u32 s58, 0\n"  \
+      "s_cbranch_scc1 171f\n"  \
+      "v_sub_f32 v54, v46, v38\n"  \
+      "v_sub_f32 v55, v47, v39\n"  \
+      "v_sub_f32 v56, v48, v40\n"  \
+      "v_sub_f32 v57, v49, v41\n"  \
+      "v_fma_f32 v59, s58, |v54|, v59\n"  \
+      "v_fma_f32 v60, s58, |v55|, v60\n"  \
+      "v_fma_f32 v61, s58, |v56|, v61\n"  \
+      "v_fma_f32 v62, s58, |v57|, v62\n"  \
+      "171:\n"  \
+      "s_cmp_eq_u32 s59, 0\n"  \
+      "s_cbranch_scc1 172f\n"  \
+      "v_sub_f32 v54, v46, v42\n"  \
+      "v_sub_f32 v55, v47, v43\n"  \
+      "v_sub_f32 v56, v48, v44\n"  \
+      "v_sub_f32 v57, v49, v45\n"  \
+      "v_fma_f32 v59, s59, |v54|, v59\n"  \
+      "v_fma_f32 v60, s59, |v55|, v60\n"  \
+      "v_fma_f32 v61, s59, |v56|, v61\n"  \
+      "v_fma_f32 v62, s59, |v57|, v62\n"  \
+      "172:\n"  \
+      "v_mov_b32 v58, %[lds_lane]\n"  \
+      "ds_read_b128 v[46:49], v58\n"  \
+      "s_waitcnt lgkmcnt(1)\n"  \
+      "s_cmp_eq_u32 s60, 0\n"  \
+      "s_cbranch_scc1 173f\n"  \
+      "v_sub_f32 v54, v50, v14\n"  \
+      "v_sub_f32 v55, v51, v15\n"  \
+      "v_sub_f32 v56, v52, v16\n"  \
+      "v_sub_f32 v57, v53, v17\n"  \
+      "v_fma_f32 v59, s60, |v54|, v59\n"  \
+      "v_fma_f32 v60, s60, |v55|, v60\n"  \
+      "v_fma_f32 v61, s60, |v56|, v61\n"  \
+      "v_fma_f32 v62, s60, |v57|, v62\n"  \
+      "173:\n"  \
+      "global_load_dwordx4 v[14:17], %[glb_lane], s[20:21]\n"  \
+      "s_add_u32 s20, s20, %[bstride]\n"  \
+      "s_addc_u32 s21, s21, 0\n"  \
+      "s_cmp_eq_u32 s61, 0\n"  \
+      "s_cbranch_scc1 174f\n"  \
+      "v_sub_f32 v54, v50, v18\n"  \
+      "v_sub_f32 v55, v51, v19\n"  \
+      "v_sub_f32 v56, v52, v20\n"  \
+      "v_sub_f32 v57, v53, v21\n"  \
+      "v_fma_f32 v59, s61, |v54|, v59\n"  \
+      "v_fma_f32 v60, s61, |v55|, v60\n"  \
+      "v_fma_f32 v61, s61, |v56|, v61\n"  \
+      "v_fma_f32 v62, s61, |v57|, v62\n"  \
+      "174:\n"  \
+      "global_load_dwordx4 v[18:21], %[glb_lane], s[20:21]\n"  \
+      "s_add_u32 s20, s20, %[bstride]\n"  \
+      "s_addc_u32 s21, s21, 0\n"  \
+      "s_cmp_eq_u32 s62, 0\n"  \
+      "s_cbranch_scc1 175f\n"  \
+      "v_sub_f32 v54, v50, v22\n"  \
+      "v_sub_f32 v55, v51, v23\n"  \
+      "v_sub_f32 v56, v52, v24\n"  \
+      "v_sub_f32 v57, v53, v25\n"  \
+      "v_fma_f32 v59, s62, |v54|, v59\n"  \
+      "v_fma_f32 v60, s62, |v55|, v60\n"  \
+      "v_fma_f32 v61, s62, |v56|, v61\n"  \
+      "v_fma_f32 v62, s62, |v57|, v62\n"  \
+      "175:\n"  \
+      "global_load_dwordx4 v[22:25], %[glb_lane], s[20:21]\n"  \
+      "s_add_u32 s20, s20, %[bstride]\n"  \
+      "s_addc_u32 s21, s21, 0\n"  \
+      "s_cmp_eq_u32 s63, 0\n"  \
+      "s_cbranch_scc1 176f\n"  \
+      "v_sub_f32 v54, v50, v26\n"  \
+      "v_sub_f32 v55, v51, v27\n"  \
+      "v_sub_f32 v56, v52, v28\n"  \
+      "v_sub_f32 v57, v53, v29\n"  \
+      "v_fma_f32 v59, s63, |v54|, v59\n"  \
+      "v_fma_f32 v60, s63, |v55|, v60\n"  \
+      "v_fma_f32 v61, s63, |v56|, v61\n"  \
+      "v_fma_f32 v62, s63, |v57|, v62\n"  \
+      "176:\n"  \
+      "global_load_dwordx4 v[26:29], %[glb_lane], s[20:21]\n"  \
+      "s_add_u32 s20, s20, %[bstride]\n"  \
+      "s_addc_u32 s21, s21, 0\n"  \
+      "s_cmp_eq_u32 s64, 0\n"  \
+      "s_cbranch_scc1 177f\n"  \
+      "v_sub_f32 v54, v50, v30\n"  \
+      "v_sub_f32 v55, v51, v31\n"  \
+      "v_sub_f32 v56, v52, v32\n"  \
+      "v_sub_f32 v57, v53, v33\n"  \
+      "v_fma_f32 v59, s64, |v54|, v59\n"  \
+      "v_fma_f32 v60, s64, |v55|, v60\n"  \
+      "v_fma_f32 v61, s64, |v56|, v61\n"  \
+      "v_fma_f32 v62, s64, |v57|, v62\n"  \
+      "177:\n"  \
+      "global_load_dwordx4 v[30:33], %[glb_lane], s[20:21]\n"  \
+      "s_add_u32 s20, s20, %[bstride]\n"  \
+      "s_addc_u32 s21, s21, 0\n"  \
+      "s_cmp_eq_u32 s65, 0\n"  \
+      "s_cbranch_scc1 178f\n"  \
+      "v_sub_f32 v54, v50, v34\n"  \
+      "v_sub_f32 v55, v51, v35\n"  \
+      "v_sub_f32 v56, v52, v36\n"  \
+      "v_sub_f32 v57, v53, v37\n"  \
+      "v_fma_f32 v59, s65, |v54|, v59\n"  \
+      "v_fma_f32 v60, s65, |v55|, v60\n"  \
+      "v_fma_f32 v61, s65, |v56|, v61\n"  \
+      "v_fma_f32 v62, s65, |v57|, v62\n"  \
+      "178:\n"  \
+      "global_load_dwordx4 v[34:37], %[glb_lane], s[20:21]\n"  \
+      "s_add_u32 s20, s20, %[bstride]\n"  \
+      "s_addc_u32 s21, s21, 0\n"  \
+      "s_cmp_eq_u32 s66, 0\n"  \
+      "s_cbranch_scc1 179f\n"  \
+      "v_sub_f32 v54, v50, v38\n"  \
+      "v_sub_f32 v55, v51, v39\n"  \
+      "v_sub_f32 v56, v52, v40\n"  \
+      "v_sub_f32 v57, v53, v41\n"  \
+      "v_fma_f32 v59, s66, |v54|, v59\n"  \
+      "v_fma_f32 v60, s66, |v55|, v60\n"  \
+      "v_fma_f32 v61, s66, |v56|, v61\n"  \
+      "v_fma_f32 v62, s66, |v57|, v62\n"  \
+      "179:\n"  \
+      "global_load_dwordx4 v[38:41], %[glb_lane], s[20:21]\n"  \
+      "s_add_u32 s20, s20, %[bstride]\n"  \
+      "s_addc_u32 s21, s21, 0\n"  \
+      "s_cmp_eq_u32 s67, 0\n"  \
+      "s_cbranch_scc1 180f\n"  \
+      "v_sub_f32 v54, v50, v42\n"  \
+      "v_sub_f32 v55, v51, v43\n"  \
+      "v_sub_f32 v56, v52, v44\n"  \
+      "v_sub_f32 v57, v53, v45\n"  \
+      "v_fma_f32 v59, s67, |v54|, v59\n"  \
+      "v_fma_f32 v60, s67, |v55|, v60\n"  \
+      "v_fma_f32 v61, s67, |v56|, v61\n"  \
+      "v_fma_f32 v62, s67, |v57|, v62\n"  \
+      "180:\n"  \
+      "global_load_dwordx4 v[42:45], %[glb_lane], s[20:21]\n"  \
+      "v_cvt_f64_f32 v[54:55], v59\n"  \
+      "v_add_f64 %[s0], %[s0], v[54:55]\n"  \
+      "v_mov_b32 v59, 0\n"  \
+      "v_cvt_f64_f32 v[54:55], v60\n"  \
+      "v_add_f64 %[s1], %[s1], v[54:55]\n"  \
+      "v_mov_b32 v60, 0\n"  \
+      "v_cvt_f64_f32 v[54:55], v61\n"  \
+      "v_add_f64 %[s2], %[s2], v[54:55]\n"  \
+      "v_mov_b32 v61, 0\n"  \
+      "v_cvt_f64_f32 v[54:55], v62\n"  \
+      "v_add_f64 %[s3], %[s3], v[54:55]\n"  \
+      "v_mov_b32 v62, 0\n"  \
+      "v_mov_b32 v56, %[wgd]\n"  \
+      "v_min_u32 v57, 1, %[glb_lane]\n"  \
+      "v_xor_b32 v57, 1, v57\n"  \
+      "ds_add_rtn_u32 v56, v56, v57\n"  \
+      "s_add_u32 s22, s22, 1\n"  \
+      "s_add_u32 s53, s22, 1\n"  \
+      "s_sub_u32 s54, %[nt], 1\n"  \
+      "s_min_u32 s53, s53, s54\n"  \
+      "v_readlane_b32 s52, %[tiles], s53\n"  \
+      "s_nop 0\n"  \
+      "s_lshl_b32 s56, s52, 16\n"  \
+      "s_lshr_b32 s57, s52, 16\n"  \
+      "s_add_u32 s26, %[entw_lo], s56\n"  \
+      "s_addc_u32 s27, %[entw_hi], s57\n"  \
+      "v_readlane_b32 s52, %[ys], s53\n"  \
+      "s_nop 0\n"  \
+      "s_lshl_b32 s54, %[bstride], 3\n"  \
+      "s_mul_i32 s56, s52, s54\n"  \
+      "s_mul_hi_u32 s57, s52, s54\n"  \
+      "s_add_u32 s20, %[xsw_lo], s56\n"  \
+      "s_addc_u32 s21, %[xsw_hi], s57\n"  \
+      "s_waitcnt lgkmcnt(0)\n"  \
+      "s_nop 0\n"  \
+      "v_readfirstlane_b32 s52, v56\n"  \
+      "s_nop 0\n"  \
+      "s_add_u32 s52, s52, 1\n"  \
+      "s_add_u32 s54, s22, %[done0]\n"  \
+      "s_lshl_b32 s54, s54, 4\n"  \
+      "s_cmp_lt_u32 s54, s52\n"  \
+      "s_cbranch_scc1 64f\n"  \
+      "s_setprio 0\n"  \
+      "s_branch 65f\n"  \
+      "64:\n"  \
+      "s_setprio 2\n"  \
+      "65:\n"  \
+      "s_cmp_lt_u32 s22, %[nt]\n"  \
+      "s_cbranch_scc1 50b\n"  \
+      "s_waitcnt vmcnt(0) lgkmcnt(0)\n"  \
+      : [s0] "+v"(s_[0]), [s1] "+v"(s_[1]), [s2] "+v"(s_[2]), [s3] "+v"(s_[3])  \
+      : [lds_lane] "v"(lds_lane_), [glb_lane] "v"(glb_lane_), [tiles] "v"(tiles_), [ys] "v"(ys_),  \
+        [nt] "s"(nt_), [entw_lo] "s"(entw_lo_), [entw_hi] "s"(entw_hi_), [xsw_lo] "s"(xsw_lo_),  \
+        [xsw_hi] "s"(xsw_hi_), [bstride] "s"(bstride_), [wgd] "s"(wgd_),  \
+        [done0] "s"(done0_)  \
+      : "v14", "v15", "v16", "v17", "v18", "v19", "v20", "v21", "v22", "v23", "v24", "v25", "v26", "v27", "v28", "v29", "v30", "v31", "v32", "v33", "v34", "v35", "v36", "v37", "v38", "v39", "v40", "v41", "v42", "v43", "v44", "v45", "v46", "v47", "v48", "v49", "v50", "v51", "v52", "v53", "v54", "v55", "v56", "v57", "v58", "v59", "v60", "v61", "v62",  \
+        "s0", "s1", "s2", "s3", "s20", "s21", "s22", "s23", "s24", "s25", "s26", "s27", "s36", "s37", "s38", "s39", "s40", "s41", "s42", "s43", "s44", "s45", "s46", "s47", "s48", "s49", "s50", "s51", "s52", "s53", "s54", "s55", "s56", "s57", "s58", "s59", "s60", "s61", "s62", "s63", "s64", "s65", "s66", "s67", "scc", "memory")
```

New measurement: 2.931 billion, median of 6. +1.5%, better.
